# iucario/WorkoutDetector

Measured on AMD Instinct MI355X. Metric: clips/sec (8x3x224x224 TSM-R50), higher is better.
Workload: dtype f32

## Files before the change

workoutdetector_amd/csrc/tsm_engine.hip:

```cpp
#include <hip/hip_runtime.h>

#include <sys/stat.h>

#include <algorithm>
#include <cerrno>
#include <cmath>
#include <cstdio>
#include <cstdlib>
#include <cstring>
#include <map>
#include <string>
#include <vector>

#include "../../include/tsm_hip.h"
#include "tsm_host_util.h"
#include "tsm_kernels.h"

#ifndef TSM_BUILD_ID
#define TSM_BUILD_ID __DATE__ "/" __TIME__
#endif

namespace {

using namespace tsm_host;

const char kBuildTag[] = "tsm-build-id:" TSM_BUILD_ID;

struct Backbone {
  int depth;
  int blocks[4];
  bool basic;
};
constexpr Backbone kBackbones[] = {{18, {2, 2, 2, 2}, true}, {34, {3, 4, 6, 3}, true}, {50, {3, 4, 6, 3}, false}};
constexpr int kPlanes[4] = {64, 128, 256, 512};

const Backbone *find_backbone(int depth) {
  for (const Backbone &b : kBackbones)
    if (b.depth == depth) return &b;
  return nullptr;
}

thread_local std::string g_create_error;

struct HostTensor {
  std::vector<float> data;
  std::vector<int64_t> shape;
};

struct ConvLayer {
  std::string wkey, bnp;
  int cin = 0, cout = 0, k = 1, stride = 1;
  int cp = 0;
  int kp = 0;
  int kseg = 0;
  float *d_w = nullptr, *d_b = nullptr;
};

struct Block {
  int conv1, conv2, conv3, down;
  int stride;
  std::string name;
  float *d_wf = nullptr, *d_bf = nullptr;
  int kpf = 0;
  int ksegf = 0;
  float *d_w3f = nullptr;
  int cmid = 0;
  int cout3 = 0;
};

int ilog2(int v) {
  int l = 0;
  while ((1 << l) < v) ++l;
  return l;
}

struct GuardBuf {
  std::string name;
  char *base = nullptr;
  GuardLayout lay;
  size_t elem_bytes = 4;
  float *ptr() const { return reinterpret_cast<float *>(base + lay.lead); }
};

hipError_t guard_alloc(GuardBuf *g, const char *name, size_t payload_bytes, size_t frame_bytes, size_t elem_bytes = 4) {
  g->name = name;
  g->lay = guard_layout(payload_bytes, frame_bytes);
  g->elem_bytes = elem_bytes;
  void *q = nullptr;
  hipError_t st = hipMalloc(&q, g->lay.total());
  if (st != hipSuccess) return st;
  g->base = static_cast<char *>(q);
  st = hipMemsetD32(reinterpret_cast<hipDeviceptr_t>(q), (int)kPoisonWord, g->lay.total() / 4);
  return st != hipSuccess ? st : hipDeviceSynchronize();
}

hipError_t guard_verify(const GuardBuf &g, std::string *msg) {
  std::vector<uint32_t> host(std::max(g.lay.lead, g.lay.tail) / 4);
  for (int after = 0; after < 2; ++after) {
    const size_t bytes = after ? g.lay.tail : g.lay.lead;
    const hipError_t st = hipMemcpy(host.data(), g.base + (after ? g.lay.lead + g.lay.payload : 0), bytes, hipMemcpyDeviceToHost);
    if (st != hipSuccess) return st;
    const long bad = guard_first_bad(host.data(), bytes / 4);
    if (bad >= 0) {
      *msg = guard_message(g.name, g.lay, after != 0, (size_t)bad, g.elem_bytes, host[bad]);
      return hipSuccess;
    }
  }
  return hipSuccess;
}

}

struct tsm_engine {
  tsm_config cfg{};
  int depth = 50;
  int width = 64;
  int place = 0;
  int consensus = 0;
  int feat = 2048;
  bool weights_started = false;
  size_t tune_sig_base = 0;
  std::string err;
  hipStream_t stream = nullptr;
  bool finalized = false;
  int prec = tsm::kPrecF32;
  float *d_tap = nullptr;
  std::map<std::string, HostTensor> tensors;
  std::vector<ConvLayer> convs;
  std::vector<Block> blocks;
  float *d_fcw = nullptr, *d_fcb = nullptr;
  float *d_in = nullptr;
  float *d_in4 = nullptr;
  float *buf[5] = {nullptr, nullptr, nullptr, nullptr, nullptr};
  float *d_pooled = nullptr, *d_logits = nullptr;
  float *d_partial = nullptr;
  size_t partial_elems = 0;
  size_t buf_elems = 0;
  int h1 = 0, w1 = 0, hp = 0, wp = 0;
  hipEvent_t ev0 = nullptr, ev1 = nullptr;
  bool have_time = false;
  std::vector<void *> allocs;
  bool poison = false;
  std::vector<GuardBuf> guards;
  std::map<int, std::vector<int>> tile_cache;
  bool autotune = true;
  bool stem_pool = true;
  bool stem_direct = true;
  bool stem_planar = true;
  std::string tune_path, tune_sig;
  int force_tile = 0, force_code = -1;
  int fuse23 = -1;
  int fuse_block = -1;
  int fuse31 = -1;
  int fuse_front = -1;
  int walk = -1;
  int n_cu = 256;
  int timing_left = 0;
  bool timing_only3x3 = false;
  std::vector<std::vector<hipEvent_t>> timing;
  std::vector<hipEvent_t> event_pool;
  std::vector<hipEvent_t> *cur_timing = nullptr;
};

namespace {

int fail(tsm_engine *e, int code, const std::string &msg) {
  if (e) e->err = msg; else g_create_error = msg;
  return code;
}

#define TSM_HIP(e, call)                                                                        \
  do {                                                                                          \
    hipError_t _st = (call);                                                                    \
    if (_st != hipSuccess)                                                                      \
      return fail((e), TSM_ERR_HIP, std::string(#call) + ": " + hipGetErrorString(_st));        \
  } while (0)

void build_topology(tsm_engine *e) {
  e->convs.clear();
  e->blocks.clear();
  ConvLayer stem;
  stem.wkey = "base_model.conv1.weight";
  stem.bnp = "base_model.bn1";
  stem.cin = 3; stem.cout = 64; stem.k = 7; stem.stride = 2;
  stem.cp = 4;
  stem.kp = e->prec == tsm::kPrecF32 ? round_up(7 * 7 * 4, 32) : round_up(7 * 4 * 8, e->prec == tsm::kPrecBf16 ? 64 : 32);
  e->convs.push_back(stem);
  const Backbone &bb = *find_backbone(e->depth);
  const int expansion = bb.basic ? 1 : 4;
  int cin = 64;
  for (int li = 0; li < 4; ++li) {
    for (int b = 0; b < bb.blocks[li]; ++b) {
      const int planes = kPlanes[li];
      const int mid = planes * e->width / 64;
      const int stride = (b == 0 && li > 0) ? 2 : 1;
      const bool bp = e->place == 1;
      const std::string p = "base_model.layer" + std::to_string(li + 1) + "." + std::to_string(b) + (bp ? ".net" : "");
      const std::string c1key = p + (bp ? ".conv1.weight" : ".conv1.net.weight");
      Block blk;
      blk.stride = stride;
      blk.name = "layer" + std::to_string(li + 1) + "." + std::to_string(b);
      blk.down = -1;
      if (bb.basic) {
        ConvLayer c1; c1.wkey = c1key; c1.bnp = p + ".bn1";
        c1.cin = cin; c1.cout = planes; c1.k = 3; c1.stride = stride; c1.cp = cin; c1.kp = 9 * cin;
        ConvLayer c2; c2.wkey = p + ".conv2.weight"; c2.bnp = p + ".bn2";
        c2.cin = planes; c2.cout = planes; c2.k = 3; c2.stride = 1; c2.cp = planes; c2.kp = 9 * planes;
        c1.kseg = e->cfg.is_shift ? 0 : segment_len(c1.kp, e->prec);
        blk.conv1 = (int)e->convs.size(); e->convs.push_back(c1);
        blk.conv2 = (int)e->convs.size(); e->convs.push_back(c2);
        blk.conv3 = -1;
        if (stride != 1 || cin != planes) {
          ConvLayer d; d.wkey = p + ".downsample.0.weight"; d.bnp = p + ".downsample.1";
          d.cin = cin; d.cout = planes; d.k = 1; d.stride = stride; d.cp = cin; d.kp = cin;
          blk.down = (int)e->convs.size(); e->convs.push_back(d);
        }
        e->blocks.push_back(blk);
        cin = planes;
        continue;
      }
      ConvLayer c1; c1.wkey = c1key; c1.bnp = p + ".bn1";
      c1.cin = cin; c1.cout = mid; c1.k = 1; c1.stride = 1; c1.cp = cin; c1.kp = cin;
      ConvLayer c2; c2.wkey = p + ".conv2.weight"; c2.bnp = p + ".bn2";
      c2.cin = mid; c2.cout = mid; c2.k = 3; c2.stride = stride; c2.cp = mid; c2.kp = 9 * mid;
      ConvLayer c3; c3.wkey = p + ".conv3.weight"; c3.bnp = p + ".bn3";
      c3.cin = mid; c3.cout = planes * 4; c3.k = 1; c3.stride = 1; c3.cp = mid; c3.kp = mid;
      c1.kseg = segment_len(c1.kp, e->prec);
      c2.kseg = segment_len(c2.kp, e->prec);
      blk.conv1 = (int)e->convs.size(); e->convs.push_back(c1);
      blk.conv2 = (int)e->convs.size(); e->convs.push_back(c2);
      blk.conv3 = (int)e->convs.size(); e->convs.push_back(c3);
      if (b == 0) {
        ConvLayer d; d.wkey = p + ".downsample.0.weight"; d.bnp = p + ".downsample.1";
        d.cin = cin; d.cout = planes * 4; d.k = 1; d.stride = stride; d.cp = cin; d.kp = cin;
        blk.down = (int)e->convs.size(); e->convs.push_back(d);
      }
      e->blocks.push_back(blk);
      cin = planes * 4;
    }
  }
  e->feat = kPlanes[3] * expansion;
}

std::string unwrapped(const tsm_engine *e, const std::string &key) {
  if (e->place == 1) {
    const size_t at = key.find(".net.");
    return at == std::string::npos ? "" : key.substr(0, at) + key.substr(at + 4);
  }
  const std::string net = ".conv1.net.weight";
  if (key.size() > net.size() && key.compare(key.size() - net.size(), net.size(), net) == 0)
    return key.substr(0, key.size() - net.size()) + ".conv1.weight";
  return "";
}

const HostTensor *find_tensor(const tsm_engine *e, const std::string &key) {
  auto it = e->tensors.find(key);
  if (it != e->tensors.end()) return &it->second;
  const std::string alt = unwrapped(e, key);
  if (!alt.empty()) {
    it = e->tensors.find(alt);
    if (it != e->tensors.end()) return &it->second;
  }
  return nullptr;
}

bool known_name(const tsm_engine *e, const std::string &name) {
  if (name == "fc.weight" || name == "fc.bias") return true;
  static const char *bn_suffix[] = {".weight", ".bias", ".running_mean", ".running_var", ".num_batches_tracked"};
  auto is = [&](const std::string &key) { return name == key || name == unwrapped(e, key); };
  for (const ConvLayer &c : e->convs) {
    if (is(c.wkey)) return true;
    for (const char *s : bn_suffix)
      if (is(c.bnp + s)) return true;
  }
  return false;
}

int dev_alloc(tsm_engine *e, float **p, size_t elems, const char *name = "weights", size_t frame_elems = 0) {
  if (e->poison) {
    GuardBuf g;
    TSM_HIP(e, guard_alloc(&g, name, elems * sizeof(float), frame_elems * sizeof(float)));
    e->allocs.push_back(g.base);
    e->guards.push_back(g);
    *p = g.ptr();
    return TSM_OK;
  }
  void *q = nullptr;
  TSM_HIP(e, hipMalloc(&q, elems * sizeof(float)));
  e->allocs.push_back(q);
  *p = static_cast<float *>(q);
  return TSM_OK;
}

int poison_workspace(tsm_engine *e, hipStream_t s) {
  if (!e->poison) return TSM_OK;
  const float *targets[] = {e->buf[0], e->buf[1], e->buf[2], e->buf[3], e->buf[4], e->d_in4, e->d_pooled, e->d_logits, e->d_partial, e->d_tap};
  for (const GuardBuf &g : e->guards)
    for (const float *t : targets)
      if (t && t == g.ptr())
        TSM_HIP(e, hipMemsetD32Async(reinterpret_cast<hipDeviceptr_t>(g.ptr()), (int)kPoisonWord, g.lay.payload / 4, s));
  return TSM_OK;
}

int verify_guards(tsm_engine *e, hipStream_t s) {
  if (!e->poison) return TSM_OK;
  TSM_HIP(e, hipStreamSynchronize(s));
  for (const GuardBuf &g : e->guards) {
    std::string msg;
    TSM_HIP(e, guard_verify(g, &msg));
    if (!msg.empty()) return fail(e, TSM_ERR_GUARD, msg);
  }
  return TSM_OK;
}

tsm::ConvParams make_params(const ConvLayer &c, const float *x, const float *res, float *y, int n, int hi,
                            int wi, bool relu, int T, int shift_div, int prec = tsm::kPrecF32) {
  tsm::ConvParams p{};
  p.prec = prec;
  p.x = x; p.w = c.d_w; p.bias = c.d_b; p.res = res; p.y = y;
  p.N = n; p.Hi = hi; p.Wi = wi; p.C = c.cp; p.logC4 = ilog2(c.cp / 4);
  p.pad = c.k / 2; p.stride = c.stride;
  p.Ho = (hi + 2 * p.pad - c.k) / c.stride + 1;
  p.Wo = (wi + 2 * p.pad - c.k) / c.stride + 1;
  p.Cout = c.cout; p.Kp = c.kp; p.M = n * p.Ho * p.Wo; p.relu = relu ? 1 : 0;
  p.T = T; p.fold = T > 0 ? c.cp / shift_div : 0;
  p.kseg_len = res ? 0 : c.kseg;
  return p;
}

std::string default_tune_cache_path() {
  std::string base;
  if (const char *x = getenv("XDG_CACHE_HOME")) base = x;
  if (base.empty()) {
    const char *h = getenv("HOME");
    if (!h || !*h) return "";
    base = std::string(h) + "/.cache";
    (void)mkdir(base.c_str(), 0700);
  }
  base += "/tsm_hip";
  if (mkdir(base.c_str(), 0700) != 0 && errno != EEXIST) return "";
  return base + "/tune_cache.txt";
}

bool tune_cache_load(tsm_engine *e, int key, std::vector<int> *codes) {
  if (e->tune_path.empty()) return false;
  FILE *f = fopen(e->tune_path.c_str(), "r");
  if (!f) return false;
  const std::string want = e->tune_sig + "|" + std::to_string(key) + "|";
  char line[4096];
  bool ok = false;
  while (!ok && fgets(line, sizeof line, f)) ok = parse_tune_line(line, want, tsm::kNumTiles, codes);
  fclose(f);
  return ok;
}

void tune_cache_store(tsm_engine *e, int key, const std::vector<int> &codes) {
  if (e->tune_path.empty()) return;
  std::string line = e->tune_sig + "|" + std::to_string(key) + "|";
  for (size_t i = 0; i < codes.size(); ++i) line += (i ? "," : "") + std::to_string(codes[i]);
  line += "\n";
  if (line.size() >= 4096) return;
  FILE *f = fopen(e->tune_path.c_str(), "a");
  if (!f) return;
  fwrite(line.data(), 1, line.size(), f);
  fclose(f);
}

bool tail_split_from(const tsm::ConvParams &p, int n_cu, size_t partial_elems, int *tail_from) {
  if (p.kseg_len <= 0) return false;
  const long from = tsm_host::tail_split_point(p.M, p.Cout, tsm::conv_num_segments(p), n_cu, partial_elems);
  *tail_from = (int)from;
  return from > 0;
}

hipError_t launch_conv_code(tsm::ConvParams p, int ks, int code, float *partial, size_t partial_elems, int n_cu, hipStream_t s) {
  p.tile = code & kCodeTileMask;
  if ((code & kCodeSplitK) && p.kseg_len > 0 &&
      (size_t)tsm::conv_num_segments(p) * (size_t)p.M * (size_t)p.Cout <= partial_elems) {
    float *y = p.y;
    p.ksplit = 1;
    p.y = partial;
    hipError_t st = tsm::launch_conv(p, ks, s);
    if (st == hipSuccess)
      st = tsm::launch_splitk_reduce(partial, tsm::conv_num_segments(p), p.M, p.Cout, p.bias, nullptr, y, p.relu, s);
    return st;
  }
  if ((code & kCodeTailK) && (code & kCodeTileMask) == tsm::kTile64x64 && p.kseg_len > 0) {
    int tail_from = 0;
    if (tail_split_from(p, n_cu, partial_elems, &tail_from)) {
      float *y = p.y;
      const int mt0 = tail_from / (p.Cout / 64) * 64;
      p.ksplit = 2;
      p.tail_from = tail_from;
      p.ypart = partial;
      hipError_t st = tsm::launch_conv(p, ks, s);
      if (st == hipSuccess)
        st = tsm::launch_splitk_reduce(partial, tsm::conv_num_segments(p), p.M - mt0, p.Cout, p.bias, nullptr,
                                       y + (size_t)mt0 * p.Cout, p.relu, s);
      return st;
    }
  }
  return tsm::launch_conv(p, ks, s);
}

int checked_code(const tsm::ConvParams &p, int code) {
  return code > 0 && (code & ~kCodeValid) == 0 && tsm::conv_tile_valid(p, code & kCodeTileMask) ? code : 0;
}

struct Tap {
  const float *ptr = nullptr;
  int64_t shape[4] = {0, 0, 0, 0};
  bool hit = false;
};

struct LaunchTimer {
  tsm_engine *e;
  hipStream_t s;
  bool on;
  bool skip;
  LaunchTimer(tsm_engine *e_, hipStream_t s_, bool is3x3)
      : e(e_), s(s_), on(e_->cur_timing != nullptr), skip(e_->timing_only3x3 && !is3x3) { mark(); }
  ~LaunchTimer() { mark(); }
  void mark() {
    if (!on) return;
    if (skip) {
      e->cur_timing->push_back(nullptr);
      return;
    }
    hipEvent_t ev = nullptr;
    if (!e->event_pool.empty()) {
      ev = e->event_pool.back();
      e->event_pool.pop_back();
    } else if (hipEventCreate(&ev) != hipSuccess) {
      return;
    }
    (void)hipEventRecord(ev, s);
    e->cur_timing->push_back(ev);
  }
};
#define TSM_LAUNCH_K(e, s, is3x3, call) \
  do {                                  \
    LaunchTimer _lt((e), (s), (is3x3)); \
    TSM_HIP((e), (call));               \
  } while (0)
#define TSM_LAUNCH(e, s, call) TSM_LAUNCH_K(e, s, false, call)

void skip_slots(tsm_engine *e, int n) {
  if (e->cur_timing) e->cur_timing->insert(e->cur_timing->end(), 2 * (size_t)n, nullptr);
}

template <class F>
int time_best_of(tsm_engine *e, hipStream_t s, F &&launches, float *best_ms) {
  float ms[4];
  for (int rep = 0; rep < 4; ++rep) {
    TSM_HIP(e, hipEventRecord(e->ev0, s));
    TSM_HIP(e, launches());
    TSM_HIP(e, hipEventRecord(e->ev1, s));
    TSM_HIP(e, hipEventSynchronize(e->ev1));
    TSM_HIP(e, hipEventElapsedTime(&ms[rep], e->ev0, e->ev1));
  }
  *best_ms = std::min(ms[1], std::min(ms[2], ms[3]));
  return TSM_OK;
}

bool block_shift(const tsm_engine *e) { return e->place == 1 && e->cfg.is_shift; }

struct BlockLaunches {
  tsm::ConvParams p1, p2, p3;
  tsm::BneckParams pb{};
  tsm::FrontParams pfr{};
  tsm::Fused23Params pf{};
  tsm::Conv31Params q{};
};

BlockLaunches block_launches(const tsm_engine *e, size_t k, int nn, const float *x, float *y, float *t1, float *t2, int hh, int ww) {
  const tsm_config &cfg = e->cfg;
  const Block &blk = e->blocks[k];
  const ConvLayer &c1 = e->convs[blk.conv1], &c2 = e->convs[blk.conv2], &c3 = e->convs[blk.conv3];
  const int T = cfg.num_segments, shiftT = cfg.is_shift ? T : 0, prec = e->prec;
  const int ho = (hh + 2 - 3) / blk.stride + 1, wo = (ww + 2 - 3) / blk.stride + 1;
  const bool fused = blk.down >= 0;
  BlockLaunches L;
  L.p1 = make_params(c1, x, nullptr, t1, nn, hh, ww, true, shiftT, cfg.shift_div, prec);
  L.p2 = make_params(c2, t1, nullptr, t2, nn, hh, ww, true, 0, 1, prec);
  L.p3 = make_params(c3, t2, fused ? nullptr : x, y, nn, ho, wo, true, 0, 1, prec);
  if (fused) {
    const ConvLayer &cd = e->convs[blk.down];
    L.p3.w = blk.d_wf; L.p3.bias = blk.d_bf; L.p3.Kp = blk.kpf; L.p3.K1 = c3.kp; L.p3.kseg_len = blk.ksegf;
    L.p3.x2 = x; L.p3.C2 = cd.cp; L.p3.Hi2 = hh; L.p3.Wi2 = ww; L.p3.stride2 = blk.stride;
  }
  if (block_shift(e)) {
    L.p3.T = T;
    L.p3.fold = (fused ? e->convs[blk.down].cp : c3.cout) / cfg.shift_div;
  }
  tsm::BneckParams &pb = L.pb;
  pb.x = x; pb.w1 = c1.d_w; pb.bias1 = c1.d_b; pb.w2 = c2.d_w; pb.bias2 = c2.d_b; pb.y = y;
  pb.w3 = fused ? blk.d_wf : c3.d_w; pb.bias3 = fused ? blk.d_bf : c3.d_b;
  pb.cin = c1.cin; pb.N = nn; pb.H = hh; pb.W = ww; pb.T = shiftT; pb.fold = L.p1.fold;
  tsm::FrontParams &pfr = L.pfr;
  pfr.x = x; pfr.w1 = c1.d_w; pfr.bias1 = c1.d_b; pfr.w2 = c2.d_w; pfr.bias2 = c2.d_b; pfr.y = t2;
  pfr.N = nn; pfr.H = hh; pfr.W = ww; pfr.T = shiftT; pfr.fold = L.p1.fold;
  tsm::Fused23Params &pf = L.pf;
  pf.x = t1; pf.w2 = c2.d_w; pf.bias2 = c2.d_b; pf.w3f = blk.d_w3f ? blk.d_w3f : c3.d_w; pf.bias3 = c3.d_b; pf.res = x; pf.y = y;
  pf.N = nn; pf.H = hh; pf.W = ww; pf.M = nn * hh * ww; pf.kseg_len = c2.kseg;
  if (k + 1 < e->blocks.size() && e->blocks[k + 1].conv3 >= 0) {
    const ConvLayer &c1n = e->convs[e->blocks[k + 1].conv1];
    tsm::Conv31Params &q = L.q;
    q.t2 = L.p3.x; q.w3 = L.p3.w; q.bias3 = L.p3.bias; q.res = L.p3.res; q.y = L.p3.y;
    q.w1 = c1n.d_w; q.bias1 = c1n.d_b; q.t1 = t1;
    q.n_clips = nn / T; q.T = T; q.HW = ho * wo; q.K3 = L.p3.C; q.C = L.p3.Cout; q.N1 = c1n.cout;
    q.fold = shiftT > 0 ? c1n.cp / cfg.shift_div : 0;
  }
  return L;
}

struct BlockForms {
  bool block = false, front = false, conv23 = false, conv31 = false;
};

BlockForms fused_forms(const tsm_engine *e, size_t k, int nn, int hh, int ww, const char *stage) {
  BlockForms f;
  const Block &blk = e->blocks[k];
  if (blk.conv3 < 0 || block_shift(e)) return f;
  const ConvLayer &c1 = e->convs[blk.conv1], &c2 = e->convs[blk.conv2], &c3 = e->convs[blk.conv3];
  const BlockLaunches L = block_launches(e, k, nn, nullptr, nullptr, nullptr, nullptr, hh, ww);
  const bool bf16 = e->prec == tsm::kPrecBf16;
  auto want = [&](const char *part) { return stage && blk.name + part == stage; };
  f.block = bf16 && blk.stride == 1 && c1.cout == 64 && c2.cin == 64 && c2.cout == 64 && c3.cout == 256 &&
            (blk.down < 0 ? c1.cin == 256 : c1.cin == 64 && e->convs[blk.down].cp == 64) && e->fuse_block != 0 &&
            tsm::bneck_ws_valid(L.pb.cin, L.pb.N, L.pb.H, L.pb.W, L.pb.T, L.pb.fold) && !want(".conv1") && !want(".conv2");
  f.front = bf16 && blk.stride == 2 && c1.cin == 256 && c1.cout == 128 && c2.cin == 128 && c2.cout == 128 && e->fuse_front != 0 &&
            tsm::front_s2_valid(L.pfr.N, L.pfr.H, L.pfr.W, L.pfr.T, L.pfr.fold) && !want(".conv1");
  f.conv23 = (blk.d_w3f != nullptr || (bf16 && blk.cmid == 64 && tsm::conv23_ws_valid(nn, hh, ww))) && e->fuse23 != 0 &&
             !want(".conv2");
  f.conv31 = bf16 && blk.down < 0 && k + 1 < e->blocks.size() && e->blocks[k + 1].conv3 >= 0 && e->fuse31 != 0 &&
             tsm::conv31_valid(L.q);
  return f;
}

struct BlockPlan {
  bool block = false, front = false, conv1_done = false, conv23 = false, conv31_next = false;
};

std::vector<BlockPlan> plan_forward(const tsm_engine *e, const std::vector<int> *codes, int nn, const char *stage) {
  std::vector<BlockPlan> plan(e->blocks.size());
  int hh = e->hp, ww = e->wp;
  for (size_t k = 0; k < e->blocks.size(); ++k) {
    const Block &blk = e->blocks[k];
    const BlockForms can = fused_forms(e, k, nn, hh, ww, stage);
    auto chosen = [&](int force, int conv, int bit) { return force == 1 || (codes && ((*codes)[conv] & bit)); };
    BlockPlan &p = plan[k];
    p.conv1_done = k > 0 && plan[k - 1].conv31_next;
    if (can.block && chosen(e->fuse_block, blk.conv1, kCodeBlock)) p.block = true;
    else if (can.front && !p.conv1_done && chosen(e->fuse_front, blk.conv1, kCodeFront)) p.front = true;
    else if (can.conv23 && chosen(e->fuse23, blk.conv2, kCodeConv23)) p.conv23 = true;
    else if (can.conv31 && chosen(e->fuse31, blk.conv3, kCodeConv31)) p.conv31_next = true;
    hh = (hh + 2 - 3) / blk.stride + 1;
    ww = (ww + 2 - 3) / blk.stride + 1;
  }
  return plan;
}

struct Forward {
  tsm_engine *e;
  hipStream_t s;
  const char *stage;
  Tap *tap;
  int T, shiftT, prec;
  float *t1, *t2, *idb;
  std::vector<int> *tiles = nullptr;
  bool tuning = false;
  bool tapped = false;
  int flip = 0;
  int prev31 = -1;
  BlockLaunches prev;

  Forward(tsm_engine *e_, hipStream_t s_, const char *stage_, Tap *tap_)
      : e(e_), s(s_), stage(stage_), tap(tap_), T(e_->cfg.num_segments), shiftT(e_->cfg.is_shift ? T : 0), prec(e_->prec),
        t1(e_->buf[2]), t2(e_->buf[3]), idb(e_->buf[4]) {}

  int dir(int d) const { return e->walk >= 0 ? e->walk : d; }
  int next_dir() { return dir(flip ^= 1); }
  bool want(const std::string &name) const { return stage && name == stage; }
  int hit(const float *p, int64_t a, int64_t b, int64_t c, int64_t d) {
    tap->ptr = p; tap->shape[0] = a; tap->shape[1] = b; tap->shape[2] = c; tap->shape[3] = d; tap->hit = true;
    tapped = true;
    return TSM_OK;
  }
  hipError_t launch_code(tsm::ConvParams p, int ks, int code);
  hipError_t launch_pair(const tsm::ConvParams &a, int ks_a, int code_a, const tsm::ConvParams &b, int ks_b, int code_b) {
    const hipError_t st = launch_code(a, ks_a, code_a);
    return st != hipSuccess ? st : launch_code(b, ks_b, code_b);
  }
  template <class A, class B>
  int fused_wins(A &&many, B &&one, bool *wins) {
    float many_ms = 0.f, one_ms = 0.f;
    int rc = time_best_of(e, s, many, &many_ms);
    if (!rc) rc = time_best_of(e, s, one, &one_ms);
    *wins = one_ms < many_ms;
    return rc;
  }
  int conv(int idx, tsm::ConvParams p, int ks, bool is3x3);
  int run_basic(size_t k, int nn, float *x, float *y, int hh, int ww);
  int run_block(size_t k, const BlockPlan &plan, int nn, float *x, float *y, int hh, int ww);
  int tune_block(size_t k, int nn, float *x, float *y, int hh, int ww);
};

hipError_t Forward::launch_code(tsm::ConvParams p, int ks, int code) {
  return launch_conv_code(p, ks, code, e->d_partial, e->partial_elems, e->n_cu, s);
}

int Forward::conv(int idx, tsm::ConvParams p, int ks, bool is3x3) {
  p.reverse = next_dir();
  if (!tuning) {
    int code = tiles ? (*tiles)[idx] : 0;
    if (e->force_tile) code = e->force_tile;
    if (e->force_code >= 0) code = e->force_code;
    TSM_LAUNCH_K(e, s, is3x3, launch_code(p, ks, checked_code(p, code)));
    return TSM_OK;
  }
  std::vector<int> cands;
  if (p.kseg_len > 0) {
    const size_t need = (size_t)tsm::conv_num_segments(p) * p.M * p.Cout;
    const long tiles64 = (long)((p.M + 63) / 64) * (p.Cout / 64);
    for (int t : {(int)tsm::kTile64x64, (int)tsm::kTile32x32}) {
      cands.push_back(t);
      if (need <= e->partial_elems && tiles64 < 4L * e->n_cu) cands.push_back(t | kCodeSplitK);
    }
    int tail_from = 0;
    if (tail_split_from(p, e->n_cu, e->partial_elems, &tail_from)) cands.push_back((int)tsm::kTile64x64 | kCodeTailK);
  } else {
    for (int t = 1; t < tsm::kNumTiles; ++t)
      if (tsm::conv_tile_valid(p, t)) cands.push_back(t);
  }
  float best_ms = 0.f;
  int best = 0;
  for (int t : cands) {
    float ms = 0.f;
    const int rc = time_best_of(e, s, [&] { return launch_code(p, ks, t); }, &ms);
    if (rc) return rc;
    if (best == 0 || ms < best_ms) {
      best = t;
      best_ms = ms;
    }
  }
  (*tiles)[idx] = best;
  return TSM_OK;
}

int Forward::run_basic(size_t k, int nn, float *x, float *y, int hh, int ww) {
  const Block &blk = e->blocks[k];
  const std::string &name = blk.name;
  const ConvLayer &c1 = e->convs[blk.conv1], &c2 = e->convs[blk.conv2];
  const int ho = (hh + 2 - 3) / blk.stride + 1, wo = (ww + 2 - 3) / blk.stride + 1;
  const float *identity = x;
  if (blk.down >= 0) {
    tsm::ConvParams pd = make_params(e->convs[blk.down], x, nullptr, idb, nn, hh, ww, false, block_shift(e) ? shiftT : 0,
                                     e->cfg.shift_div, prec);
    int rcd = conv(blk.down, pd, 1, false);
    if (rcd) return rcd;
    identity = idb;
  }
  tsm::ConvParams p1 = make_params(c1, x, nullptr, t1, nn, hh, ww, true, shiftT, e->cfg.shift_div, prec);
  int rc1 = conv(blk.conv1, p1, 3, true);
  if (rc1) return rc1;
  if (want(name + ".conv1")) return hit(t1, nn, ho, wo, c1.cout);
  tsm::ConvParams p2 = make_params(c2, t1, identity, y, nn, ho, wo, true, 0, 1, prec);
  if (block_shift(e) && blk.down < 0) {
    p2.T = T;
    p2.fold = c2.cout / e->cfg.shift_div;
  }
  int rc2 = conv(blk.conv2, p2, 3, true);
  if (rc2) return rc2;
  if (want(name)) return hit(y, nn, ho, wo, c2.cout);
  return TSM_OK;
}

int Forward::run_block(size_t k, const BlockPlan &plan, int nn, float *x, float *y, int hh, int ww) {
  const Block &blk = e->blocks[k];
  const std::string &name = blk.name;
  const int c1out = e->convs[blk.conv1].cout, c2out = e->convs[blk.conv2].cout, c3out = e->convs[blk.conv3].cout;
  const int ho = (hh + 2 - 3) / blk.stride + 1, wo = (ww + 2 - 3) / blk.stride + 1;
  BlockLaunches L = block_launches(e, k, nn, x, y, t1, t2, hh, ww);
  if (blk.down >= 0) skip_slots(e, 1);
  if (plan.block) {
    L.pb.reverse = next_dir();
    TSM_LAUNCH(e, s, tsm::launch_bneck_ws(L.pb, s));
    skip_slots(e, 2);
    return want(name) ? hit(y, nn, ho, wo, c3out) : TSM_OK;
  }
  if (plan.front) {
    L.pfr.reverse = next_dir();
    TSM_LAUNCH(e, s, tsm::launch_front_s2(L.pfr, s));
    next_dir();
    skip_slots(e, 1);
  } else {
    if (plan.conv1_done) {
      skip_slots(e, 1);
    } else {
      int rc1 = conv(blk.conv1, L.p1, 1, false);
      if (rc1) return rc1;
    }
    if (want(name + ".conv1")) return hit(t1, nn, hh, ww, c1out);
    if (plan.conv23) {
      L.pf.reverse = next_dir();
      TSM_LAUNCH_K(e, s, true, tsm::launch_conv23_fused(L.pf, blk.cmid, blk.cout3, prec, s));
      skip_slots(e, 1);
      return want(name) ? hit(y, nn, ho, wo, c3out) : TSM_OK;
    }
    int rc2 = conv(blk.conv2, L.p2, 3, true);
    if (rc2) return rc2;
  }
  if (want(name + ".conv2")) return hit(t2, nn, ho, wo, c2out);
  if (plan.conv31_next) {
    L.q.reverse = next_dir();
    TSM_LAUNCH(e, s, tsm::launch_conv31_fused(L.q, s));
  } else {
    int rc3 = conv(blk.conv3, L.p3, 1, false);
    if (rc3) return rc3;
  }
  return want(name) ? hit(y, nn, ho, wo, c3out) : TSM_OK;
}

int Forward::tune_block(size_t k, int nn, float *x, float *y, int hh, int ww) {
  const Block &blk = e->blocks[k];
  std::vector<int> &codes = *tiles;
  const BlockForms can = fused_forms(e, k, nn, hh, ww, nullptr);
  BlockLaunches L = block_launches(e, k, nn, x, y, t1, t2, hh, ww);
  const int r1 = flip ^ 1;
  bool wins = false;
  int rc = conv(blk.conv1, L.p1, 1, false);
  if (rc) return rc;
  L.p1.reverse = dir(r1);
  if (prev31 >= 0 && e->fuse31 < 0) {
    const int conv3 = e->blocks[prev31].conv3, code3 = codes[conv3], code1 = codes[blk.conv1];
    tsm::ConvParams pc = L.p1;
    pc.reverse = dir(prev.p3.reverse ^ 1);
    prev.q.reverse = prev.p3.reverse;
    rc = fused_wins([&] { return launch_pair(prev.p3, 1, code3, pc, 1, code1); },
                    [&] { return tsm::launch_conv31_fused(prev.q, s); }, &wins);
    if (rc) return rc;
    if (wins) codes[conv3] |= kCodeConv31;
  }
  rc = conv(blk.conv2, L.p2, 3, true);
  if (rc) return rc;
  L.p2.reverse = dir(r1 ^ 1);
  if (can.front && e->fuse_front < 0) {
    const int code1 = codes[blk.conv1], code2 = codes[blk.conv2];
    L.pfr.reverse = dir(r1);
    rc = fused_wins([&] { return launch_pair(L.p1, 1, code1, L.p2, 3, code2); },
                    [&] { return tsm::launch_front_s2(L.pfr, s); }, &wins);
    if (rc) return rc;
    if (wins) codes[blk.conv1] |= kCodeFront;
  }
  rc = conv(blk.conv3, L.p3, 1, false);
  if (rc) return rc;
  L.p3.reverse = dir(r1);
  prev31 = can.conv31 ? (int)k : -1;
  prev = L;
  const int code1 = codes[blk.conv1], code2 = codes[blk.conv2], code3 = codes[blk.conv3];
  L.pf.reverse = dir(r1 ^ 1);
  L.pb.reverse = dir(r1);
  auto pair = [&] { return launch_pair(L.p2, 3, code2, L.p3, 1, code3); };
  auto fused23 = [&] { return tsm::launch_conv23_fused(L.pf, blk.cmid, blk.cout3, prec, s); };
  bool use_fused = can.conv23 && e->fuse23 == 1;
  if (can.conv23 && e->fuse23 < 0) {
    rc = fused_wins(pair, fused23, &use_fused);
    if (rc) return rc;
    if (use_fused) codes[blk.conv2] |= kCodeConv23;
  }
  if (can.block && e->fuse_block < 0) {
    rc = fused_wins([&] {
      const hipError_t st = launch_code(L.p1, 1, code1);
      return st != hipSuccess ? st : use_fused ? fused23() : pair();
    }, [&] { return tsm::launch_bneck_ws(L.pb, s); }, &wins);
    if (rc) return rc;
    if (wins) codes[blk.conv1] |= kCodeBlock;
  }
  return TSM_OK;
}

int run_forward(tsm_engine *e, const float *d_clips, int layout, int n_clips, float *d_logits,
                hipStream_t s, const char *stage, Tap *tap) {
  const tsm_config &cfg = e->cfg;
  const int T = cfg.num_segments, n = n_clips * T;
  Forward f(e, s, stage, tap);
  if (e->autotune && !stage) {
    auto it = e->tile_cache.find(tile_bucket(n_clips) * T);
    if (it == e->tile_cache.end()) {
      it = e->tile_cache.emplace(tile_bucket(n_clips) * T, std::vector<int>(e->convs.size(), 0)).first;
      f.tuning = true;
    }
    f.tiles = &it->second;
  }

  const int prec = e->prec;
  const float *in4 = e->d_in4;
  const bool pool_stem = e->stem_direct && e->stem_pool && !f.want("conv1");
  const bool planar = layout == TSM_LAYOUT_NTCHW && e->stem_planar && pool_stem && !f.want("input") &&
                      (double)cfg.height * cfg.width * 12.0 < 2.0e9 && (reinterpret_cast<uintptr_t>(d_clips) & 15u) == 0;
  if (layout >= TSM_LAYOUT_NTHWC4 || planar) {
    in4 = d_clips;
    skip_slots(e, 1);
  } else {
    TSM_LAUNCH(e, s, tsm::launch_pack_input(d_clips, e->d_in4, n, cfg.height, cfg.width,
                                            layout == TSM_LAYOUT_NTCHW ? 1 : 0, prec, s));
  }
  if (f.want("input"))
    return prec == tsm::kPrecF32 ? f.hit(in4, n, cfg.height, cfg.width, 4) : f.hit(in4, n, cfg.height, (cfg.width + 1) / 2, 8);

  float *cur = e->buf[0], *out = e->buf[1], *t1 = f.t1;
  {
    tsm::ConvParams p = make_params(e->convs[0], in4, nullptr, t1, n, cfg.height, cfg.width, true, 0, 1, prec);
    const bool direct = prec != tsm::kPrecF32 && e->stem_direct;
    if (pool_stem) {
      TSM_LAUNCH(e, s, tsm::launch_stem_pool(in4, e->convs[0].d_w, e->convs[0].d_b, cur, n, cfg.height, cfg.width,
                                              e->convs[0].kp, 1, prec, s, planar ? 1 : 0));
      skip_slots(e, 1);
    } else {
      if (direct) {
        TSM_LAUNCH(e, s, tsm::launch_stem_direct(in4, e->convs[0].d_w, e->convs[0].d_b, t1, n, cfg.height, cfg.width,
                                                  e->convs[0].kp, 1, prec, s));
      } else {
        int rc0 = f.conv(0, p, 7, false);
        if (rc0) return rc0;
      }
      if (f.want("conv1")) return f.hit(t1, n, e->h1, e->w1, 64);
      TSM_LAUNCH(e, s, tsm::launch_maxpool3x3s2(t1, cur, n, e->h1, e->w1, 64, prec, s));
    }
    if (f.want("stem")) return f.hit(cur, n, e->hp, e->wp, 64);
  }
  int h = e->hp, w = e->wp;
  const std::vector<BlockPlan> plan = f.tuning ? std::vector<BlockPlan>() : plan_forward(e, f.tiles, n, stage);
  for (size_t k = 0; k < e->blocks.size(); ++k) {
    const int rc = e->blocks[k].conv3 < 0 ? f.run_basic(k, n, cur, out, h, w)
                   : f.tuning            ? f.tune_block(k, n, cur, out, h, w)
                                         : f.run_block(k, plan[k], n, cur, out, h, w);
    if (rc || f.tapped) return rc;
    std::swap(cur, out);
    h = (h + 2 - 3) / e->blocks[k].stride + 1;
    w = (w + 2 - 3) / e->blocks[k].stride + 1;
  }
  if (stage) return fail(e, TSM_ERR_INVALID_ARG, std::string("unknown stage: ") + stage);
  if (e->consensus == 1) {
    TSM_LAUNCH(e, s, tsm::launch_head_segments(cur, e->d_fcw, e->d_fcb, d_logits, n, h * w, e->feat, cfg.num_class, prec, s));
    return TSM_OK;
  }
  TSM_LAUNCH(e, s, tsm::launch_head(cur, e->d_fcw, e->d_fcb, e->d_pooled, d_logits, n_clips, T, h * w, e->feat,
                                    cfg.num_class, prec, s));
  return TSM_OK;
}

int ensure_tuned(tsm_engine *e, const float *d_clips, int layout, int n_clips, float *d_out, hipStream_t s,
                 bool *from_file = nullptr) {
  const int tune_key = tile_bucket(n_clips) * e->cfg.num_segments;
  if (from_file) *from_file = false;
  if (!e->autotune || e->tile_cache.find(tune_key) != e->tile_cache.end()) return TSM_OK;
  std::vector<int> cached(e->convs.size(), 0);
  if (tune_cache_load(e, tune_key, &cached)) {
    e->tile_cache.emplace(tune_key, cached);
    if (from_file) *from_file = true;
    return TSM_OK;
  }
  std::vector<hipEvent_t> *saved = e->cur_timing;
  e->cur_timing = nullptr;
  const int rc = run_forward(e, d_clips, layout, n_clips, d_out, s, nullptr, nullptr);
  e->cur_timing = saved;
  if (rc) return rc;
  tune_cache_store(e, tune_key, e->tile_cache[tune_key]);
  return TSM_OK;
}

hipStream_t pick_stream(tsm_engine *e, int memkind, void *stream) {
  if (stream) return static_cast<hipStream_t>(stream);
  return memkind == TSM_MEM_HOST ? e->stream : nullptr;
}

void retag_tune_sig(tsm_engine *e) {
  if (e->tune_sig.empty()) return;
  e->tune_sig.resize(e->tune_sig_base);
  if (e->depth != 50) e->tune_sig += " r" + std::to_string(e->depth);
  if (e->width != 64) e->tune_sig += " w" + std::to_string(e->width);
  if (e->place == 1) e->tune_sig += " block";
}

int check_forward_args(tsm_engine *e, const void *clips, int memkind, int layout, int n_clips) {
  if (!e) return TSM_ERR_INVALID_ARG;
  if (!e->finalized) return fail(e, TSM_ERR_NOT_FINALIZED, "tsm_finalize has not been called");
  if (!clips) return fail(e, TSM_ERR_INVALID_ARG, "clips is NULL");
  if (memkind != TSM_MEM_HOST && memkind != TSM_MEM_DEVICE) return fail(e, TSM_ERR_INVALID_ARG, "bad memkind");
  if (layout < TSM_LAYOUT_NTCHW || layout > TSM_LAYOUT_NTHWC8B) return fail(e, TSM_ERR_INVALID_ARG, "bad layout");
  if (layout >= TSM_LAYOUT_NTHWC4 && memkind != TSM_MEM_DEVICE)
    return fail(e, TSM_ERR_INVALID_ARG, "packed layouts (NTHWC4 / NTHWC8S / NTHWC8B) are device-memory layouts");
  if ((layout == TSM_LAYOUT_NTHWC4 && e->prec != tsm::kPrecF32) ||
      (layout == TSM_LAYOUT_NTHWC8S && e->prec != tsm::kPrecBf16x3) ||
      (layout == TSM_LAYOUT_NTHWC8B && e->prec != tsm::kPrecBf16))
    return fail(e, TSM_ERR_INVALID_ARG, "packed layout does not match the engine dtype");
  if (n_clips <= 0) return fail(e, TSM_ERR_INVALID_ARG, "n_clips must be positive");
  if (n_clips > e->cfg.max_clips)
    return fail(e, TSM_ERR_CAPACITY, "n_clips " + std::to_string(n_clips) + " exceeds max_clips " +
                                         std::to_string(e->cfg.max_clips));
  return TSM_OK;
}

}

extern "C" {

int tsm_abi_version(void) { return TSM_ABI_VERSION; }

const char *tsm_build_id(void) { return kBuildTag + sizeof("tsm-build-id:") - 1; }

int tsm_trace_launches(int32_t on) {
  tsm::trace_launches(on != 0);
  return TSM_OK;
}

int64_t tsm_launch_trace(char *buf, int64_t cap) {
  const char *t = tsm::launch_trace();
  const int64_t need = (int64_t)strlen(t) + 1;
  if (buf && cap >= need) memcpy(buf, t, (size_t)need);
  return need;
}

const char *tsm_last_error(const tsm_engine *e) { return e ? e->err.c_str() : g_create_error.c_str(); }

int tsm_create(const tsm_config *cfg, tsm_engine **out) {
  if (!cfg || !out) return fail(nullptr, TSM_ERR_INVALID_ARG, "cfg/out is NULL");
  *out = nullptr;
  if (cfg->struct_size != (int32_t)sizeof(tsm_config))
    return fail(nullptr, TSM_ERR_INVALID_ARG, "tsm_config.struct_size mismatch (ABI)");
  if (cfg->num_class <= 0 || cfg->num_segments <= 0 || cfg->max_clips <= 0)
    return fail(nullptr, TSM_ERR_INVALID_ARG, "num_class, num_segments, max_clips must be positive");
  if (cfg->height < 32 || cfg->width < 32)
    return fail(nullptr, TSM_ERR_INVALID_ARG, "height/width must be >= 32");
  {
    const int64_t rows = (int64_t)cfg->max_clips * cfg->num_segments * ((cfg->height + 1) / 2) * ((cfg->width + 1) / 2);
    if (rows >= (int64_t)1 << 31)
      return fail(nullptr, TSM_ERR_CAPACITY, "max_clips * num_segments * (H/2) * (W/2) must stay below 2^31");
  }
  if (cfg->shift_div <= 0 || (64 % cfg->shift_div) != 0 || (64 / cfg->shift_div) % 4 != 0)
    return fail(nullptr, TSM_ERR_UNSUPPORTED, "shift_div must divide 64 with fold % 4 == 0 (8 or 16... )");
  if (cfg->dtype != TSM_DTYPE_F32 && cfg->dtype != TSM_DTYPE_BF16X3 && cfg->dtype != TSM_DTYPE_BF16)
    return fail(nullptr, TSM_ERR_UNSUPPORTED, "dtype must be TSM_DTYPE_F32, TSM_DTYPE_BF16X3 or TSM_DTYPE_BF16");
  if (cfg->dtype != TSM_DTYPE_F32 && (64 / cfg->shift_div) % 8 != 0)
    return fail(nullptr, TSM_ERR_UNSUPPORTED, "the bf16 formats need fold % 8 == 0 (shift_div <= 8)");
  int ndev = 0;
  hipError_t st = hipGetDeviceCount(&ndev);
  if (st != hipSuccess || ndev <= 0)
    return fail(nullptr, TSM_ERR_HIP, std::string("no HIP device: ") + hipGetErrorString(st));
  if (cfg->device_id < 0 || cfg->device_id >= ndev) return fail(nullptr, TSM_ERR_INVALID_ARG, "bad device_id");
  tsm_engine *e = new tsm_engine();
  e->cfg = *cfg;
  e->prec = cfg->dtype == TSM_DTYPE_BF16X3 ? tsm::kPrecBf16x3
            : cfg->dtype == TSM_DTYPE_BF16 ? tsm::kPrecBf16 : tsm::kPrecF32;
  if (const char *at = getenv("TSM_AUTOTUNE")) e->autotune = atoi(at) != 0;
  if (const char *sd = getenv("TSM_STEM_DIRECT")) e->stem_direct = atoi(sd) != 0;
  if (const char *sp = getenv("TSM_STEM_POOL")) e->stem_pool = atoi(sp) != 0;
  if (const char *pl = getenv("TSM_STEM_PLANAR")) e->stem_planar = atoi(pl) != 0;
  if (const char *ft = getenv("TSM_CONV_TILE")) e->force_tile = tsm::conv_tile_from_name(ft);
  if (const char *fc = getenv("TSM_CONV_CODE")) e->force_code = atoi(fc);
  if (const char *f23 = getenv("TSM_FUSE_CONV23")) e->fuse23 = atoi(f23) != 0;
  if (const char *fb = getenv("TSM_FUSE_BLOCK")) e->fuse_block = atoi(fb) != 0;
  if (const char *f31 = getenv("TSM_FUSE_C3C1")) e->fuse31 = atoi(f31) != 0;
  if (const char *ff = getenv("TSM_FUSE_FRONT")) e->fuse_front = atoi(ff) != 0;
  if (const char *wk = getenv("TSM_WALK")) e->walk = atoi(wk) != 0;
  if (const char *po = getenv("TSM_POISON")) e->poison = atoi(po) != 0;
  {
    const char *tc = getenv("TSM_TUNE_CACHE");
    if (tc) {
      if (*tc && strcmp(tc, "0") != 0 && strcmp(tc, "off") != 0) e->tune_path = tc;
    } else {
      e->tune_path = default_tune_cache_path();
    }
  }
  build_topology(e);
  st = hipSetDevice(cfg->device_id);
  if (st == hipSuccess) st = hipStreamCreateWithFlags(&e->stream, hipStreamNonBlocking);
  if (st == hipSuccess) st = hipDeviceGetAttribute(&e->n_cu, hipDeviceAttributeMultiprocessorCount, cfg->device_id);
  if (st == hipSuccess) st = hipEventCreate(&e->ev0);
  if (st == hipSuccess) st = hipEventCreate(&e->ev1);
  if (st != hipSuccess) {
    g_create_error = std::string("engine init: ") + hipGetErrorString(st);
    delete e;
    return TSM_ERR_HIP;
  }
  if (!e->tune_path.empty()) {
    hipDeviceProp_t prop;
    e->tune_sig = "abi" + std::to_string(TSM_ABI_VERSION) + " build " TSM_BUILD_ID " " +
                  (hipGetDeviceProperties(&prop, cfg->device_id) == hipSuccess ? std::string(prop.gcnArchName) : "?") +
                  " cu" + std::to_string(e->n_cu) +
                  " T" + std::to_string(cfg->num_segments) + " " + std::to_string(cfg->height) + "x" +
                  std::to_string(cfg->width) + " dtype" + std::to_string(cfg->dtype) + " shift" +
                  std::to_string(cfg->is_shift ? cfg->shift_div : 0) + " fuse" + std::to_string(e->fuse23) + "/" + std::to_string(e->fuse_block) + "/" + std::to_string(e->fuse31) + "/" + std::to_string(e->fuse_front) +
                  " stem" + std::to_string(e->stem_direct ? 1 : 0) +
                  std::to_string(e->stem_pool ? 1 : 0) + std::to_string(e->stem_planar ? 1 : 0);
    e->tune_sig_base = e->tune_sig.size();
  }
  *out = e;
  return TSM_OK;
}

int tsm_set_backbone(tsm_engine *e, int32_t depth) {
  if (!e) return TSM_ERR_INVALID_ARG;
  if (e->weights_started || e->finalized)
    return fail(e, TSM_ERR_INVALID_ARG, "tsm_set_backbone must come before the first tsm_set_tensor");
  if (!find_backbone(depth)) return fail(e, TSM_ERR_UNSUPPORTED, "depth must be 18, 34 or 50");
  if (find_backbone(depth)->basic && e->width != 64)
    return fail(e, TSM_ERR_UNSUPPORTED, "a BasicBlock backbone (depth 18 / 34) has no bottleneck width: the engine's is " +
                                            std::to_string(e->width));
  e->depth = depth;
  build_topology(e);
  retag_tune_sig(e);
  return TSM_OK;
}

int tsm_set_bottleneck_width(tsm_engine *e, int32_t width_per_group) {
  if (!e) return TSM_ERR_INVALID_ARG;
  if (e->weights_started || e->finalized)
    return fail(e, TSM_ERR_INVALID_ARG, "tsm_set_bottleneck_width must come before the first tsm_set_tensor");
  if (width_per_group != 64 && width_per_group != 128)
    return fail(e, TSM_ERR_UNSUPPORTED, "width_per_group must be 64 or 128 (wide_resnet50_2)");
  if (width_per_group != 64 && find_backbone(e->depth)->basic)
    return fail(e, TSM_ERR_UNSUPPORTED, "width_per_group 128 needs a Bottleneck backbone (depth 50): torchvision's BasicBlock "
                                        "supports 64 only");
  e->width = width_per_group;
  build_topology(e);
  retag_tune_sig(e);
  return TSM_OK;
}

int tsm_set_shift_place(tsm_engine *e, int32_t place) {
  if (!e) return TSM_ERR_INVALID_ARG;
  if (e->weights_started || e->finalized)
    return fail(e, TSM_ERR_INVALID_ARG, "tsm_set_shift_place must come before the first tsm_set_tensor");
  if (place != 0 && place != 1) return fail(e, TSM_ERR_UNSUPPORTED, "place must be 0 (blockres) or 1 (block)");
  e->place = place;
  build_topology(e);
  retag_tune_sig(e);
  return TSM_OK;
}

int tsm_set_consensus(tsm_engine *e, int32_t consensus) {
  if (!e) return TSM_ERR_INVALID_ARG;
  if (e->weights_started || e->finalized)
    return fail(e, TSM_ERR_INVALID_ARG, "tsm_set_consensus must come before the first tsm_set_tensor");
  if (consensus != 0 && consensus != 1) return fail(e, TSM_ERR_UNSUPPORTED, "consensus must be 0 (avg) or 1 (identity)");
  e->consensus = consensus;
  return TSM_OK;
}

void tsm_destroy(tsm_engine *e) {
  if (!e) return;
  (void)hipSetDevice(e->cfg.device_id);
  if (e->stream) (void)hipStreamSynchronize(e->stream);
  for (void *p : e->allocs) (void)hipFree(p);
  for (auto &v : e->timing)
    for (hipEvent_t ev : v)
      if (ev) (void)hipEventDestroy(ev);
  for (hipEvent_t ev : e->event_pool) (void)hipEventDestroy(ev);
  if (e->ev0) (void)hipEventDestroy(e->ev0);
  if (e->ev1) (void)hipEventDestroy(e->ev1);
  if (e->stream) (void)hipStreamDestroy(e->stream);
  delete e;
}

int tsm_set_tensor(tsm_engine *e, const char *name, const float *host_data, const int64_t *shape,
                   int32_t ndim) {
  if (!e) return TSM_ERR_INVALID_ARG;
  if (!name || !host_data || !shape || ndim < 1 || ndim > 4) return fail(e, TSM_ERR_INVALID_ARG, "bad tensor args");
  if (e->finalized) return fail(e, TSM_ERR_INVALID_ARG, "engine already finalized");
  const std::string key(name);
  e->weights_started = true;
  if (!known_name(e, key)) return fail(e, TSM_ERR_INVALID_ARG, "unknown tensor name: " + key);
  HostTensor t;
  size_t elems = 1;
  for (int i = 0; i < ndim; ++i) {
    if (shape[i] <= 0) return fail(e, TSM_ERR_SHAPE, "non-positive dim in " + key);
    t.shape.push_back(shape[i]);
    elems *= (size_t)shape[i];
  }
  t.data.assign(host_data, host_data + elems);
  e->tensors[key] = std::move(t);
  return TSM_OK;
}

int tsm_finalize(tsm_engine *e) {
  if (!e) return TSM_ERR_INVALID_ARG;
  if (e->finalized) return TSM_OK;
  TSM_HIP(e, hipSetDevice(e->cfg.device_id));
  const tsm_config &cfg = e->cfg;
  std::vector<std::vector<float>> host_wp(e->convs.size()), host_bias(e->convs.size());
  for (size_t ci = 0; ci < e->convs.size(); ++ci) {
    ConvLayer &c = e->convs[ci];
    const HostTensor *w = find_tensor(e, c.wkey);
    const HostTensor *g = find_tensor(e, c.bnp + ".weight"), *b = find_tensor(e, c.bnp + ".bias");
    const HostTensor *m = find_tensor(e, c.bnp + ".running_mean"), *v = find_tensor(e, c.bnp + ".running_var");
    if (!w) return fail(e, TSM_ERR_MISSING_TENSOR, "missing " + c.wkey);
    if (!g || !b || !m || !v) return fail(e, TSM_ERR_MISSING_TENSOR, "missing BatchNorm tensors of " + c.bnp);
    const std::vector<int64_t> want = {c.cout, c.cin, c.k, c.k};
    if (w->shape != want) return fail(e, TSM_ERR_SHAPE, "shape mismatch for " + c.wkey);
    for (const HostTensor *t : {g, b, m, v})
      if (t->shape.size() != 1 || t->shape[0] != c.cout) return fail(e, TSM_ERR_SHAPE, "BN shape mismatch for " + c.bnp);
    std::vector<float> wp, bias;
    if (c.k == 7 && e->prec != tsm::kPrecF32)
      fold_and_pack_stem_pairs(w->data.data(), g->data.data(), b->data.data(), m->data.data(), v->data.data(), c.cout,
                               c.kp, &wp, &bias);
    else
      fold_and_pack(w->data.data(), g->data.data(), b->data.data(), m->data.data(), v->data.data(), c.cout,
                    c.cin, c.k, c.cp, c.kp, &wp, &bias);
    if (c.k == 1) {
      host_wp[ci] = wp;
      host_bias[ci] = bias;
    }
    if (e->prec == tsm::kPrecBf16x3) to_split(&wp);
    if (e->prec == tsm::kPrecBf16) to_bf16(&wp);
    int rc = dev_alloc(e, &c.d_w, wp.size());
    if (rc) return rc;
    rc = dev_alloc(e, &c.d_b, bias.size());
    if (rc) return rc;
    TSM_HIP(e, hipMemcpy(c.d_w, wp.data(), wp.size() * sizeof(float), hipMemcpyHostToDevice));
    TSM_HIP(e, hipMemcpy(c.d_b, bias.data(), bias.size() * sizeof(float), hipMemcpyHostToDevice));
  }
  for (Block &blk : e->blocks) {
    if (blk.down < 0 || blk.conv3 < 0) continue;
    const ConvLayer &c3 = e->convs[blk.conv3], &cd = e->convs[blk.down];
    blk.kpf = c3.kp + cd.kp;
    blk.ksegf = segment_len(blk.kpf, e->prec);
    std::vector<float> wf, bf;
    concat_k_pair(host_wp[blk.conv3], host_bias[blk.conv3], c3.kp, host_wp[blk.down], host_bias[blk.down], cd.kp, c3.cout,
                  &wf, &bf);
    if (e->prec == tsm::kPrecBf16x3) to_split(&wf);
    if (e->prec == tsm::kPrecBf16) to_bf16(&wf);
    int rcf = dev_alloc(e, &blk.d_wf, wf.size());
    if (rcf) return rcf;
    rcf = dev_alloc(e, &blk.d_bf, bf.size());
    if (rcf) return rcf;
    TSM_HIP(e, hipMemcpy(blk.d_wf, wf.data(), wf.size() * sizeof(float), hipMemcpyHostToDevice));
    TSM_HIP(e, hipMemcpy(blk.d_bf, bf.data(), bf.size() * sizeof(float), hipMemcpyHostToDevice));
  }
  for (Block &blk : e->blocks) {
    if (blk.conv3 < 0) continue;
    const ConvLayer &c2 = e->convs[blk.conv2], &c3 = e->convs[blk.conv3];
    if (blk.down >= 0 || blk.stride != 1 || (c2.cout != 64 && c2.cout != 128)) continue;
    if (e->prec == tsm::kPrecBf16) {
      if (c2.cout == 64 && c2.cin == 64 && c3.cout == 256) { blk.cmid = 64; blk.cout3 = 256; }
      continue;
    }
    const int nchunk = c3.cout == 4 * c2.cout ? 4 : (c3.cout == 2 * c2.cout && c2.cout == 128) ? 2 : 0;
    if (nchunk == 0) continue;
    std::vector<float> w3f;
    if (e->prec == tsm::kPrecBf16x3) pack_w3_fragments_split(host_wp[blk.conv3].data(), c2.cout, &w3f, nchunk);
    else pack_w3_fragments(host_wp[blk.conv3].data(), c2.cout, &w3f, nchunk);
    int rcw = dev_alloc(e, &blk.d_w3f, w3f.size());
    if (rcw) return rcw;
    TSM_HIP(e, hipMemcpy(blk.d_w3f, w3f.data(), w3f.size() * sizeof(float), hipMemcpyHostToDevice));
    blk.cmid = c2.cout;
    blk.cout3 = c3.cout;
  }
  host_wp.clear();
  host_bias.clear();
  const HostTensor *fw = find_tensor(e, "fc.weight"), *fb = find_tensor(e, "fc.bias");
  if (!fw || !fb) return fail(e, TSM_ERR_MISSING_TENSOR, "missing fc.weight / fc.bias");
  if (fw->shape != std::vector<int64_t>{cfg.num_class, e->feat} || fb->shape != std::vector<int64_t>{cfg.num_class})
    return fail(e, TSM_ERR_SHAPE, "fc shape mismatch (want [num_class, " + std::to_string(e->feat) + "])");
  int rc = dev_alloc(e, &e->d_fcw, fw->data.size());
  if (rc) return rc;
  rc = dev_alloc(e, &e->d_fcb, fb->data.size());
  if (rc) return rc;
  TSM_HIP(e, hipMemcpy(e->d_fcw, fw->data.data(), fw->data.size() * sizeof(float), hipMemcpyHostToDevice));
  TSM_HIP(e, hipMemcpy(e->d_fcb, fb->data.data(), fb->data.size() * sizeof(float), hipMemcpyHostToDevice));

  e->h1 = (cfg.height + 6 - 7) / 2 + 1;
  e->w1 = (cfg.width + 6 - 7) / 2 + 1;
  e->hp = (e->h1 + 2 - 3) / 2 + 1;
  e->wp = (e->w1 + 2 - 3) / 2 + 1;
  const size_t frames = (size_t)cfg.max_clips * cfg.num_segments;
  size_t per_frame = (size_t)e->h1 * e->w1 * 64;
  {
    int hh = e->hp, ww = e->wp;
    for (const Block &blk : e->blocks) {
      const size_t in_px = (size_t)hh * ww;
      hh = (hh + 2 - 3) / blk.stride + 1;
      ww = (ww + 2 - 3) / blk.stride + 1;
      const size_t out_px = (size_t)hh * ww;
      for (int ci : {blk.conv1, blk.conv2, blk.conv3, blk.down}) {
        if (ci < 0) continue;
        const bool at_input = blk.conv3 >= 0 && ci == blk.conv1;
        per_frame = std::max(per_frame, (at_input ? in_px : out_px) * (size_t)e->convs[ci].cout);
      }
    }
  }
  e->buf_elems = frames * per_frame;
  for (int i = 0; i < 5; ++i) {
    static const char *const kBufNames[5] = {"buf[0]", "buf[1]", "buf[2]", "buf[3]", "buf[4]"};
    rc = dev_alloc(e, &e->buf[i], e->buf_elems, kBufNames[i], per_frame);
    if (rc) return rc;
  }
  rc = dev_alloc(e, &e->d_in, frames * 3 * cfg.height * cfg.width, "d_in", (size_t)3 * cfg.height * cfg.width);
  if (rc) return rc;
  rc = dev_alloc(e, &e->d_in4, frames * 4 * cfg.height * (cfg.width + 1), "d_in4", (size_t)4 * cfg.height * (cfg.width + 1));
  if (rc) return rc;
  rc = dev_alloc(e, &e->d_pooled, frames * (size_t)e->feat, "d_pooled", (size_t)e->feat);
  if (rc) return rc;
  rc = dev_alloc(e, &e->d_logits, (size_t)cfg.max_clips * (e->consensus == 1 ? cfg.num_segments : 1) * cfg.num_class, "d_logits",
                 (size_t)cfg.num_class);
  if (rc) return rc;
  if (e->prec == tsm::kPrecF32) {
    e->partial_elems = (size_t)16 << 20;
    rc = dev_alloc(e, &e->d_partial, e->partial_elems, "d_partial", per_frame);
    if (rc) return rc;
  }
  e->tensors.clear();
  e->finalized = true;
  return TSM_OK;
}

int tsm_forward(tsm_engine *e, const void *clips, int32_t memkind, int32_t layout, int32_t n_clips,
                float *logits, void *stream) {
  int rc = check_forward_args(e, clips, memkind, layout, n_clips);
  if (rc) return rc;
  if (!logits) return fail(e, TSM_ERR_INVALID_ARG, "logits is NULL");
  TSM_HIP(e, hipSetDevice(e->cfg.device_id));
  hipStream_t s = pick_stream(e, memkind, stream);
  const size_t in_elems = (size_t)n_clips * e->cfg.num_segments * 3 * e->cfg.height * e->cfg.width;
  const float *d_clips = static_cast<const float *>(clips);
  float *d_out = logits;
  if (memkind == TSM_MEM_HOST) {
    TSM_HIP(e, hipMemcpyAsync(e->d_in, clips, in_elems * sizeof(float), hipMemcpyHostToDevice, s));
    d_clips = e->d_in;
    d_out = e->d_logits;
  }
  e->cur_timing = nullptr;
  if (e->timing_left > 0) {
    --e->timing_left;
    e->timing.emplace_back();
    e->cur_timing = &e->timing.back();
  }
  rc = ensure_tuned(e, d_clips, layout, n_clips, d_out, s);
  if (rc) return rc;
  rc = poison_workspace(e, s);
  if (rc) return rc;
  TSM_HIP(e, hipEventRecord(e->ev0, s));
  rc = run_forward(e, d_clips, layout, n_clips, d_out, s, nullptr, nullptr);
  e->cur_timing = nullptr;
  if (rc) return rc;
  TSM_HIP(e, hipEventRecord(e->ev1, s));
  e->have_time = true;
  if (memkind == TSM_MEM_HOST) {
    const size_t rows = (size_t)n_clips * (e->consensus == 1 ? e->cfg.num_segments : 1);
    TSM_HIP(e, hipMemcpyAsync(logits, e->d_logits, rows * e->cfg.num_class * sizeof(float), hipMemcpyDeviceToHost, s));
    TSM_HIP(e, hipStreamSynchronize(s));
  }
  return e->poison ? verify_guards(e, s) : TSM_OK;
}

int tsm_tune(tsm_engine *e, int32_t n_clips, void *stream) {
  if (!e) return TSM_ERR_INVALID_ARG;
  if (!e->finalized) return fail(e, TSM_ERR_NOT_FINALIZED, "tsm_finalize has not been called");
  if (n_clips <= 0) return fail(e, TSM_ERR_INVALID_ARG, "n_clips must be positive");
  if (n_clips > e->cfg.max_clips)
    return fail(e, TSM_ERR_CAPACITY, "n_clips " + std::to_string(n_clips) + " exceeds max_clips " + std::to_string(e->cfg.max_clips));
  const int tune_key = tile_bucket(n_clips) * e->cfg.num_segments;
  if (!e->autotune || e->tile_cache.find(tune_key) != e->tile_cache.end()) return TSM_OK;
  TSM_HIP(e, hipSetDevice(e->cfg.device_id));
  hipStream_t s = static_cast<hipStream_t>(stream);
  const size_t frames = (size_t)n_clips * e->cfg.num_segments;
  TSM_HIP(e, hipMemsetAsync(e->d_in4, 0, frames * 4 * e->cfg.height * (e->cfg.width + 1) * sizeof(float), s));
  const int layout = e->prec == tsm::kPrecF32 ? TSM_LAYOUT_NTHWC4 : e->prec == tsm::kPrecBf16x3 ? TSM_LAYOUT_NTHWC8S : TSM_LAYOUT_NTHWC8B;
  bool from_file = false;
  int rc = ensure_tuned(e, e->d_in4, layout, n_clips, e->d_logits, s, &from_file);
  if (rc || !from_file) return rc;
  std::vector<hipEvent_t> *saved = e->cur_timing;
  e->cur_timing = nullptr;
  rc = run_forward(e, e->d_in4, layout, n_clips, e->d_logits, s, nullptr, nullptr);
  e->cur_timing = saved;
  return rc;
}

int tsm_forward_tap(tsm_engine *e, const void *clips, int32_t memkind, int32_t layout, int32_t n_clips,
                    const char *stage, float *out, int64_t out_capacity, int64_t out_shape[4],
                    void *stream) {
  int rc = check_forward_args(e, clips, memkind, layout, n_clips);
  if (rc) return rc;
  if (!stage || !out || !out_shape) return fail(e, TSM_ERR_INVALID_ARG, "stage/out/out_shape is NULL");
  TSM_HIP(e, hipSetDevice(e->cfg.device_id));
  hipStream_t s = pick_stream(e, memkind, stream);
  const size_t in_elems = (size_t)n_clips * e->cfg.num_segments * 3 * e->cfg.height * e->cfg.width;
  const float *d_clips = static_cast<const float *>(clips);
  if (memkind == TSM_MEM_HOST) {
    TSM_HIP(e, hipMemcpyAsync(e->d_in, clips, in_elems * sizeof(float), hipMemcpyHostToDevice, s));
    d_clips = e->d_in;
  }
  rc = poison_workspace(e, s);
  if (rc) return rc;
  Tap tap;
  rc = run_forward(e, d_clips, layout, n_clips, e->d_logits, s, stage, &tap);
  if (rc) return rc;
  const int64_t elems = tap.shape[0] * tap.shape[1] * tap.shape[2] * tap.shape[3];
  for (int i = 0; i < 4; ++i) out_shape[i] = tap.shape[i];
  if (elems > out_capacity) return fail(e, TSM_ERR_CAPACITY, "tap output buffer too small");
  if (e->prec != tsm::kPrecF32) {
    if (!e->d_tap) {
      const size_t cap = e->buf_elems > (size_t)e->cfg.max_clips * e->cfg.num_segments * 8 * e->cfg.height * e->cfg.width
                             ? e->buf_elems
                             : (size_t)e->cfg.max_clips * e->cfg.num_segments * 8 * e->cfg.height * e->cfg.width;
      rc = dev_alloc(e, &e->d_tap, cap, "d_tap", cap / ((size_t)e->cfg.max_clips * e->cfg.num_segments));
      if (rc) return rc;
    }
    TSM_HIP(e, tsm::launch_to_f32(tap.ptr, e->d_tap, elems / 8, e->prec, s));
    tap.ptr = e->d_tap;
  }
  TSM_HIP(e, hipMemcpyAsync(out, tap.ptr, (size_t)elems * sizeof(float),
                            memkind == TSM_MEM_HOST ? hipMemcpyDeviceToHost : hipMemcpyDeviceToDevice, s));
  TSM_HIP(e, hipStreamSynchronize(s));
  return e->poison ? verify_guards(e, s) : TSM_OK;
}

int tsm_set_layer_timing(tsm_engine *e, int32_t n_forwards, int32_t only_conv3x3) {
  if (!e) return TSM_ERR_INVALID_ARG;
  if (n_forwards < 0 || n_forwards > 64) return fail(e, TSM_ERR_INVALID_ARG, "n_forwards must be in [0, 64]");
  e->timing_only3x3 = only_conv3x3 != 0;
  for (auto &v : e->timing)
    for (hipEvent_t ev : v)
      if (ev) e->event_pool.push_back(ev);
  e->timing.clear();
  e->timing.reserve(64);
  e->timing_left = n_forwards;
  return TSM_OK;
}

int tsm_layer_times(tsm_engine *e, int32_t forward_index, float *ms_out, int32_t cap, int32_t *n_out) {
  if (!e || !ms_out || !n_out) return TSM_ERR_INVALID_ARG;
  if (forward_index < 0 || forward_index >= (int32_t)e->timing.size())
    return fail(e, TSM_ERR_INVALID_ARG, "no timing recorded for that forward");
  const std::vector<hipEvent_t> &ev = e->timing[forward_index];
  const int n = (int)ev.size() / 2;
  *n_out = n;
  if (n > cap) return fail(e, TSM_ERR_CAPACITY, "ms_out too small");
  for (int i = 0; i < n; ++i) {
    ms_out[i] = -1.f;
    if (!ev[2 * i] || !ev[2 * i + 1]) continue;
    TSM_HIP(e, hipEventSynchronize(ev[2 * i + 1]));
    TSM_HIP(e, hipEventElapsedTime(&ms_out[i], ev[2 * i], ev[2 * i + 1]));
  }
  return TSM_OK;
}

int tsm_conv_tiles(tsm_engine *e, int32_t n_clips, int32_t *tiles_out, int32_t cap, int32_t *n_out) {
  if (!e || !tiles_out || !n_out) return TSM_ERR_INVALID_ARG;
  std::vector<int> codes(e->convs.size(), 0);
  auto it = e->tile_cache.find(tile_bucket(n_clips) * e->cfg.num_segments);
  if (it != e->tile_cache.end()) {
    const std::vector<BlockPlan> plan = plan_forward(e, &it->second, n_clips * e->cfg.num_segments, nullptr);
    for (size_t i = 0; i < codes.size(); ++i) codes[i] = it->second[i] & ~kCodeFused;
    for (size_t k = 0; k < e->blocks.size(); ++k) {
      const Block &b = e->blocks[k];
      const BlockPlan &p = plan[k];
      codes[b.conv1] |= it->second[b.conv1] & ((p.block ? kCodeBlock : 0) | (p.front ? kCodeFront : 0));
      if (p.conv23) codes[b.conv2] |= it->second[b.conv2] & kCodeConv23;
      if (p.conv31_next) codes[b.conv3] |= it->second[b.conv3] & kCodeConv31;
    }
  }
  std::vector<int> order{0};
  for (const Block &b : e->blocks)
    for (int ci : {b.down, b.conv1, b.conv2, b.conv3})
      if (ci >= 0) order.push_back(ci);
  *n_out = (int32_t)order.size();
  if ((int)order.size() > cap) return fail(e, TSM_ERR_CAPACITY, "tiles_out too small");
  for (size_t i = 0; i < order.size(); ++i) tiles_out[i] = codes[order[i]];
  return TSM_OK;
}

float tsm_last_forward_ms(tsm_engine *e) {
  if (!e || !e->have_time) return -1.f;
  if (hipEventSynchronize(e->ev1) != hipSuccess) return -1.f;
  float ms = -1.f;
  if (hipEventElapsedTime(&ms, e->ev0, e->ev1) != hipSuccess) return -1.f;
  return ms;
}


int tsm_temporal_shift(const float *x, float *y, int64_t n_frames, int32_t n_segment, int64_t hw, int32_t c,
                       int32_t fold_div, void *stream) {
  if (!x || !y || n_frames <= 0 || hw <= 0 || c <= 0 || fold_div <= 0) return TSM_ERR_INVALID_ARG;
  const int fold = c / fold_div;
  hipError_t st = tsm::launch_temporal_shift(x, y, n_frames, n_segment, hw, c, fold, static_cast<hipStream_t>(stream));
  if (st != hipSuccess) return fail(nullptr, st == hipErrorInvalidValue ? TSM_ERR_INVALID_ARG : TSM_ERR_HIP,
                                    std::string("temporal_shift: ") + hipGetErrorString(st));
  return TSM_OK;
}

int tsm_conv_op(const tsm_conv_args *a, void *stream) {
  if (!a || a->struct_size != (int32_t)sizeof(tsm_conv_args))
    return fail(nullptr, TSM_ERR_INVALID_ARG, "tsm_conv_args.struct_size must be sizeof(tsm_conv_args)");
  const int dtype = a->dtype;
  if (dtype != TSM_DTYPE_F32 && dtype != TSM_DTYPE_BF16X3 && dtype != TSM_DTYPE_BF16)
    return fail(nullptr, TSM_ERR_UNSUPPORTED, "bad dtype");
  const int prec = dtype == TSM_DTYPE_BF16X3 ? tsm::kPrecBf16x3 : dtype == TSM_DTYPE_BF16 ? tsm::kPrecBf16 : tsm::kPrecF32;
  const bool x3 = prec != tsm::kPrecF32;
  const int n = a->n, hi = a->hi, wi = a->wi, cin = a->cin, cout = a->cout, k = a->k, stride = a->stride;
  const int T = a->shift_segments, fold_div = a->fold_div > 0 ? a->fold_div : 1;
  const float *residual = a->residual;
  const bool dual = a->x2 != nullptr;
  if (!a->x || !a->w || !a->gamma || !a->beta || !a->mean || !a->var || !a->y) return fail(nullptr, TSM_ERR_INVALID_ARG, "NULL pointer");
  if (n <= 0 || hi <= 0 || wi <= 0) return fail(nullptr, TSM_ERR_INVALID_ARG, "n, hi and wi must be positive");
  if (k != 1 && k != 3 && k != 7) return fail(nullptr, TSM_ERR_UNSUPPORTED, "k must be 1, 3 or 7");
  if (stride != 1 && stride != 2) return fail(nullptr, TSM_ERR_UNSUPPORTED, "stride must be 1 or 2");
  const bool stem = (k == 7);
  if (stem ? (cin != 3) : (cin % 32 != 0 || (cin & (cin - 1)) != 0))
    return fail(nullptr, TSM_ERR_UNSUPPORTED, "cin must be 3 (k=7) or a power of two >= 32");
  if (prec == tsm::kPrecBf16 && !stem && cin % 64 != 0)
    return fail(nullptr, TSM_ERR_UNSUPPORTED, "TSM_DTYPE_BF16 needs cin % 64 == 0");
  if (cout % 64 != 0) return fail(nullptr, TSM_ERR_UNSUPPORTED, "cout must be a multiple of 64");
  if (stem && (residual || dual || T > 0)) return fail(nullptr, TSM_ERR_INVALID_ARG, "the 7x7 stem has no residual, second source or shift");
  if (a->shift_target != 0 && a->shift_target != 1) return fail(nullptr, TSM_ERR_INVALID_ARG, "shift_target must be 0 or 1");
  const bool strided_1x1 = k == 1 && stride != 1;
  if (a->shift_target == 1 && !residual && !dual && !strided_1x1)
    return fail(nullptr, TSM_ERR_INVALID_ARG, "shift_target 1 needs a residual, a second source or a 1x1 at stride 2");
  if (T > 0 && a->shift_target == 0) {
    if (residual) return fail(nullptr, TSM_ERR_INVALID_ARG, "a shifted input with a residual: no such launch (shift_target 1 shifts the residual)");
    if (dual) return fail(nullptr, TSM_ERR_INVALID_ARG, "a shifted first source with a second source: no such launch");
    if (strided_1x1) return fail(nullptr, TSM_ERR_INVALID_ARG, "a shifted 1x1 at stride 2 is the identity's (shift_target 1)");
  }
  const int pad_ = k / 2;
  const int ho = (hi + 2 * pad_ - k) / stride + 1, wo = (wi + 2 * pad_ - k) / stride + 1;
  const int cin2 = a->cin2;
  if (dual) {
    if (k != 1) return fail(nullptr, TSM_ERR_UNSUPPORTED, "a second source needs a 1x1 main conv");
    if (residual) return fail(nullptr, TSM_ERR_INVALID_ARG, "a second source with a residual: no such launch");
    if (!a->w2 || !a->gamma2 || !a->beta2 || !a->mean2 || !a->var2) return fail(nullptr, TSM_ERR_INVALID_ARG, "NULL pointer (second source)");
    if (cin2 % 32 != 0 || (cin2 & (cin2 - 1)) != 0 || (prec == tsm::kPrecBf16 && cin2 % 64 != 0))
      return fail(nullptr, TSM_ERR_UNSUPPORTED, "cin2 must be a power of two >= 32 (TSM_DTYPE_BF16: >= 64)");
    if (a->stride2 != 1 && a->stride2 != 2) return fail(nullptr, TSM_ERR_UNSUPPORTED, "stride2 must be 1 or 2");
    if (a->hi2 <= 0 || a->wi2 <= 0 || (a->hi2 - 1) / a->stride2 + 1 != ho || (a->wi2 - 1) / a->stride2 + 1 != wo)
      return fail(nullptr, TSM_ERR_INVALID_ARG, "the second source's output size must equal the main conv's");
  }
  int fold = 0;
  if (T > 0) {
    const int shifted_c = a->shift_target == 0 ? cin : residual ? cout : dual ? cin2 : cin;
    fold = shifted_c / fold_div;
    if (n % T != 0) return fail(nullptr, TSM_ERR_INVALID_ARG, "n must be a whole number of T-frame clips");
    if (fold % (x3 ? 8 : 4) != 0)
      return fail(nullptr, TSM_ERR_UNSUPPORTED, x3 ? "the bf16 formats shift whole 8-channel groups: fold % 8 == 0"
                                                   : "fp32 shifts whole 4-channel groups: fold % 4 == 0");
    if (2 * fold > shifted_c) return fail(nullptr, TSM_ERR_INVALID_ARG, "2 * fold exceeds the shifted tensor's channels");
  }
  hipStream_t s = static_cast<hipStream_t>(stream);
  ConvLayer c;
  c.cin = cin; c.cout = cout; c.k = k; c.stride = stride;
  c.cp = stem ? 4 : cin;
  c.kp = (stem && x3) ? round_up(7 * 4 * 8, prec == tsm::kPrecBf16 ? 64 : 32)
                      : round_up(k * k * c.cp, prec == tsm::kPrecBf16 ? 64 : 32);
  const int kp2 = dual ? round_up(cin2, prec == tsm::kPrecBf16 ? 64 : 32) : 0;
#define TSM_HIP0(call)                                                                              \
  do {                                                                                              \
    hipError_t _st = (call);                                                                        \
    if (_st != hipSuccess) return fail(nullptr, TSM_ERR_HIP, std::string(#call) + ": " + hipGetErrorString(_st)); \
  } while (0)
  auto fetch_packed = [&](const float *w, const float *g, const float *b, const float *m, const float *v, int ci, int kk,
                          int cp, int kp, std::vector<float> *wp, std::vector<float> *bias) -> int {
    std::vector<float> hw_((size_t)cout * ci * kk * kk), hg(cout), hb(cout), hm(cout), hv(cout);
    TSM_HIP0(hipMemcpy(hw_.data(), w, hw_.size() * sizeof(float), hipMemcpyDeviceToHost));
    TSM_HIP0(hipMemcpy(hg.data(), g, cout * sizeof(float), hipMemcpyDeviceToHost));
    TSM_HIP0(hipMemcpy(hb.data(), b, cout * sizeof(float), hipMemcpyDeviceToHost));
    TSM_HIP0(hipMemcpy(hm.data(), m, cout * sizeof(float), hipMemcpyDeviceToHost));
    TSM_HIP0(hipMemcpy(hv.data(), v, cout * sizeof(float), hipMemcpyDeviceToHost));
    if (kk == 7 && x3) fold_and_pack_stem_pairs(hw_.data(), hg.data(), hb.data(), hm.data(), hv.data(), cout, kp, wp, bias);
    else fold_and_pack(hw_.data(), hg.data(), hb.data(), hm.data(), hv.data(), cout, ci, kk, cp, kp, wp, bias);
    return TSM_OK;
  };
  if (stem && x3 && stride != 2) return fail(nullptr, TSM_ERR_UNSUPPORTED, "the bf16 formats implement the 7x7 stem for stride 2 only");
  TSM_HIP0(hipStreamSynchronize(s));
  std::vector<float> wp, bias;
  int rc = fetch_packed(a->w, a->gamma, a->beta, a->mean, a->var, cin, k, c.cp, c.kp, &wp, &bias);
  if (rc) return rc;
  if (dual) {
    std::vector<float> wp2, bias2, wf, bf;
    rc = fetch_packed(a->w2, a->gamma2, a->beta2, a->mean2, a->var2, cin2, 1, cin2, kp2, &wp2, &bias2);
    if (rc) return rc;
    concat_k_pair(wp, bias, c.kp, wp2, bias2, kp2, cout, &wf, &bf);
    wp.swap(wf);
    bias.swap(bf);
  }
  if (prec == tsm::kPrecBf16x3) to_split(&wp);
  if (prec == tsm::kPrecBf16) to_bf16(&wp);
  float *d_w = nullptr, *d_b = nullptr, *d_x4 = nullptr, *d_xs = nullptr, *d_rs = nullptr, *d_ys = nullptr, *d_x2s = nullptr,
        *d_part = nullptr;
  struct Scratch {
    GuardBuf g[8];
    int n = 0;
    ~Scratch() {
      for (int i = 0; i < n; ++i)
        if (g[i].base) (void)hipFree(g[i].base);
    }
  } scratch;
  auto galloc = [&scratch](float **p, const char *name, size_t bytes, size_t frame_bytes, size_t elem_bytes) -> hipError_t {
    GuardBuf &g = scratch.g[scratch.n++];
    const hipError_t st_ = guard_alloc(&g, name, bytes, frame_bytes, elem_bytes);
    if (st_ == hipSuccess) *p = g.ptr();
    return st_;
  };
  const size_t act_bytes = prec == tsm::kPrecBf16 ? 2 : 4;
  TSM_HIP0(galloc(&d_w, "d_w", wp.size() * sizeof(float), (size_t)(wp.size() / cout) * sizeof(float), 4));
  TSM_HIP0(galloc(&d_b, "d_b", bias.size() * sizeof(float), 0, 4));
  TSM_HIP0(hipMemcpy(d_w, wp.data(), wp.size() * sizeof(float), hipMemcpyHostToDevice));
  TSM_HIP0(hipMemcpy(d_b, bias.data(), bias.size() * sizeof(float), hipMemcpyHostToDevice));
  c.d_w = d_w; c.d_b = d_b;
  const float *xin = a->x, *x2in = a->x2;
  const float *rin = residual;
  float *yout = a->y;
  const size_t out_elems = (size_t)n * ho * wo * cout;
  if (stem) {
    TSM_HIP0(galloc(&d_x4, "d_x4", (size_t)n * hi * wi * 8 * sizeof(float), (size_t)hi * wi * 8 * sizeof(float), 4));
    TSM_HIP0(tsm::launch_pack_input(a->x, d_x4, n, hi, wi, 0, prec, s));
    xin = d_x4;
  } else if (x3) {
    TSM_HIP0(galloc(&d_xs, "d_xs", (size_t)n * hi * wi * cin * act_bytes, (size_t)hi * wi * cin * act_bytes, act_bytes));
    TSM_HIP0(tsm::launch_from_f32(a->x, d_xs, (int64_t)n * hi * wi * cin / 8, prec, s));
    xin = d_xs;
  }
  if (x3) {
    TSM_HIP0(galloc(&d_ys, "d_ys", out_elems * act_bytes, (size_t)ho * wo * cout * act_bytes, act_bytes));
    yout = d_ys;
    if (residual) {
      TSM_HIP0(galloc(&d_rs, "d_rs", out_elems * act_bytes, (size_t)ho * wo * cout * act_bytes, act_bytes));
      TSM_HIP0(tsm::launch_from_f32(residual, d_rs, (int64_t)out_elems / 8, prec, s));
      rin = d_rs;
    }
    if (dual) {
      const size_t x2_elems = (size_t)n * a->hi2 * a->wi2 * cin2;
      TSM_HIP0(galloc(&d_x2s, "d_x2s", x2_elems * act_bytes, (size_t)a->hi2 * a->wi2 * cin2 * act_bytes, act_bytes));
      TSM_HIP0(tsm::launch_from_f32(a->x2, d_x2s, (int64_t)x2_elems / 8, prec, s));
      x2in = d_x2s;
    }
  }
  tsm::ConvParams p = make_params(c, xin, rin, yout, n, hi, wi, a->relu != 0, T > 0 ? T : 0, fold_div, prec);
  p.fold = fold;
  p.reverse = a->reverse != 0;
  if (dual) {
    p.Kp = c.kp + kp2; p.K1 = c.kp; p.kseg_len = segment_len(p.Kp, prec);
    p.x2 = x2in; p.C2 = cin2; p.Hi2 = a->hi2; p.Wi2 = a->wi2; p.stride2 = a->stride2;
  }
  const int code = checked_code(p, a->code);
  size_t part_elems = 0;
  if ((code & (kCodeSplitK | kCodeTailK)) && p.kseg_len > 0) {
    part_elems = (size_t)tsm::conv_num_segments(p) * p.M * p.Cout;
    TSM_HIP0(galloc(&d_part, "d_part", part_elems * sizeof(float), (size_t)ho * wo * cout * sizeof(float), 4));
  }
  int dev = 0, n_cu = 256;
  TSM_HIP0(hipGetDevice(&dev));
  TSM_HIP0(hipDeviceGetAttribute(&n_cu, hipDeviceAttributeMultiprocessorCount, dev));
  const char *sd_env = getenv("TSM_STEM_DIRECT");
  hipError_t st;
  if (stem && x3 && cout == 64 && !(sd_env && atoi(sd_env) == 0))
    st = tsm::launch_stem_direct(xin, c.d_w, c.d_b, yout, n, hi, wi, c.kp, a->relu != 0, prec, s);
  else
    st = launch_conv_code(p, k, code, d_part, part_elems, n_cu, s);
  if (st == hipSuccess && x3) st = tsm::launch_to_f32(d_ys, a->y, (int64_t)out_elems / 8, prec, s);
  hipError_t st2 = hipStreamSynchronize(s);
  if (st != hipSuccess) return fail(nullptr, st == hipErrorInvalidValue ? TSM_ERR_INVALID_ARG : TSM_ERR_HIP,
                                    std::string("launch_conv: ") + hipGetErrorString(st));
  if (st2 != hipSuccess) return fail(nullptr, TSM_ERR_HIP, std::string("conv sync: ") + hipGetErrorString(st2));
  for (int i = 0; i < scratch.n; ++i) {
    std::string msg;
    TSM_HIP0(guard_verify(scratch.g[i], &msg));
    if (!msg.empty()) return fail(nullptr, TSM_ERR_GUARD, "tsm_conv_op: " + msg);
  }
  return TSM_OK;
#undef TSM_HIP0
}

int tsm_conv_bn_act(const float *x, const float *w, const float *gamma, const float *beta, const float *mean,
                    const float *var, const float *residual, float *y, int32_t n, int32_t hi, int32_t wi,
                    int32_t cin, int32_t cout, int32_t k, int32_t stride, int32_t relu, int32_t shift_segments,
                    int32_t fold_div, int32_t dtype, void *stream) {
  tsm_conv_args a{};
  a.struct_size = sizeof(tsm_conv_args);
  a.x = x; a.w = w; a.gamma = gamma; a.beta = beta; a.mean = mean; a.var = var; a.residual = residual; a.y = y;
  a.n = n; a.hi = hi; a.wi = wi; a.cin = cin; a.cout = cout; a.k = k; a.stride = stride; a.relu = relu;
  a.shift_segments = shift_segments; a.fold_div = fold_div; a.dtype = dtype;
  a.code = tsm::conv_tile_from_name(getenv("TSM_CONV_TILE"));
  return tsm_conv_op(&a, stream);
}

int tsm_maxpool3x3s2(const float *x, float *y, int32_t n, int32_t hi, int32_t wi, int32_t c, void *stream) {
  if (!x || !y || n <= 0 || hi <= 0 || wi <= 0) return TSM_ERR_INVALID_ARG;
  hipError_t st = tsm::launch_maxpool3x3s2(x, y, n, hi, wi, c, tsm::kPrecF32, static_cast<hipStream_t>(stream));
  if (st != hipSuccess) return fail(nullptr, st == hipErrorInvalidValue ? TSM_ERR_INVALID_ARG : TSM_ERR_HIP,
                                    std::string("maxpool: ") + hipGetErrorString(st));
  return TSM_OK;
}

int tsm_preprocess(const void *frames, int32_t pixel, int32_t n, int32_t h, int32_t w, float *out,
                   int32_t out_layout, int32_t resize, int32_t crop, int32_t scale_255, void *stream) {
  if (!frames || !out || n <= 0 || h <= 0 || w <= 0 || resize <= 0 || crop <= 0)
    return fail(nullptr, TSM_ERR_INVALID_ARG, "bad preprocess arguments");
  if (pixel != TSM_PIXEL_U8 && pixel != TSM_PIXEL_F32) return fail(nullptr, TSM_ERR_INVALID_ARG, "bad pixel type");
  if (out_layout != TSM_LAYOUT_NTHWC4 && out_layout != TSM_LAYOUT_NTCHW && out_layout != TSM_LAYOUT_NTHWC8S &&
      out_layout != TSM_LAYOUT_NTHWC8B)
    return fail(nullptr, TSM_ERR_INVALID_ARG, "out_layout must be NTHWC4, NTHWC8S, NTHWC8B or NTCHW");
  tsm::PreprocParams p{};
  p.src = frames; p.dst = out; p.n = n; p.h = h; p.w = w;
  if (h <= w) { p.nh = resize; p.nw = (int)((double)resize * w / h); }
  else { p.nh = (int)((double)resize * h / w); p.nw = resize; }
  if (crop > p.nh || crop > p.nw) return fail(nullptr, TSM_ERR_INVALID_ARG, "crop larger than the resized frame");
  p.top = (int)std::nearbyint((p.nh - crop) / 2.0);
  p.left = (int)std::nearbyint((p.nw - crop) / 2.0);
  p.crop = crop;
  p.src_is_u8 = pixel == TSM_PIXEL_U8;
  p.out_mode = out_layout == TSM_LAYOUT_NTCHW ? 1 : out_layout == TSM_LAYOUT_NTHWC8S ? 2
               : out_layout == TSM_LAYOUT_NTHWC8B ? 3 : 0;
  p.pre_scale = scale_255 ? 1.0f / 255.0f : 1.0f;
  hipError_t st = tsm::launch_preprocess(p, static_cast<hipStream_t>(stream));
  if (st != hipSuccess) return fail(nullptr, st == hipErrorInvalidValue ? TSM_ERR_INVALID_ARG : TSM_ERR_HIP,
                                    std::string("preprocess: ") + hipGetErrorString(st));
  return TSM_OK;
}

int tsm_gather_clips(const void *frames, int64_t n_frames, int64_t frame_bytes, int64_t first_frame, int64_t total_frames,
                     int64_t pad_frame, int64_t first_clip, int32_t n_clips, int32_t n_segment, int32_t clip_step,
                     int32_t clip_stride, void *out, void *stream) {
  if (!frames || !out) return fail(nullptr, TSM_ERR_INVALID_ARG, "gather_clips: null pointer");
  tsm::GatherParams p{};
  p.frames = frames; p.out = out; p.n_frames = n_frames; p.frame_bytes = frame_bytes; p.first_frame = first_frame;
  p.total_frames = total_frames; p.first_clip = first_clip; p.pad_frame = pad_frame; p.n_clips = n_clips;
  p.n_segment = n_segment; p.clip_step = clip_step; p.clip_stride = clip_stride;
  hipError_t st = tsm::launch_gather_clips(p, static_cast<hipStream_t>(stream));
  if (st != hipSuccess)
    return fail(nullptr, st == hipErrorInvalidValue ? TSM_ERR_INVALID_ARG : TSM_ERR_HIP,
                st == hipErrorInvalidValue ? std::string("gather_clips: a clip of the range reads outside the frame buffer, "
                                                         "the pad frame is one of the range's video frames, or frame_bytes "
                                                         "is not a multiple of 16")
                                           : std::string("gather_clips: ") + hipGetErrorString(st));
  return TSM_OK;
}

int tsm_preprocess_clips(const void *frames, int32_t pixel, int64_t n_frames, int32_t h, int32_t w, int64_t first_frame,
                         int64_t total_frames, int64_t first_clip, int32_t n_clips, int32_t n_segment, int32_t clip_step,
                         int32_t clip_stride, const int32_t *boxes, float *out, int32_t out_layout, int32_t size,
                         int32_t scale_255, void *stream) {
  if (!frames || !boxes || !out) return fail(nullptr, TSM_ERR_INVALID_ARG, "preprocess_clips: null pointer");
  if (n_frames <= 0 || h <= 0 || w <= 0 || size <= 0 || n_clips <= 0 || n_segment <= 0)
    return fail(nullptr, TSM_ERR_INVALID_ARG, "preprocess_clips: non-positive size");
  if (pixel != TSM_PIXEL_U8 && pixel != TSM_PIXEL_F32) return fail(nullptr, TSM_ERR_INVALID_ARG, "bad pixel type");
  if (out_layout != TSM_LAYOUT_NTHWC4 && out_layout != TSM_LAYOUT_NTCHW && out_layout != TSM_LAYOUT_NTHWC8S &&
      out_layout != TSM_LAYOUT_NTHWC8B)
    return fail(nullptr, TSM_ERR_INVALID_ARG, "out_layout must be NTHWC4, NTHWC8S, NTHWC8B or NTCHW");
  tsm::ClipPreprocParams p{};
  p.src = frames; p.dst = out; p.boxes = boxes; p.n_frames = n_frames; p.first_frame = first_frame;
  p.total_frames = total_frames; p.first_clip = first_clip; p.n_clips = n_clips; p.n_segment = n_segment;
  p.clip_step = clip_step; p.clip_stride = clip_stride; p.h = h; p.w = w; p.size = size;
  p.src_is_u8 = pixel == TSM_PIXEL_U8;
  p.out_mode = out_layout == TSM_LAYOUT_NTCHW ? 1 : out_layout == TSM_LAYOUT_NTHWC8S ? 2
               : out_layout == TSM_LAYOUT_NTHWC8B ? 3 : 0;
  p.pre_scale = scale_255 ? 1.0f / 255.0f : 1.0f;
  hipError_t st = tsm::launch_preprocess_clips(p, static_cast<hipStream_t>(stream));
  if (st != hipSuccess)
    return fail(nullptr, st == hipErrorInvalidValue ? TSM_ERR_INVALID_ARG : TSM_ERR_HIP,
                st == hipErrorInvalidValue ? std::string("preprocess_clips: clip_step is not a multiple of clip_stride, a clip "
                                                         "starts past the end of the video, or a clip of the range reads "
                                                         "outside the frame buffer")
                                           : std::string("preprocess_clips: ") + hipGetErrorString(st));
  return TSM_OK;
}

int tsm_head(const float *feat, const float *fc_w, const float *fc_b, float *logits, int32_t n_clips,
             int32_t n_segment, int32_t hw, int32_t c, int32_t num_class, void *stream) {
  if (!feat || !fc_w || !fc_b || !logits || n_clips <= 0 || n_segment <= 0 || hw <= 0 || c <= 0 || num_class <= 0)
    return TSM_ERR_INVALID_ARG;
  hipStream_t s = static_cast<hipStream_t>(stream);
  float *pooled = nullptr;
  hipError_t st = hipMalloc(reinterpret_cast<void **>(&pooled), (size_t)n_clips * n_segment * c * sizeof(float));
  if (st != hipSuccess) return fail(nullptr, TSM_ERR_HIP, std::string("head scratch: ") + hipGetErrorString(st));
  st = tsm::launch_head(feat, fc_w, fc_b, pooled, logits, n_clips, n_segment, hw, c, num_class, tsm::kPrecF32, s);
  hipError_t st2 = hipStreamSynchronize(s);
  (void)hipFree(pooled);
  if (st != hipSuccess || st2 != hipSuccess)
    return fail(nullptr, TSM_ERR_HIP, std::string("head: ") + hipGetErrorString(st != hipSuccess ? st : st2));
  return TSM_OK;
}

int tsm_head_segments(const float *feat, const float *fc_w, const float *fc_b, float *logits, int32_t n_frames, int32_t hw,
                      int32_t c, int32_t num_class, void *stream) {
  if (!feat || !fc_w || !fc_b || !logits || n_frames <= 0 || hw <= 0 || c <= 0 || num_class <= 0)
    return fail(nullptr, TSM_ERR_INVALID_ARG, "head_segments: NULL pointer or non-positive size");
  if (c % 8 != 0 || c > 2048) return fail(nullptr, TSM_ERR_UNSUPPORTED, "head_segments: c must be a multiple of 8, at most 2048");
  hipError_t st = tsm::launch_head_segments(feat, fc_w, fc_b, logits, n_frames, hw, c, num_class, tsm::kPrecF32,
                                            static_cast<hipStream_t>(stream));
  if (st != hipSuccess) return fail(nullptr, TSM_ERR_HIP, std::string("head_segments: ") + hipGetErrorString(st));
  return TSM_OK;
}

int tsm_scores_to_states(const float *logits, int32_t n_clips, int32_t num_class, int32_t softmax, float threshold,
                         int32_t *states, float *top_score, void *stream) {
  if (!logits || !states || n_clips <= 0 || num_class <= 0)
    return fail(nullptr, TSM_ERR_INVALID_ARG, "scores_to_states: NULL pointer or non-positive size");
  hipError_t st = tsm::launch_scores_to_states(logits, n_clips, num_class, softmax != 0, threshold, states, top_score,
                                               static_cast<hipStream_t>(stream));
  if (st != hipSuccess) return fail(nullptr, TSM_ERR_HIP, std::string("scores_to_states: ") + hipGetErrorString(st));
  return TSM_OK;
}

}
```

workoutdetector_amd/csrc/tsm_host_util.h:

```cpp
#pragma once
#include <cmath>
#include <cstddef>
#include <cstdint>
#include <cstdio>
#include <cstdlib>
#include <cstring>
#include <string>
#include <vector>

namespace tsm_host {

constexpr float kBnEps = 1e-5f;

inline int segment_len(int kp, int prec) {
  if (prec != 0 ) return 0;
  const int nk = kp / 32;
  if (nk < 32) return 0;
  const int nseg = nk / 16;
  return (nk + nseg - 1) / nseg;
}

inline int round_up(int v, int m) { return (v + m - 1) / m * m; }

inline long tail_split_point(long m_rows, int cout, int n_seg, int n_cu, size_t scratch_elems, int wg_per_cu = 5) {
  if (m_rows <= 0 || cout <= 0 || cout % 64 != 0 || n_seg < 2 || n_cu <= 0) return 0;
  const long ntn = cout / 64, ntm = (m_rows + 63) / 64, tiles = ntm * ntn, slots = (long)wg_per_cu * n_cu;
  const long rounds = tiles / slots, rem = tiles - rounds * slots;
  if (rounds < 1 || rem == 0 || rem * 100 > slots * 85) return 0;
  const long from = rounds * slots / ntn * ntn;
  if (from <= 0 || from >= tiles) return 0;
  const size_t tail_rows = (size_t)(m_rows - (from / ntn) * 64);
  if ((size_t)n_seg * tail_rows * (size_t)cout > scratch_elems) return 0;
  return from;
}

inline uint16_t f2bf(float f) {
  uint32_t u;
  std::memcpy(&u, &f, 4);
  if ((u & 0x7fffffffu) > 0x7f800000u) return (uint16_t)((u >> 16) | 0x40);
  u += 0x7fffu + ((u >> 16) & 1u);
  return (uint16_t)(u >> 16);
}
inline float bf2f(uint16_t h) {
  const uint32_t u = (uint32_t)h << 16;
  float f;
  std::memcpy(&f, &u, 4);
  return f;
}
inline void to_bf16(std::vector<float> *v) {
  std::vector<float> out((v->size() + 1) / 2, 0.f);
  uint16_t *o = reinterpret_cast<uint16_t *>(out.data());
  for (size_t i = 0; i < v->size(); ++i) o[i] = f2bf((*v)[i]);
  v->swap(out);
}
inline void to_split(std::vector<float> *v) {
  uint16_t g[16];
  for (size_t i = 0; i + 8 <= v->size(); i += 8) {
    for (int e = 0; e < 8; ++e) {
      const float x = (*v)[i + e];
      g[e] = f2bf(x);
      g[8 + e] = f2bf(x - bf2f(g[e]));
    }
    std::memcpy(v->data() + i, g, 32);
  }
}

inline void fold_and_pack_stem_pairs(const float *w, const float *gamma, const float *beta, const float *mean,
                              const float *var, int cout, int kp, std::vector<float> *wp, std::vector<float> *bias) {
  wp->assign((size_t)cout * kp, 0.f);
  bias->resize(cout);
  for (int o = 0; o < cout; ++o) {
    const float scale = gamma[o] / std::sqrt(var[o] + kBnEps);
    (*bias)[o] = beta[o] - mean[o] * scale;
    float *dst = wp->data() + (size_t)o * kp;
    for (int c = 0; c < 3; ++c)
      for (int ky = 0; ky < 7; ++ky)
        for (int kx = 0; kx < 7; ++kx) {
          const int j = (kx + 1) >> 1, q = (kx + 1) & 1;
          dst[((ky * 4 + j) * 2 + q) * 4 + c] = w[(((size_t)o * 3 + c) * 7 + ky) * 7 + kx] * scale;
        }
  }
}

inline void fold_and_pack(const float *w, const float *gamma, const float *beta, const float *mean,
                   const float *var, int cout, int cin, int k, int cp, int kp, std::vector<float> *wp,
                   std::vector<float> *bias) {
  wp->assign((size_t)cout * kp, 0.f);
  bias->resize(cout);
  for (int o = 0; o < cout; ++o) {
    const float scale = gamma[o] / std::sqrt(var[o] + kBnEps);
    (*bias)[o] = beta[o] - mean[o] * scale;
    float *dst = wp->data() + (size_t)o * kp;
    for (int c = 0; c < cin; ++c)
      for (int ky = 0; ky < k; ++ky)
        for (int kx = 0; kx < k; ++kx)
          dst[(ky * k + kx) * cp + c] = w[(((size_t)o * cin + c) * k + ky) * k + kx] * scale;
  }
}

inline void concat_k_pair(const std::vector<float> &w1, const std::vector<float> &b1, int kp1, const std::vector<float> &w2,
                          const std::vector<float> &b2, int kp2, int cout, std::vector<float> *wf, std::vector<float> *bf) {
  const int kpf = kp1 + kp2;
  wf->assign((size_t)cout * kpf, 0.f);
  bf->resize(cout);
  for (int o = 0; o < cout; ++o) {
    std::memcpy(&(*wf)[(size_t)o * kpf], &w1[(size_t)o * kp1], kp1 * sizeof(float));
    std::memcpy(&(*wf)[(size_t)o * kpf + kp1], &w2[(size_t)o * kp2], kp2 * sizeof(float));
    (*bf)[o] = b1[o] + b2[o];
  }
}

constexpr uint32_t kPoisonWord = 0x7FC07FC0u;
constexpr size_t kGuardAlign = 512, kGuardMinBand = 4096;

inline size_t guard_band_bytes(size_t frame_bytes) {
  const size_t r = (frame_bytes + kGuardAlign - 1) / kGuardAlign * kGuardAlign;
  return r < kGuardMinBand ? kGuardMinBand : r;
}

struct GuardLayout {
  size_t lead = 0;
  size_t payload = 0;
  size_t tail = 0;
  size_t total() const { return lead + payload + tail; }
};

inline GuardLayout guard_layout(size_t payload_bytes, size_t frame_bytes) {
  GuardLayout g;
  g.payload = (payload_bytes + 3) / 4 * 4;
  g.lead = guard_band_bytes(frame_bytes);
  g.tail = (g.payload + kGuardAlign - 1) / kGuardAlign * kGuardAlign - g.payload + g.lead;
  return g;
}

inline long guard_first_bad(const uint32_t *words, size_t n, uint32_t fill = kPoisonWord) {
  for (size_t i = 0; i < n; ++i)
    if (words[i] != fill) return (long)i;
  return -1;
}

inline std::string guard_message(const std::string &name, const GuardLayout &g, bool after, size_t idx, size_t elem_bytes, uint32_t got) {
  const long long rel = after ? (long long)(g.payload + 4 * idx) : (long long)(4 * idx) - (long long)g.lead;
  const long long eb = elem_bytes ? (long long)elem_bytes : 4;
  const long long elem = rel >= 0 ? rel / eb : -((-rel + eb - 1) / eb);
  char hex[16];
  std::snprintf(hex, sizeof hex, "0x%08x", got);
  return name + ": stray store into the band " + (after ? "after" : "before") + " the buffer, element offset " + std::to_string(elem) +
         (after ? " (" + std::to_string(rel - (long long)g.payload) + " bytes past its end)" : " (" + std::to_string(-rel) + " bytes before its start)") +
         ", the word there is " + hex;
}

inline int tile_bucket(int n_clips) {
  int b = 1;
  while (b < n_clips) b <<= 1;
  return b;
}


inline void pack_w3_fragments(const float *w3p, int cmid, std::vector<float> *out, int nchunk = 4) {
  const int wgn = cmid / 32, nkk = cmid / 8;
  out->assign((size_t)nchunk * cmid * cmid, 0.f);
  for (int j = 0; j < nchunk; ++j)
    for (int wn = 0; wn < wgn; ++wn)
      for (int kk = 0; kk < nkk; ++kk)
        for (int lane = 0; lane < 64; ++lane)
          for (int s = 0; s < 4; ++s) {
            const int n = j * cmid + wn * 32 + (lane & 31), k = 8 * kk + 4 * (lane >> 5) + s;
            (*out)[((((size_t)j * wgn + wn) * nkk + kk) * 64 + lane) * 4 + s] = w3p[(size_t)n * cmid + k];
          }
}

inline void pack_w3_fragments_split(const float *w3p, int cmid, std::vector<float> *out, int nchunk = 4) {
  const int wgn = cmid / 32, nkq = cmid / 16;
  out->assign((size_t)nchunk * cmid * cmid, 0.f);
  uint16_t *o = reinterpret_cast<uint16_t *>(out->data());
  for (int j = 0; j < nchunk; ++j)
    for (int wn = 0; wn < wgn; ++wn)
      for (int kq = 0; kq < nkq; ++kq)
        for (int lane = 0; lane < 64; ++lane) {
          const int n = j * cmid + wn * 32 + (lane & 31), k0 = 16 * kq + 8 * (lane >> 5);
          const size_t base = ((((size_t)j * wgn + wn) * (2 * nkq) + 2 * kq) * 64 + lane) * 8;
          for (int e = 0; e < 8; ++e) {
            const float x = w3p[(size_t)n * cmid + k0 + e];
            const uint16_t hi = f2bf(x);
            o[base + e] = hi;
            o[base + 64 * 8 + e] = f2bf(x - bf2f(hi));
          }
        }
}

constexpr int kCodeTileMask = 0xF;
constexpr int kCodeSplitK = 0x100;
constexpr int kCodeTailK = 0x200;
constexpr int kCodeConv23 = 0x400;
constexpr int kCodeBlock = 0x800;
constexpr int kCodeConv31 = 0x1000;
constexpr int kCodeFront = 0x2000;
constexpr int kCodeFused = kCodeConv23 | kCodeBlock | kCodeConv31 | kCodeFront;
constexpr int kCodeValid = kCodeTileMask | kCodeSplitK | kCodeTailK | kCodeFused;

inline bool parse_tune_line(const char *line, const std::string &want, int num_tiles, std::vector<int> *codes) {
  if (strncmp(line, want.c_str(), want.size()) != 0) return false;
  std::vector<int> got;
  const char *q = line + want.size();
  while (*q && *q != '\n') {
    char *end = nullptr;
    const long v = strtol(q, &end, 10);
    if (end == q) return false;
    if (v < 0 || (v & ~(long)kCodeValid) != 0 || (int)(v & kCodeTileMask) >= num_tiles) return false;
    got.push_back((int)v);
    if (*end == ',') q = end + 1;
    else if (*end == '\n' || *end == 0) q = end;
    else return false;
  }
  if (got.size() != codes->size()) return false;
  *codes = got;
  return true;
}

}
```

workoutdetector_amd/csrc/tsm_igemm.hip:

```cpp
#include "tsm_device.h"

namespace tsm {

template <int BM, int BN, int WGM, int WGN, int KS, bool SHIFT, bool RES, int PREC, bool DUAL = false, bool SEG = false>
__global__ void __launch_bounds__(64 * WGM * WGN, (SEG && BM == 64) ? ((PREC & kPrecBlockShift) ? 4 : 5) : 1)
conv_igemm(const ConvParams p) {
  constexpr bool BSHIFT = (PREC & kPrecBlockShift) != 0;
  constexpr int PMODE = PREC & ~kPrecBlockShift;
  static_assert(!BSHIFT || (!SHIFT && !RES), "block placement: a shifted identity (DUAL = false) or a shifted second source");
  constexpr bool RESID = RES || (BSHIFT && !DUAL);
  static_assert(!SEG || (PMODE == kPrecF32 && !RES && WGM * WGN <= 4 && BM == BN && BM <= 64),
                "segmented K accumulation: fp32, 64x64 / 32x32 tiles, no residual (ConvParams::kseg_len)");
  static_assert(WGM * WGN == 4 || WGM * WGN == 1 || WGM * WGN == 8,
                "4 waves per workgroup, 1 (32x32 small-M tiles) or 8 (128x128 with 4 waves per SIMD at 2 workgroups/CU)");
  constexpr int NT = 64 * WGM * WGN;
  constexpr int LRP = NT / 8;
  static_assert(!DUAL || (KS == 1 && !SHIFT && !RES), "K-concatenated second source: plain 1x1 convs only");
  constexpr bool X3 = PMODE == kPrecBf16x3;
  constexpr bool BF = PMODE == kPrecBf16;
  constexpr int EB = BF ? 2 : 4;
  constexpr int KC = 128 / EB;
  static_assert(!SHIFT || KS == 1 || (KS == 3 && !SEG), "the temporal shift is fused into 1x1 and unsegmented 3x3 convs only");
  constexpr int WTM = BM / WGM, WTN = BN / WGN;
  constexpr int TM = WTM / 32, TN = WTN / 32;
  constexpr int APASS = BM / LRP, BPASS = BN / LRP;
  constexpr bool RK = PMODE == kPrecF32 && ((BM == 64 && BN == 64) || (BM == 32 && BN == 32));
  constexpr int NBUF = RK ? 1 : 2;
  constexpr int CLD = BN + 4;
  static_assert(TM >= 1 && TN >= 1, "wave tile must hold at least one 32x32 MFMA tile");
  constexpr int SMEM_FLOATS = NBUF * (BM + BN) * kLds > BM * CLD ? NBUF * (BM + BN) * kLds : BM * CLD;

  __shared__ __attribute__((aligned(16))) float smem[SMEM_FLOATS];

  const int tid = threadIdx.x;
  const int lane = tid & 63;
  const int wave = tid >> 6;
  const int wm = wave / WGN, wn = wave % WGN;
  const int half = lane >> 5, l31 = lane & 31;

  const int bid = blockIdx.x;
  const bool tail_mode = SEG && p.ksplit == 2;
  const bool in_tail = tail_mode && bid >= p.tail_from;
  const int nwg = tail_mode ? p.tail_from : (int)gridDim.x;
  const int q = nwg >> 3, r = nwg & 7, xcd = bid & 7;
  int tile = (xcd < r ? xcd * (q + 1) : r * (q + 1) + (xcd - r) * q) + (bid >> 3);
  if (p.reverse) tile = nwg - 1 - tile;
  int seg = 0;
  if (SEG && p.ksplit == 1) {
    seg = tile / (p.ntm * p.ntn);
    tile -= seg * (p.ntm * p.ntn);
  }
  if (in_tail) {
    const int u = bid - p.tail_from, n_tail = p.ntm * p.ntn - p.tail_from;
    seg = u / n_tail;
    tile = p.tail_from + (u - seg * n_tail);
  }
  const bool split_wg = SEG && (p.ksplit == 1 || in_tail);
  const int tm = tile / p.ntn, tn = tile - tm * p.ntn;
  const int m0 = tm * BM, n0 = tn * BN;

  const int HoWo = p.Ho * p.Wo;
  const int n_first = m0 / HoWo;
  const int frame0 = SHIFT ? (n_first > 0 ? n_first - 1 : 0) : n_first;
  constexpr bool PAIRS = KS == 7 && PMODE != kPrecF32;
  const int wpairs = (p.Wi + 1) >> 1;
  const size_t frame_elems = PAIRS ? (size_t)p.Hi * wpairs * 8 : (size_t)p.Hi * p.Wi * p.C;
  const size_t a_bytes = ((size_t)p.N - frame0) * frame_elems * EB;
  const __amdgpu_buffer_rsrc_t rsrcA = __builtin_amdgcn_make_buffer_rsrc(
      const_cast<char *>(reinterpret_cast<const char *>(p.x) + (size_t)frame0 * frame_elems * EB), 0,
      (int)(a_bytes > 0x7FFFFFF0u ? 0x7FFFFFF0u : a_bytes), 0x00020000);
  const __amdgpu_buffer_rsrc_t rsrcB = __builtin_amdgcn_make_buffer_rsrc(
      const_cast<char *>(reinterpret_cast<const char *>(p.w) + (size_t)n0 * p.Kp * EB), 0, BN * p.Kp * EB,
      0x00020000);

  const size_t frame_elems2 = DUAL ? (size_t)p.Hi2 * p.Wi2 * p.C2 : 0;
  const int frame02 = (BSHIFT && DUAL && n_first > 0) ? n_first - 1 : n_first;
  const size_t a2_bytes = DUAL ? ((size_t)p.N - frame02) * frame_elems2 * EB : 0;
  const __amdgpu_buffer_rsrc_t rsrcA2 = __builtin_amdgcn_make_buffer_rsrc(
      const_cast<char *>(reinterpret_cast<const char *>(DUAL ? p.x2 : p.x) + (size_t)frame02 * frame_elems2 * EB), 0,
      (int)(a2_bytes > 0x7FFFFFF0u ? 0x7FFFFFF0u : a2_bytes), 0x00020000);

  const int lrow = tid >> 3;
  const int chunk = tid & 7;
  const int frame_bytes = (int)(frame_elems * EB);
  unsigned a_off[APASS];
  unsigned a_offp[SHIFT ? APASS : 1], a_offm[SHIFT ? APASS : 1];
  unsigned a_mask[KS == 3 ? APASS : 1];
  unsigned a_off2[DUAL ? APASS : 1];
  unsigned a_off2p[(BSHIFT && DUAL) ? APASS : 1], a_off2m[(BSHIFT && DUAL) ? APASS : 1];
  int a_iy[KS == 7 ? APASS : 1], a_ix[KS == 7 ? APASS : 1];
#pragma unroll
  for (int pp = 0; pp < APASS; ++pp) {
    const int m = m0 + lrow + LRP * pp;
    const bool ok = m < p.M;
    const int mm = ok ? m : m0;
    const int n = mm / HoWo;
    const int rem = mm - n * HoWo;
    const int oy = rem / p.Wo, ox = rem - oy * p.Wo;
    const int iy0 = oy * p.stride - p.pad, ix0 = ox * p.stride - p.pad;
    if (KS == 7) {
      a_off[pp] = ok ? (unsigned)((n - frame0) * frame_bytes) : kInvalid;
      a_iy[pp] = iy0;
      a_ix[pp] = PAIRS ? (ix0 - 1) >> 1 : ix0;
    } else {
      const int base = (n - frame0) * frame_bytes + (iy0 * p.Wi + ix0) * p.C * EB + chunk * 16;
      a_off[pp] = (KS == 1 && !ok) ? kInvalid : (unsigned)base;
      if (DUAL)
        a_off2[pp] = ok ? (unsigned)((n - frame02) * (int)(frame_elems2 * EB) +
                                     (oy * p.stride2 * p.Wi2 + ox * p.stride2) * p.C2 * EB + chunk * 16)
                        : kInvalid;
      if (BSHIFT && DUAL) {
        const int t = n % p.T;
        a_off2p[pp] = (ok && t < p.T - 1) ? a_off2[pp] + (unsigned)(frame_elems2 * EB) : kInvalid;
        a_off2m[pp] = (ok && t > 0) ? a_off2[pp] - (unsigned)(frame_elems2 * EB) : kInvalid;
      }
      if (KS == 3) {
        unsigned mask = 0;
#pragma unroll
        for (int ky = 0; ky < 3; ++ky)
#pragma unroll
          for (int kx = 0; kx < 3; ++kx)
            if ((unsigned)(iy0 + ky) < (unsigned)p.Hi && (unsigned)(ix0 + kx) < (unsigned)p.Wi)
              mask |= 1u << (ky * 3 + kx);
        a_mask[pp] = ok ? mask : 0u;
      }
      if (SHIFT) {
        const int t = n % p.T;
        a_offp[pp] = (ok && t < p.T - 1) ? (unsigned)(base + frame_bytes) : kInvalid;
        a_offm[pp] = (ok && t > 0) ? (unsigned)(base - frame_bytes) : kInvalid;
      }
    }
  }
  unsigned b_off[BPASS];
#pragma unroll
  for (int pp = 0; pp < BPASS; ++pp) b_off[pp] = (unsigned)((lrow + LRP * pp) * p.Kp * EB + chunk * 16);

  f32x4 ra[APASS], rb[BPASS];
  const int nk1 = DUAL ? p.K1 / KC : 0;

  constexpr int NITEMS = APASS + BPASS;
  struct KStep {
    unsigned kbytes;
    int tap, tap_off;
    unsigned dead;
    unsigned mp, mm, m0;
  };
  auto kstep = [&](int kt, int nk_) {
    KStep k;
    k.kbytes = (unsigned)kt * (kBK * 4);
    k.dead = (~(unsigned)((kt - nk_) >> 31)) & kInvalid;
    k.tap = 0;
    k.tap_off = 0;
    int c0 = kt * KC;
    if (KS == 3) {
      k.tap = (kt * KC) >> (p.logC4 + 2);
      c0 = kt * KC - k.tap * p.C;
      const int ky = k.tap / 3, kx = k.tap - ky * 3;
      k.tap_off = ((ky * p.Wi + kx) * p.C + c0) * EB;
    }
    k.mp = k.mm = 0u;
    k.m0 = ~0u;
    if (SHIFT) {
      const int c = c0 + (X3 ? (chunk >> 1) * 8 : (BF ? chunk * 8 : chunk * 4));
      k.mp = 0u - (unsigned)(c < p.fold);
      k.mm = (0u - (unsigned)(c < 2 * p.fold)) & ~k.mp;
      k.m0 = ~(k.mp | k.mm);
    }
    if (BSHIFT && DUAL) {
      const int c = c0 - nk1 * KC + (X3 ? (chunk >> 1) * 8 : (BF ? chunk * 8 : chunk * 4));
      k.mp = 0u - (unsigned)(c < p.fold);
      k.mm = (0u - (unsigned)(c < 2 * p.fold)) & ~k.mp;
      k.m0 = ~(k.mp | k.mm);
    }
    return k;
  };
  auto gload_item = [&](const KStep &k, int kt, int item) {
    if (item < APASS) {
      const int pp = item;
      if (KS == 1) {
        unsigned off = a_off[pp];
        if (SHIFT) off = (a_offp[pp] & k.mp) | (a_offm[pp] & k.mm) | (a_off[pp] & k.m0);
        if (DUAL) {
          const bool second = kt >= nk1;
          const unsigned off2 = BSHIFT ? (a_off2p[pp] & k.mp) | (a_off2m[pp] & k.mm) | (a_off2[pp] & k.m0) : a_off2[pp];
          ra[pp] = buf_load4(second ? rsrcA2 : rsrcA, (second ? off2 : off) | k.dead,
                             second ? k.kbytes - (unsigned)nk1 * 128u : k.kbytes);
        } else {
          ra[pp] = buf_load4(rsrcA, off | k.dead, k.kbytes);
        }
      } else if (KS == 3) {
        if (SHIFT) {
          const unsigned off = (a_offp[pp] & k.mp) | (a_offm[pp] & k.mm) | (a_off[pp] & k.m0);
          const bool ok = ((a_mask[pp] >> k.tap) & 1u) && off != kInvalid;
          ra[pp] = buf_load4(rsrcA, (ok ? off + (unsigned)k.tap_off : kInvalid) | k.dead, 0);
        } else {
          ra[pp] = buf_load4(rsrcA, (((a_mask[pp] >> k.tap) & 1u) ? a_off[pp] + (unsigned)k.tap_off : kInvalid) | k.dead, 0);
        }
      } else {
        if constexpr (PAIRS) {
          const int g = X3 ? (kt * 8 + chunk) >> 1 : kt * 8 + chunk;
          const int ky = g >> 2, j = g & 3;
          const int iy = a_iy[pp] + ky, pc = a_ix[pp] + j;
          const bool ok = g < 28 && (unsigned)iy < (unsigned)p.Hi && (unsigned)pc < (unsigned)wpairs;
          const unsigned pix = X3 ? (unsigned)((iy * wpairs + pc) * 32 + (chunk & 1) * 16)
                                  : (unsigned)((iy * wpairs + pc) * 16);
          ra[pp] = buf_load4(rsrcA, (ok ? a_off[pp] + pix : kInvalid) | k.dead, 0);
        } else {
          const int tap = kt * 8 + chunk;
          const int ky = tap / 7, kx = tap - ky * 7;
          const int iy = a_iy[pp] + ky, ix = a_ix[pp] + kx;
          const bool ok = tap < 49 && (unsigned)iy < (unsigned)p.Hi && (unsigned)ix < (unsigned)p.Wi;
          ra[pp] = buf_load4(rsrcA, (ok ? a_off[pp] + (unsigned)((iy * p.Wi + ix) * 16) : kInvalid) | k.dead, 0);
        }
      }
    } else {
      const int pp = item - APASS;
      rb[pp] = buf_load4(rsrcB, b_off[pp] | k.dead, k.kbytes);
    }
  };
  auto lstore_item = [&](int buf, int item) {
    float *As = smem + buf * (BM + BN) * kLds;
    if (item < APASS)
      *reinterpret_cast<f32x4 *>(As + (lrow + LRP * item) * kLds + chunk * 4) = ra[item];
    else
      *reinterpret_cast<f32x4 *>(As + BM * kLds + (lrow + LRP * (item - APASS)) * kLds + chunk * 4) = rb[item - APASS];
  };

  f32x16 acc[TM][TN];
#pragma unroll
  for (int i = 0; i < TM; ++i)
#pragma unroll
    for (int j = 0; j < TN; ++j)
#pragma unroll
      for (int e = 0; e < 16; ++e) acc[i][j][e] = 0.f;

  f32x4 af[2][TM], bf[2][TN];
  auto frag_load = [&](int buf, int kk, int set) {
    const float *As = smem + buf * (BM + BN) * kLds + (wm * WTM + l31) * kLds + half * 4;
    const float *Bs = smem + buf * (BM + BN) * kLds + BM * kLds + (wn * WTN + l31) * kLds + half * 4;
#pragma unroll
    for (int i = 0; i < TM; ++i) af[set][i] = *reinterpret_cast<const f32x4 *>(As + i * 32 * kLds + kk * 8);
#pragma unroll
    for (int j = 0; j < TN; ++j) bf[set][j] = *reinterpret_cast<const f32x4 *>(Bs + j * 32 * kLds + kk * 8);
  };
  constexpr int NMFMA = 4 * TM * TN;
  auto mfma_group = [&](int set, auto &&inject) {
    int cnt = 0;
#pragma unroll
    for (int s = 0; s < 4; ++s)
#pragma unroll
      for (int i = 0; i < TM; ++i)
#pragma unroll
        for (int j = 0; j < TN; ++j) {
          acc[i][j] = __builtin_amdgcn_mfma_f32_32x32x2f32(af[set][i][s], bf[set][j][s], acc[i][j], 0, 0, 0);
          ++cnt;
          const int done = (cnt * NITEMS) / NMFMA, before = ((cnt - 1) * NITEMS) / NMFMA;
#pragma unroll
          for (int it = before; it < done; ++it) {
            inject(it);
            __builtin_amdgcn_sched_barrier(0);
          }
        }
  };
  auto no_inject = [](int) {};
  auto mfma_plain = [&](int set) {
#pragma unroll
    for (int s = 0; s < 4; ++s)
#pragma unroll
      for (int i = 0; i < TM; ++i)
#pragma unroll
        for (int j = 0; j < TN; ++j)
          acc[i][j] = __builtin_amdgcn_mfma_f32_32x32x2f32(af[set][i][s], bf[set][j][s], acc[i][j], 0, 0, 0);
  };
  (void)no_inject;

  u32x4 ah[2][TM], al[2][TM], bh[2][TN], bl[2][TN];
  auto frag_load_x3 = [&](int buf, int qg, int set) {
    const float *As = smem + buf * (BM + BN) * kLds + (wm * WTM + l31) * kLds + (2 * qg + half) * 8;
    const float *Bs = smem + buf * (BM + BN) * kLds + BM * kLds + (wn * WTN + l31) * kLds + (2 * qg + half) * 8;
#pragma unroll
    for (int i = 0; i < TM; ++i) {
      ah[set][i] = *reinterpret_cast<const u32x4 *>(As + i * 32 * kLds);
      al[set][i] = *reinterpret_cast<const u32x4 *>(As + i * 32 * kLds + 4);
    }
#pragma unroll
    for (int j = 0; j < TN; ++j) {
      bh[set][j] = *reinterpret_cast<const u32x4 *>(Bs + j * 32 * kLds);
      bl[set][j] = *reinterpret_cast<const u32x4 *>(Bs + j * 32 * kLds + 4);
    }
  };
  constexpr int NMFMA3 = 3 * TM * TN;
  auto mfma_x3 = [&](int set, int nitems, auto &&inject) {
    int cnt = 0;
#pragma unroll
    for (int i = 0; i < TM; ++i)
#pragma unroll
      for (int j = 0; j < TN; ++j)
#pragma unroll
        for (int t = 0; t < 3; ++t) {
          const bf16x8 a = __builtin_bit_cast(bf16x8, t == 2 ? al[set][i] : ah[set][i]);
          const bf16x8 b = __builtin_bit_cast(bf16x8, t == 1 ? bl[set][j] : bh[set][j]);
          acc[i][j] = __builtin_amdgcn_mfma_f32_32x32x16_bf16(a, b, acc[i][j], 0, 0, 0);
          ++cnt;
          const int done = (cnt * nitems) / NMFMA3, before = ((cnt - 1) * nitems) / NMFMA3;
#pragma unroll
          for (int it = before; it < done; ++it) {
            inject(it);
            __builtin_amdgcn_sched_barrier(0);
          }
        }
  };

  u32x4 af16[4][TM], bf16f[4][TN];
  auto frag_load_bf = [&](int buf, int qg) {
    const float *As = smem + buf * (BM + BN) * kLds + (wm * WTM + l31) * kLds + qg * 8 + half * 4;
    const float *Bs = smem + buf * (BM + BN) * kLds + BM * kLds + (wn * WTN + l31) * kLds + qg * 8 + half * 4;
#pragma unroll
    for (int i = 0; i < TM; ++i) af16[qg][i] = *reinterpret_cast<const u32x4 *>(As + i * 32 * kLds);
#pragma unroll
    for (int j = 0; j < TN; ++j) bf16f[qg][j] = *reinterpret_cast<const u32x4 *>(Bs + j * 32 * kLds);
  };
  constexpr int NMFMA_BF = TM * TN;
  auto mfma_bf = [&](int qg, int item0, int nitems, auto &&inject) {
    int cnt = 0;
#pragma unroll
    for (int i = 0; i < TM; ++i)
#pragma unroll
      for (int j = 0; j < TN; ++j) {
        acc[i][j] = __builtin_amdgcn_mfma_f32_32x32x16_bf16(__builtin_bit_cast(bf16x8, af16[qg][i]),
                                                            __builtin_bit_cast(bf16x8, bf16f[qg][j]), acc[i][j], 0, 0, 0);
        ++cnt;
        const int done = (cnt * nitems) / NMFMA_BF, before = ((cnt - 1) * nitems) / NMFMA_BF;
#pragma unroll
        for (int it = before; it < done; ++it) {
          inject(item0 + it);
          __builtin_amdgcn_sched_barrier(0);
        }
      }
  };

  constexpr int EW = (X3 || BF) ? 8 : 4;
  constexpr int TPR = BN / EW;
  constexpr int RPP = NT / TPR;
  constexpr int EPASS = BM / RPP;
  const int ecol = (tid % TPR) * EW, erow = tid / TPR;
  f32x4 rres[(RESID && !X3 && !BF) ? EPASS : 1];
  u32x4 rres_h[(RESID && (X3 || BF)) ? EPASS : 1], rres_l[(RESID && X3) ? EPASS : 1];
  if (RESID && (X3 || BF) && !BSHIFT) {
    const size_t r_bytes = ((size_t)p.M - m0) * p.Cout * EB;
    const __amdgpu_buffer_rsrc_t rsrcR = __builtin_amdgcn_make_buffer_rsrc(
        const_cast<char *>(reinterpret_cast<const char *>(p.res) + (size_t)m0 * p.Cout * EB), 0,
        (int)(r_bytes > 0x7FFFFFF0u ? 0x7FFFFFF0u : r_bytes), 0x00020000);
#pragma unroll
    for (int k = 0; k < EPASS; ++k) {
      const unsigned o = (unsigned)(((erow + k * RPP) * p.Cout + n0 + ecol) * EB);
      rres_h[k] = __builtin_amdgcn_raw_buffer_load_b128(rsrcR, (int)o, 0, 0);
      if (X3) rres_l[k] = __builtin_amdgcn_raw_buffer_load_b128(rsrcR, (int)(o + 16), 0, 0);
    }
  }
  if (RESID && !X3 && !BF && !BSHIFT) {
    const size_t r_bytes = ((size_t)p.M - m0) * p.Cout * 4;
    const __amdgpu_buffer_rsrc_t rsrcR = __builtin_amdgcn_make_buffer_rsrc(
        const_cast<float *>(p.res + (size_t)m0 * p.Cout), 0,
        (int)(r_bytes > 0x7FFFFFF0u ? 0x7FFFFFF0u : r_bytes), 0x00020000);
#pragma unroll
    for (int k = 0; k < EPASS; ++k)
      rres[k] = buf_load4(rsrcR, (unsigned)(((erow + k * RPP) * p.Cout + n0 + ecol) * 4), 0);
  }
  if constexpr (RESID && BSHIFT) {
    const int rbase = m0 >= HoWo ? m0 - HoWo : 0;
    const int c = n0 + ecol;
    const int sel = c < p.fold ? 1 : c < 2 * p.fold ? -1 : 0;
    const unsigned step = (unsigned)(HoWo * p.Cout * EB);
    const size_t r_bytes = ((size_t)p.M - rbase) * p.Cout * EB;
    const __amdgpu_buffer_rsrc_t rsrcR = __builtin_amdgcn_make_buffer_rsrc(
        const_cast<char *>(reinterpret_cast<const char *>(p.res) + (size_t)rbase * p.Cout * EB), 0,
        (int)(r_bytes > 0x7FFFFFF0u ? 0x7FFFFFF0u : r_bytes), 0x00020000);
#pragma unroll
    for (int k = 0; k < EPASS; ++k) {
      const int rr = erow + k * RPP;
      const int t = ((m0 + rr) / HoWo) % p.T;
      unsigned o = (unsigned)(((m0 - rbase + rr) * p.Cout + c) * EB);
      if (sel > 0) o = t < p.T - 1 ? o + step : kInvalid;
      if (sel < 0) o = t > 0 ? o - step : kInvalid;
      if constexpr (X3 || BF) {
        rres_h[k] = __builtin_amdgcn_raw_buffer_load_b128(rsrcR, (int)o, 0, 0);
        if (X3) rres_l[k] = __builtin_amdgcn_raw_buffer_load_b128(rsrcR, (int)(o + 16), 0, 0);
      } else {
        rres[k] = buf_load4(rsrcR, o, 0);
      }
    }
  }

  int kt0 = 0, nk = p.Kp / KC;
  if (split_wg) {
    kt0 = seg * p.kseg_len;
    nk = kt0 + p.kseg_len < nk ? kt0 + p.kseg_len : nk;
  }
  f32x16 tot[SEG ? TM : 1][SEG ? TN : 1];
  if constexpr (SEG) {
#pragma unroll
    for (int i = 0; i < TM; ++i)
#pragma unroll
      for (int j = 0; j < TN; ++j)
#pragma unroll
        for (int e = 0; e < 16; ++e) tot[i][j][e] = 0.f;
  }
  auto seg_flush = [&]() {
    if constexpr (SEG) {
#pragma unroll
      for (int i = 0; i < TM; ++i)
#pragma unroll
        for (int j = 0; j < TN; ++j) {
          tot[i][j] += acc[i][j];
#pragma unroll
          for (int e = 0; e < 16; ++e) acc[i][j][e] = 0.f;
        }
    }
  };
  const int seg_len = (SEG && p.kseg_len > 0) ? p.kseg_len : 0x3fffffff;
  {
    const KStep k0 = kstep(kt0, nk);
#pragma unroll
    for (int it = 0; it < NITEMS; ++it) gload_item(k0, kt0, it);
#pragma unroll
    for (int it = 0; it < NITEMS; ++it) lstore_item(0, it);
    const KStep k1 = kstep(kt0 + 1, nk);
#pragma unroll
    for (int it = 0; it < NITEMS; ++it) gload_item(k1, kt0 + 1, it);
  }
  __syncthreads();
  if constexpr (BF) {
    frag_load_bf(0, 0);
    frag_load_bf(0, 1);
    for (int kt = kt0; kt < nk; ++kt) {
      const int cur = (kt - kt0) & 1;
      const KStep k2 = kstep(kt + 2, nk);
      frag_load_bf(cur, 2);
      frag_load_bf(cur, 3);
      auto inject = [&](int it) {
        if (it < NITEMS) lstore_item(cur ^ 1, it);
        else gload_item(k2, kt + 2, it - NITEMS);
      };
      mfma_bf(0, 0, NITEMS, inject);
      mfma_bf(1, NITEMS, NITEMS, inject);
      __syncthreads();
      __builtin_amdgcn_sched_barrier(0);
      mfma_bf(2, 0, 0, [](int) {});
      frag_load_bf(cur ^ 1, 0);
      __builtin_amdgcn_sched_barrier(0);
      mfma_bf(3, 0, 0, [](int) {});
      __builtin_amdgcn_sched_barrier(0);
      frag_load_bf(cur ^ 1, 1);
      __builtin_amdgcn_sched_barrier(0);
    }
  } else if constexpr (RK) {
    f32x4 ra_[4], rb_[4];
    const bool trim = KS == 7 && p.Kp == 224 && nk == 7;
    const int nk_full = trim ? nk - 1 : nk;
    for (int kt = kt0; kt < nk_full;) {
    const int kend = (SEG && kt + seg_len < nk_full) ? kt + seg_len : nk_full;
    for (; kt < kend; ++kt) {
      const KStep k2 = kstep(kt + 2, nk);
      {
        const float *As = smem + (wm * WTM + l31) * kLds + half * 4;
        const float *Bs = smem + BM * kLds + (wn * WTN + l31) * kLds + half * 4;
#pragma unroll
        for (int kk = 0; kk < 4; ++kk) {
          ra_[kk] = *reinterpret_cast<const f32x4 *>(As + kk * 8);
          rb_[kk] = *reinterpret_cast<const f32x4 *>(Bs + kk * 8);
        }
      }
      __syncthreads();
      int cnt = 0;
#pragma unroll
      for (int kk = 0; kk < 4; ++kk)
#pragma unroll
        for (int s4 = 0; s4 < 4; ++s4) {
          acc[0][0] = __builtin_amdgcn_mfma_f32_32x32x2f32(ra_[kk][s4], rb_[kk][s4], acc[0][0], 0, 0, 0);
          ++cnt;
          const int done = cnt < 12 ? (cnt * 2 * NITEMS) / 12 : 2 * NITEMS;
          const int before = cnt - 1 < 12 ? ((cnt - 1) * 2 * NITEMS) / 12 : 2 * NITEMS;
#pragma unroll
          for (int it = before; it < done; ++it) {
            if (it < NITEMS) lstore_item(0, it);
            else gload_item(k2, kt + 2, it - NITEMS);
            __builtin_amdgcn_sched_barrier(0);
          }
        }
      __syncthreads();
    }
    seg_flush();
    }
    if (KS == 7 && trim) {
      const f32x4 a0 = *reinterpret_cast<const f32x4 *>(smem + (wm * WTM + l31) * kLds + half * 4);
      const f32x4 b0 = *reinterpret_cast<const f32x4 *>(smem + BM * kLds + (wn * WTN + l31) * kLds + half * 4);
      __syncthreads();
#pragma unroll
      for (int s4 = 0; s4 < 4; ++s4)
        acc[0][0] = __builtin_amdgcn_mfma_f32_32x32x2f32(a0[s4], b0[s4], acc[0][0], 0, 0, 0);
    }
  } else if constexpr (!X3) {
    frag_load(0, 0, 0);
    frag_load(0, 1, 1);
    for (int kt = kt0; kt < nk;) {
    const int kend = (SEG && kt + seg_len < nk) ? kt + seg_len : nk;
    for (; kt < kend; ++kt) {
      const int cur = (kt - kt0) & 1;
      const KStep k2 = kstep(kt + 2, nk);
      mfma_plain(0);
      frag_load(cur, 2, 0);
      mfma_group(1, [&](int it) { lstore_item(cur ^ 1, it); });
      frag_load(cur, 3, 1);
      mfma_group(0, [&](int it) { gload_item(k2, kt + 2, it); });
      __syncthreads();
      frag_load(cur ^ 1, 0, 0);
      __builtin_amdgcn_sched_barrier(0);
      mfma_plain(1);
      __builtin_amdgcn_sched_barrier(0);
      frag_load(cur ^ 1, 1, 1);
      __builtin_amdgcn_sched_barrier(0);
    }
    seg_flush();
    }
  } else {
    frag_load_x3(0, 0, 0);
    frag_load_x3(0, 1, 1);
    for (int kt = kt0; kt < nk; ++kt) {
      const int cur = (kt - kt0) & 1;
      const KStep k2 = kstep(kt + 2, nk);
      mfma_x3(0, 2 * NITEMS, [&](int it) {
        if (it < NITEMS) lstore_item(cur ^ 1, it);
        else gload_item(k2, kt + 2, it - NITEMS);
      });
      __syncthreads();
      frag_load_x3(cur ^ 1, 0, 0);
      __builtin_amdgcn_sched_barrier(0);
      mfma_x3(1, 0, [](int) {});
      __builtin_amdgcn_sched_barrier(0);
      frag_load_x3(cur ^ 1, 1, 1);
      __builtin_amdgcn_sched_barrier(0);
    }
  }

  float *Cs = smem;
#pragma unroll
  for (int i = 0; i < TM; ++i)
#pragma unroll
    for (int j = 0; j < TN; ++j)
#pragma unroll
      for (int e = 0; e < 16; ++e)
        Cs[(wm * WTM + i * 32 + (e & 3) + 8 * (e >> 2) + 4 * half) * CLD + wn * WTN + j * 32 + l31] =
            SEG ? tot[SEG ? i : 0][SEG ? j : 0][e] : acc[i][j][e];
  __syncthreads();

  const bool partial = split_wg;
  const size_t y_bytes = ((size_t)p.M - m0) * p.Cout * EB;
  const int mt0 = in_tail ? (p.tail_from / p.ntn) * BM : 0;
  char *ybase = in_tail ? reinterpret_cast<char *>(p.ypart) + ((size_t)seg * (p.M - mt0) + (m0 - mt0)) * p.Cout * EB
                        : reinterpret_cast<char *>(p.y) + ((size_t)(partial ? seg : 0) * p.M + m0) * p.Cout * EB;
  const __amdgpu_buffer_rsrc_t rsrcY = __builtin_amdgcn_make_buffer_rsrc(
      ybase, 0, (int)(y_bytes > 0x7FFFFFF0u ? 0x7FFFFFF0u : y_bytes), 0x00020000);
  const float floor_ = (p.relu && !partial) ? 0.f : -INFINITY;
  if constexpr (BF) {
    const f32x4 bias0 = *reinterpret_cast<const f32x4 *>(p.bias + n0 + ecol);
    const f32x4 bias1 = *reinterpret_cast<const f32x4 *>(p.bias + n0 + ecol + 4);
#pragma unroll
    for (int k = 0; k < EPASS; ++k) {
      const int rr = erow + k * RPP;
      const f32x4 c0 = *reinterpret_cast<const f32x4 *>(Cs + rr * CLD + ecol);
      const f32x4 c1 = *reinterpret_cast<const f32x4 *>(Cs + rr * CLD + ecol + 4);
      float v[8] = {c0[0] + bias0[0], c0[1] + bias0[1], c0[2] + bias0[2], c0[3] + bias0[3],
                    c1[0] + bias1[0], c1[1] + bias1[1], c1[2] + bias1[2], c1[3] + bias1[3]};
      if (RESID) {
#pragma unroll
        for (int e = 0; e < 8; ++e) v[e] += split_elem(rres_h[k], e);
      }
      u32x4 o;
#pragma unroll
      for (int w = 0; w < 4; ++w) o[w] = pack_bf16(fmaxf(v[2 * w], floor_), fmaxf(v[2 * w + 1], floor_));
      __builtin_amdgcn_raw_buffer_store_b128(o, rsrcY, (rr * p.Cout + n0 + ecol) * 2, 0, 0);
    }
  } else if constexpr (!X3) {
    f32x4 bias = *reinterpret_cast<const f32x4 *>(p.bias + n0 + ecol);
    if (partial) bias = f32x4{0.f, 0.f, 0.f, 0.f};
#pragma unroll
    for (int k = 0; k < EPASS; ++k) {
      const int rr = erow + k * RPP;
      f32x4 v = *reinterpret_cast<const f32x4 *>(Cs + rr * CLD + ecol);
      v += bias;
      if (RESID) v += rres[k];
      v[0] = fmaxf(v[0], floor_);
      v[1] = fmaxf(v[1], floor_);
      v[2] = fmaxf(v[2], floor_);
      v[3] = fmaxf(v[3], floor_);
      __builtin_amdgcn_raw_buffer_store_b128(__builtin_bit_cast(u32x4, v), rsrcY,
                                             (int)((rr * p.Cout + n0 + ecol) * 4), 0, 0);
    }
  } else {
    const f32x4 bias0 = *reinterpret_cast<const f32x4 *>(p.bias + n0 + ecol);
    const f32x4 bias1 = *reinterpret_cast<const f32x4 *>(p.bias + n0 + ecol + 4);
#pragma unroll
    for (int k = 0; k < EPASS; ++k) {
      const int rr = erow + k * RPP;
      const f32x4 c0 = *reinterpret_cast<const f32x4 *>(Cs + rr * CLD + ecol);
      const f32x4 c1 = *reinterpret_cast<const f32x4 *>(Cs + rr * CLD + ecol + 4);
      float v[8] = {c0[0] + bias0[0], c0[1] + bias0[1], c0[2] + bias0[2], c0[3] + bias0[3],
                    c1[0] + bias1[0], c1[1] + bias1[1], c1[2] + bias1[2], c1[3] + bias1[3]};
      if (RESID) {
#pragma unroll
        for (int e = 0; e < 8; ++e) v[e] += split_elem(rres_h[k], e) + split_elem(rres_l[k], e);
      }
      u32x4 oh, ol;
#pragma unroll
      for (int w = 0; w < 4; ++w) {
        const float x0 = fmaxf(v[2 * w], floor_), x1 = fmaxf(v[2 * w + 1], floor_);
        unsigned hw, lw;
        split_pair(x0, x1, &hw, &lw);
        oh[w] = hw;
        ol[w] = lw;
      }
      const int o = (rr * p.Cout + n0 + ecol) * 4;
      __builtin_amdgcn_raw_buffer_store_b128(oh, rsrcY, o, 0, 0);
      __builtin_amdgcn_raw_buffer_store_b128(ol, rsrcY, o + 16, 0, 0);
    }
  }
}

int conv_num_segments(const ConvParams &p) {
  if (p.kseg_len <= 0) return 1;
  const int nk = p.Kp / kBK;
  return (nk + p.kseg_len - 1) / p.kseg_len;
}

template <int BM, int BN, int WGM, int WGN, int KS, bool SHIFT>
static hipError_t launch_conv_seg(ConvParams p, hipStream_t s) {
  if constexpr (!((BM == 64 && BN == 64) || (BM == 32 && BN == 32))) {
    return hipErrorInvalidValue;
  } else {
    p.ntm = (p.M + BM - 1) / BM;
    p.ntn = p.Cout / BN;
    const int ntiles = p.ntm * p.ntn;
    if (p.ksplit == 2 && (!p.ypart || p.tail_from <= 0 || p.tail_from >= ntiles || p.tail_from % p.ntn != 0)) return hipErrorInvalidValue;
    const dim3 grid((unsigned)(p.ksplit == 2 ? p.tail_from + (ntiles - p.tail_from) * conv_num_segments(p)
                                             : ntiles * (p.ksplit ? conv_num_segments(p) : 1)));
    const dim3 block(64 * WGM * WGN);
    if constexpr (KS == 1 && !SHIFT) {
      if (p.x2 && p.T > 0) {
        TSM_KLAUNCH_WALK(p.reverse, (conv_igemm<BM, BN, WGM, WGN, 1, false, false, kPrecF32 | kPrecBlockShift, true, true>), grid, block, 0, s, p);
        return hipGetLastError();
      }
      if (p.x2) {
        TSM_KLAUNCH_WALK(p.reverse, (conv_igemm<BM, BN, WGM, WGN, 1, false, false, kPrecF32, true, true>), grid, block, 0, s, p);
        return hipGetLastError();
      }
    }
    TSM_KLAUNCH_WALK(p.reverse, (conv_igemm<BM, BN, WGM, WGN, KS, SHIFT, false, kPrecF32, false, true>), grid, block, 0, s, p);
    return hipGetLastError();
  }
}

template <int BM, int BN, int WGM, int WGN, int KS, bool SHIFT, bool RES>
static hipError_t launch_conv_t(ConvParams p, hipStream_t s) {
  if (p.kseg_len > 0) {
    if constexpr (!RES && KS != 7 && !(SHIFT && KS == 3)) return launch_conv_seg<BM, BN, WGM, WGN, KS, SHIFT>(p, s);
    else return hipErrorInvalidValue;
  }
  p.ntm = (p.M + BM - 1) / BM;
  p.ntn = p.Cout / BN;
  const dim3 grid((unsigned)(p.ntm * p.ntn));
  if constexpr (KS == 1 && !SHIFT && !RES) {
    if (p.x2 && p.T > 0) {
      if (p.prec == kPrecBf16x3)
        TSM_KLAUNCH_WALK(p.reverse, (conv_igemm<BM, BN, WGM, WGN, 1, false, false, kPrecBf16x3 | kPrecBlockShift, true>), grid, dim3(64 * WGM * WGN), 0, s, p);
      else if (p.prec == kPrecBf16)
        TSM_KLAUNCH_WALK(p.reverse, (conv_igemm<BM, BN, WGM, WGN, 1, false, false, kPrecBf16 | kPrecBlockShift, true>), grid, dim3(64 * WGM * WGN), 0, s, p);
      else
        TSM_KLAUNCH_WALK(p.reverse, (conv_igemm<BM, BN, WGM, WGN, 1, false, false, kPrecF32 | kPrecBlockShift, true>), grid, dim3(64 * WGM * WGN), 0, s, p);
      return hipGetLastError();
    }
    if (p.x2) {
      if (p.prec == kPrecBf16x3)
        TSM_KLAUNCH_WALK(p.reverse, (conv_igemm<BM, BN, WGM, WGN, 1, false, false, kPrecBf16x3, true>), grid, dim3(64 * WGM * WGN), 0, s, p);
      else if (p.prec == kPrecBf16)
        TSM_KLAUNCH_WALK(p.reverse, (conv_igemm<BM, BN, WGM, WGN, 1, false, false, kPrecBf16, true>), grid, dim3(64 * WGM * WGN), 0, s, p);
      else
        TSM_KLAUNCH_WALK(p.reverse, (conv_igemm<BM, BN, WGM, WGN, 1, false, false, kPrecF32, true>), grid, dim3(64 * WGM * WGN), 0, s, p);
      return hipGetLastError();
    }
  }
  if constexpr (RES && !SHIFT && KS != 7) {
    if (p.T > 0) {
      if (p.prec == kPrecBf16x3)
        TSM_KLAUNCH_WALK(p.reverse, (conv_igemm<BM, BN, WGM, WGN, KS, false, false, kPrecBf16x3 | kPrecBlockShift>), grid, dim3(64 * WGM * WGN), 0, s, p);
      else if (p.prec == kPrecBf16)
        TSM_KLAUNCH_WALK(p.reverse, (conv_igemm<BM, BN, WGM, WGN, KS, false, false, kPrecBf16 | kPrecBlockShift>), grid, dim3(64 * WGM * WGN), 0, s, p);
      else
        TSM_KLAUNCH_WALK(p.reverse, (conv_igemm<BM, BN, WGM, WGN, KS, false, false, kPrecF32 | kPrecBlockShift>), grid, dim3(64 * WGM * WGN), 0, s, p);
      return hipGetLastError();
    }
  }
  if (p.prec == kPrecBf16x3)
    TSM_KLAUNCH_WALK(p.reverse, (conv_igemm<BM, BN, WGM, WGN, KS, SHIFT, RES, kPrecBf16x3>), grid, dim3(64 * WGM * WGN), 0, s, p);
  else if (p.prec == kPrecBf16)
    TSM_KLAUNCH_WALK(p.reverse, (conv_igemm<BM, BN, WGM, WGN, KS, SHIFT, RES, kPrecBf16>), grid, dim3(64 * WGM * WGN), 0, s, p);
  else
    TSM_KLAUNCH_WALK(p.reverse, (conv_igemm<BM, BN, WGM, WGN, KS, SHIFT, RES, kPrecF32>), grid, dim3(64 * WGM * WGN), 0, s, p);
  return hipGetLastError();
}

void conv_tile_shape(const ConvParams &p, int *bm, int *bn) {
  int BN = (p.Cout % 128 == 0) ? 128 : 64;
  int BM = 128;
  const long tiles128 = (long)((p.M + 127) / 128) * (p.Cout / BN);
  if (tiles128 < 256) {
    BM = 64;
    BN = 64;
  }
  *bm = BM;
  *bn = BN;
}

int conv_tile_from_name(const char *name) {
  if (!name) return kTileAuto;
  static const struct { const char *n; int t; } names[] = {{"128x128", kTile128x128}, {"128x64", kTile128x64},
      {"64x64", kTile64x64}, {"32x32", kTile32x32}, {"128x128w8", kTile128x128w8}, {"256x256", kTile256x256}, {"ws", kTileWs}, {"256x256p", kTile256x256p}};
  for (const auto &e : names)
    if (strcmp(name, e.n) == 0) return e.t;
  return kTileAuto;
}

bool conv_tile_valid(const ConvParams &p, int tile) {
  if (p.T > 0 && (p.res || p.x2 || (p.pad == 0 && p.stride != 1)) &&
      (tile == kTile256x256 || tile == kTileWs || (tile == kTile256x256p && (p.pad != 0 || !(p.res || p.x2)))))
    return false;
  switch (tile) {
    case kTile128x128: return p.Cout % 128 == 0;
    case kTile128x64:
    case kTile64x64: return p.Cout % 64 == 0;
    case kTile32x32: return p.Cout % 32 == 0 && p.prec == kPrecF32;
    case kTile128x128w8: return p.Cout % 128 == 0;
    case kTile256x256:
      return p.prec == kPrecBf16 && p.Cout % 256 == 0 && p.C % 64 == 0 && !(p.res && p.x2) && (p.pad != 1 || (!p.res && p.T == 0)) &&
             (!p.x2 || (p.K1 % 64 == 0 && p.C2 % 64 == 0));
    case kTile256x256p:
      return p.prec == kPrecBf16 && p.Cout % 256 == 0 && p.Cout <= 2048 && p.C % 64 == 0 && p.Kp >= 128 && !(p.res && p.x2) &&
             (p.pad != 1 || (!p.res && p.T == 0)) &&
             (!p.x2 || (p.K1 % 64 == 0 && p.C2 % 64 == 0));
    case kTileWs: return conv3x3_ws_valid(p) || conv3x3_ws128_valid(p) || conv1x1_ws_valid(p) || conv1x1_wsn_valid(p);
    default: return false;
  }
}

void conv_tile_dims(int tile, int *bm, int *bn) {
  *bm = (tile == kTile256x256 || tile == kTile256x256p || tile == kTileWs) ? 256 : tile == kTile32x32 ? 32 : (tile == kTile64x64 ? 64 : 128);
  *bn = (tile == kTile256x256 || tile == kTile256x256p) ? 256 : tile == kTile32x32 ? 32 : ((tile == kTile128x128 || tile == kTile128x128w8) ? 128 : 64);
}


template <int KS, bool SHIFT, bool RES>
static hipError_t launch_conv_ks(const ConvParams &p_in, hipStream_t s) {
  ConvParams p = p_in;
  int bm, bn;
  conv_tile_shape(p, &bm, &bn);
  if (p.tile != kTileAuto) {
    if (!conv_tile_valid(p, p.tile)) return hipErrorInvalidValue;
    conv_tile_dims(p.tile, &bm, &bn);
  }
  if (p.tile == kTile256x256) {
    if constexpr (KS != 7) return launch_conv_bf16_256(p, KS, s);
    else return hipErrorInvalidValue;
  }
  if (p.tile == kTile256x256p) {
    if constexpr (KS != 7) return launch_conv_bf16_256p(p, KS, s);
    else return hipErrorInvalidValue;
  }
  if (p.tile == kTileWs) {
    if constexpr (KS == 3) return launch_conv3x3_ws(p, s);
    else if constexpr (KS == 1 && !RES) return conv1x1_ws_valid(p) ? launch_conv1x1_ws(p, s) : launch_conv1x1_wsn(p, s);
    else return hipErrorInvalidValue;
  }
  if (p.kseg_len > 0 && !(bm == 32 && bn == 32)) {
    bm = 64;
    bn = 64;
    if (p.tile == kTile128x128w8) p.tile = kTile64x64;
  }
  if (bm == 32 && bn == 32) {
    if (p.prec != kPrecF32) return hipErrorInvalidValue;
    return launch_conv_t<32, 32, 1, 1, KS, SHIFT, RES>(p, s);
  }
  if (bm == 128 && bn == 128 && p.tile == kTile128x128w8) return launch_conv_t<128, 128, 4, 2, KS, SHIFT, RES>(p, s);
  if (bm == 128 && bn == 128) return launch_conv_t<128, 128, 2, 2, KS, SHIFT, RES>(p, s);
  if (bm == 128 && bn == 64) return launch_conv_t<128, 64, 2, 2, KS, SHIFT, RES>(p, s);
  return launch_conv_t<64, 64, 2, 2, KS, SHIFT, RES>(p, s);
}

hipError_t launch_conv(const ConvParams &p_in, int ks, hipStream_t s) {
  ConvParams p = p_in;
  const int kc = p.prec == kPrecBf16 ? 64 : kBK;
  if (p.Cout % 64 != 0 || p.Kp % kc != 0 || p.M <= 0) return hipErrorInvalidValue;
  if ((1 << p.logC4) * 4 != p.C) return hipErrorInvalidValue;
  if (ks != 7 && p.C % kc != 0) return hipErrorInvalidValue;
  if (p.T > 0 && ((ks != 1 && ks != 3) || (ks == 3 && p.kseg_len > 0) || p.N % p.T != 0 || p.fold % 4 != 0 ||
                  (p.res && 2 * p.fold > p.Cout) || (p.x2 && 2 * p.fold > p.C2)))
    return hipErrorInvalidValue;
  if (p.x2 && (ks != 1 || p.res || p.K1 % kc != 0 || p.C2 % kc != 0 || p.K1 + p.C2 != p.Kp || p.K1 != p.C))
    return hipErrorInvalidValue;
  if (p.x2 && (128.0 / ((double)p.Ho * p.Wo) + 4.0) * (double)p.Hi2 * p.Wi2 * p.C2 * 4.0 > 2.0e9) return hipErrorInvalidValue;
  if (p.T > 0 && p.res && (128.0 + 2.0 * p.Ho * p.Wo) * p.Cout * 4.0 > 2.0e9) return hipErrorInvalidValue;
  if (p.prec != kPrecF32 && p.prec != kPrecBf16x3 && p.prec != kPrecBf16) return hipErrorInvalidValue;
  if (p.kseg_len < 0 || (p.kseg_len > 0 && (p.prec != kPrecF32 || p.res || ks == 7))) return hipErrorInvalidValue;
  if ((p.ksplit && p.kseg_len <= 0) || p.ksplit < 0 || p.ksplit > 2) return hipErrorInvalidValue;
  if (p.prec != kPrecF32 && p.T > 0 && p.fold % 8 != 0) return hipErrorInvalidValue;
  if (ks == 7 && (p.C != 4 || (p.prec != kPrecF32 && (p.stride != 2 || p.pad != 3)))) return hipErrorInvalidValue;
  const double frames = 128.0 / ((double)p.Ho * p.Wo) + 4.0;
  if (frames * (double)p.Hi * p.Wi * p.C * 4.0 > 2.0e9) return hipErrorInvalidValue;
  switch (ks) {
    case 1:
      if (p.res) return launch_conv_ks<1, false, true>(p, s);
      return p.T > 0 && !p.x2 ? launch_conv_ks<1, true, false>(p, s) : launch_conv_ks<1, false, false>(p, s);
    case 3:
      if (p.res) return launch_conv_ks<3, false, true>(p, s);
      return p.T > 0 ? launch_conv_ks<3, true, false>(p, s) : launch_conv_ks<3, false, false>(p, s);
    case 7: return p.res ? hipErrorInvalidValue : launch_conv_ks<7, false, false>(p, s);
    default: return hipErrorInvalidValue;
  }
}


__global__ void __launch_bounds__(256) splitk_reduce_kernel(const float *__restrict__ partial, int n_seg, int64_t n4,
                                                            int64_t seg_stride4, int cout4,
                                                            const float *__restrict__ bias, const float *__restrict__ res,
                                                            float *__restrict__ y, int relu) {
  const int64_t stride = (int64_t)gridDim.x * blockDim.x;
  const float floor_ = relu ? 0.f : -INFINITY;
  const f32x4 *p4 = reinterpret_cast<const f32x4 *>(partial);
  for (int64_t i = (int64_t)blockIdx.x * blockDim.x + threadIdx.x; i < n4; i += stride) {
    f32x4 t = p4[i];
    for (int sgm = 1; sgm < n_seg; ++sgm) t += p4[i + sgm * seg_stride4];
    f32x4 v = t + reinterpret_cast<const f32x4 *>(bias)[i % cout4];
    if (res) v += reinterpret_cast<const f32x4 *>(res)[i];
    v[0] = fmaxf(v[0], floor_);
    v[1] = fmaxf(v[1], floor_);
    v[2] = fmaxf(v[2], floor_);
    v[3] = fmaxf(v[3], floor_);
    reinterpret_cast<f32x4 *>(y)[i] = v;
  }
}


hipError_t launch_splitk_reduce(const float *partial, int n_seg, int64_t m, int cout, const float *bias,
                                const float *res, float *y, int relu, hipStream_t s) {
  if (!partial || !bias || !y || n_seg < 1 || m <= 0 || cout <= 0 || cout % 4 != 0) return hipErrorInvalidValue;
  const int64_t n4 = m * cout / 4;
  TSM_KLAUNCH(splitk_reduce_kernel, dim3(grid_for(n4, 2048)), dim3(256), 0, s, partial, n_seg, n4, n4, cout / 4,
                     bias, res, y, relu);
  return hipGetLastError();
}

}
```

workoutdetector_amd/csrc/tsm_kernels.h:

```cpp
#pragma once
#include <hip/hip_runtime.h>
#include <stdint.h>

namespace tsm {

struct ConvParams {
  const float *x;
  const float *w;
  const float *bias;
  const float *res;
  float *y;
  int N, Hi, Wi, C, logC4;
  int Ho, Wo, Cout;
  int stride, pad;
  int Kp;
  int M;
  int relu;
  int T;
  int fold;
  int ntm, ntn;
  int tile;
  int prec;
  const float *x2;
  int C2, Hi2, Wi2, stride2;
  int K1;
  int kseg_len;
  int ksplit;
  int tail_from;
  float *ypart;
  int reverse;
};

enum ConvPrec { kPrecF32 = 0, kPrecBf16x3 = 1, kPrecBf16 = 2 };
constexpr int kPrecBlockShift = 4;

enum ConvTile {
  kTileAuto = 0, kTile128x128 = 1, kTile128x64 = 2, kTile64x64 = 3, kTile32x32 = 4,
  kTile128x128w8 = 5,
  kTile256x256 = 6,
  kTileWs = 7,
  kTile256x256p = 8,
  kNumTiles = 9
};
void conv_tile_dims(int tile, int *bm, int *bn);
int conv_tile_from_name(const char *name);
bool conv_tile_valid(const ConvParams &p, int tile);
bool conv3x3_ws_valid(const ConvParams &p);
bool conv3x3_ws128_valid(const ConvParams &p);
bool conv1x1_wsn_valid(const ConvParams &p);
bool conv1x1_ws_valid(const ConvParams &p);

hipError_t launch_conv(const ConvParams &p, int ks, hipStream_t s);
struct Fused23Params {
  const float *x;
  const float *w2;
  const float *bias2;
  const float *w3f;
  const float *bias3;
  const float *res;
  float *y;
  int N, H, W;
  int M;
  int kseg_len;
  int reverse;
};
hipError_t launch_conv23_fused(const Fused23Params &p, int cmid, int cout3, int prec, hipStream_t s);
bool conv23_ws_valid(int n, int h, int w);

struct BneckParams {
  const void *x;
  const void *w1;
  const float *bias1;
  const void *w2;
  const float *bias2;
  const void *w3;
  const float *bias3;
  void *y;
  int cin;
  int N, H, W;
  int T, fold;
  int reverse;
};
bool bneck_ws_valid(int cin, int n, int h, int w, int T, int fold);
hipError_t launch_bneck_ws(const BneckParams &p, hipStream_t s);

struct FrontParams {
  const void *x;
  const void *w1;
  const float *bias1;
  const void *w2;
  const float *bias2;
  void *y;
  int N, H, W;
  int T, fold;
  int reverse;
};
bool front_s2_valid(int n, int h, int w, int T, int fold);
hipError_t launch_front_s2(const FrontParams &p, hipStream_t s);

struct Conv31Params {
  const void *t2;
  const void *w3;
  const float *bias3;
  const void *res;
  void *y;
  const void *w1;
  const float *bias1;
  void *t1;
  int n_clips, T, HW;
  int K3, C, N1;
  int fold;
  int reverse;
  int log_px;
};
bool conv31_valid(const Conv31Params &p);
hipError_t launch_conv31_fused(const Conv31Params &p, hipStream_t s);

hipError_t launch_stem_direct(const float *x, const float *w, const float *bias, float *y, int n, int hi, int wi, int kp,
                              int relu, int prec, hipStream_t s);
hipError_t launch_stem_pool(const float *x, const float *w, const float *bias, float *y, int n, int hi, int wi, int kp,
                            int relu, int prec, hipStream_t s, int planar = 0);
int conv_num_segments(const ConvParams &p);
hipError_t launch_splitk_reduce(const float *partial, int n_seg, int64_t m, int cout, const float *bias,
                                const float *res, float *y, int relu, hipStream_t s);
void conv_tile_shape(const ConvParams &p, int *bm, int *bn);

hipError_t launch_pack_input(const float *src, float *dst, int64_t n_frames, int h, int w,
                             int nchw, int prec, hipStream_t s);
hipError_t launch_from_f32(const float *x, float *y, int64_t n8, int prec, hipStream_t s);
hipError_t launch_to_f32(const float *x, float *y, int64_t n8, int prec, hipStream_t s);
struct PreprocParams {
  const void *src;
  float *dst;
  int n, h, w;
  int nh, nw;
  int top, left, crop;
  int src_is_u8;
  int out_mode;
  float pre_scale;
};
hipError_t launch_preprocess(const PreprocParams &p, hipStream_t s);

struct GatherParams {
  const void *frames;
  void *out;
  int64_t n_frames, frame_bytes, first_frame, total_frames, first_clip, pad_frame;
  int n_clips, n_segment, clip_step, clip_stride;
  int64_t row0;
};
hipError_t launch_gather_clips(const GatherParams &p, hipStream_t s);

struct ClipPreprocParams {
  const void *src;
  float *dst;
  const int *boxes;
  int64_t n_frames, first_frame, total_frames, first_clip;
  int n_clips, n_segment, clip_step, clip_stride;
  int h, w, size;
  int src_is_u8;
  int out_mode;
  float pre_scale;
};
hipError_t launch_preprocess_clips(const ClipPreprocParams &p, hipStream_t s);

hipError_t launch_maxpool3x3s2(const float *x, float *y, int n, int hi, int wi, int c, int prec,
                               hipStream_t s);
hipError_t launch_temporal_shift(const float *x, float *y, int64_t n_frames, int n_segment,
                                 int64_t hw, int c, int fold, hipStream_t s);
hipError_t launch_head(const float *feat, const float *fc_w, const float *fc_b, float *pooled,
                       float *logits, int n_clips, int n_segment, int hw, int c, int num_class, int prec,
                       hipStream_t s);
hipError_t launch_head_segments(const float *feat, const float *fc_w, const float *fc_b, float *logits, int n_frames,
                                int hw, int c, int num_class, int prec, hipStream_t s);

hipError_t launch_scores_to_states(const float *logits, int n, int c, int softmax, float threshold, int *states, float *top,
                                   hipStream_t s);

void note_launch(const char *kernel, const char *where, int reverse = -1);
void trace_launches(bool on);
const char *launch_trace();

}
```

workoutdetector_amd/engine.py:

```python
from __future__ import annotations

import ctypes as C
from dataclasses import dataclass
from typing import Dict, List, Mapping, Optional, Sequence

import numpy as np

from . import _lib
from .weights import (BACKBONES, DEPTHS, SHIFT_PLACES, WIDTHS, is_mmaction_state_dict, make_state_dict, remap_checkpoint_keys,
                      remap_mmaction_keys)

CONSENSUS_TYPES = {'avg': 0, 'identity': 1}


@dataclass
class NodeArg:
    name: str
    shape: list
    type: str = 'tensor(float)'


def _as_f32(a) -> np.ndarray:
    return np.ascontiguousarray(np.asarray(a), dtype=np.float32)


class TsmEngine:
    INPUT_NAME = 'input'
    OUTPUT_NAME = 'output'

    def __init__(self, num_class: int = 12, num_segments: int = 8, height: int = 224, width: int = 224,
                 shift_div: int = 8, is_shift: bool = True, max_clips: int = 32, device: int = 0,
                 state_dict: Optional[Mapping[str, object]] = None, dtype: str = 'f32',
                 base_model: str = 'resnet50', shift_place: str = 'blockres', consensus_type: str = 'avg'):
        if base_model not in DEPTHS:
            raise NotImplementedError(f'{base_model}: the engine implements {", ".join(sorted(DEPTHS))}')
        if shift_place not in SHIFT_PLACES:
            raise ValueError(f"shift_place must be one of {list(SHIFT_PLACES)}, got {shift_place!r}")
        if consensus_type not in CONSENSUS_TYPES:
            raise ValueError(f"consensus_type must be one of {list(CONSENSUS_TYPES)}, got {consensus_type!r}")
        self._lib = _lib.load()
        self._h = C.c_void_p()
        self.num_class, self.num_segments = int(num_class), int(num_segments)
        self.height, self.width = int(height), int(width)
        self.max_clips, self.device = int(max_clips), int(device)
        if dtype not in _lib.DTYPES:
            raise ValueError(f'dtype must be one of {sorted(_lib.DTYPES)}, got {dtype!r}')
        self.dtype = dtype
        self.base_model = base_model
        self.shift_place = shift_place
        self.consensus_type = consensus_type
        self.packed_layout = {'f32': _lib.LAYOUT_NTHWC4, 'bf16x3': _lib.LAYOUT_NTHWC8S,
                              'bf16': _lib.LAYOUT_NTHWC8B}[dtype]
        cfg = _lib.TsmConfig(C.sizeof(_lib.TsmConfig), num_class, num_segments, height, width, shift_div,
                             1 if is_shift else 0, max_clips, device, _lib.DTYPES[dtype])
        _lib.check(self._lib.tsm_create(C.byref(cfg), C.byref(self._h)))
        if DEPTHS[base_model] != 50:
            _lib.check(self._lib.tsm_set_backbone(self._h, DEPTHS[base_model]), self._h)
        if base_model in WIDTHS:
            _lib.check(self._lib.tsm_set_bottleneck_width(self._h, WIDTHS[base_model]), self._h)
        if shift_place != 'blockres':
            _lib.check(self._lib.tsm_set_shift_place(self._h, SHIFT_PLACES[shift_place]), self._h)
        if consensus_type != 'avg':
            _lib.check(self._lib.tsm_set_consensus(self._h, CONSENSUS_TYPES[consensus_type]), self._h)
        self._finalized = False
        if state_dict is not None:
            self.load_state_dict(state_dict)

    def load_state_dict(self, state_dict: Mapping[str, object], strict: bool = False) -> 'TsmEngine':
        for name, value in state_dict.items():
            if name.endswith('num_batches_tracked'):
                continue
            arr = _as_f32(value.detach().cpu().numpy() if hasattr(value, 'detach') else value)
            shape = (C.c_int64 * arr.ndim)(*arr.shape)
            rc = self._lib.tsm_set_tensor(self._h, name.encode(), arr.ctypes.data, shape, arr.ndim)
            if rc == -1 and not strict and b'unknown tensor name' in (self._lib.tsm_last_error(self._h) or b''):
                continue
            _lib.check(rc, self._h)
        _lib.check(self._lib.tsm_finalize(self._h), self._h)
        self._finalized = True
        return self

    def get_inputs(self) -> List[NodeArg]:
        return [NodeArg(self.INPUT_NAME, [None, self.num_segments, 3, self.height, self.width])]

    def get_outputs(self) -> List[NodeArg]:
        return [NodeArg(self.OUTPUT_NAME, [None] + list(self._out_shape(0)[1:]))]

    def _out_shape(self, b: int) -> tuple:
        return (b, self.num_segments, self.num_class) if self.consensus_type == 'identity' else (b, self.num_class)

    def run(self, output_names: Optional[Sequence[str]], input_feed: Dict[str, np.ndarray]) -> List[np.ndarray]:
        if output_names is not None and list(output_names) != [self.OUTPUT_NAME]:
            raise ValueError(f'unknown outputs {output_names}; engine has [{self.OUTPUT_NAME!r}]')
        if set(input_feed) != {self.INPUT_NAME}:
            raise ValueError(f'feed must have exactly the key {self.INPUT_NAME!r}, got {sorted(input_feed)}')
        x = input_feed[self.INPUT_NAME]
        want = (self.num_segments, 3, self.height, self.width)
        if x.ndim != 5 or tuple(x.shape[1:]) != want:
            raise ValueError(f'input must be [B,{want[0]},3,{want[2]},{want[3]}], got {tuple(x.shape)}')
        return [self.forward_host(_as_f32(x))]

    def __call__(self, x):
        is_torch = hasattr(x, 'is_cuda')
        shape = tuple(x.shape)
        if len(shape) == 4:
            if shape[0] % self.num_segments or shape[1:] != (3, self.height, self.width):
                raise ValueError(f'input must be [B*{self.num_segments},3,{self.height},{self.width}], got {shape}')
            b = shape[0] // self.num_segments
        elif len(shape) == 5 and shape[1:] == (self.num_segments, 3, self.height, self.width):
            b = shape[0]
        else:
            raise ValueError(f'bad input shape {shape}')
        if is_torch and x.is_cuda:
            return self.forward_device(x.reshape(b, self.num_segments, 3, self.height, self.width))
        arr = _as_f32(x.detach().numpy() if is_torch else x)
        out = self.forward_host(arr.reshape(b, self.num_segments, 3, self.height, self.width))
        if is_torch:
            import torch
            return torch.from_numpy(out)
        return out

    def eval(self) -> 'TsmEngine':
        return self

    def to(self, *_args, **_kw) -> 'TsmEngine':
        return self

    def _floats_per_clip(self, layout: int) -> int:
        t, h, w = self.num_segments, self.height, self.width
        per = {_lib.LAYOUT_NTCHW: 3 * h * w, _lib.LAYOUT_NTHWC: 3 * h * w, _lib.LAYOUT_NTHWC4: 4 * h * w,
               _lib.LAYOUT_NTHWC8S: 8 * h * ((w + 1) // 2), _lib.LAYOUT_NTHWC8B: 4 * h * ((w + 1) // 2)}
        if layout not in per:
            raise ValueError(f'unknown layout {layout}')
        return t * per[layout]

    def _check_clips(self, n_elems: int, b: int, layout: int) -> None:
        if b <= 0 or n_elems != b * self._floats_per_clip(layout):
            raise ValueError(f'clips hold {n_elems} float32 values; layout {layout} needs {self._floats_per_clip(layout)} '
                             f'per clip x {b} clips (T={self.num_segments}, H={self.height}, W={self.width})')

    def forward_host(self, clips: np.ndarray, layout: int = _lib.LAYOUT_NTCHW) -> np.ndarray:
        self._need_finalized()
        clips = _as_f32(clips)
        b = clips.shape[0]
        self._check_clips(clips.size, b, layout)
        out = np.empty(self._out_shape(b), dtype=np.float32)
        for s in range(0, b, self.max_clips):
            chunk = np.ascontiguousarray(clips[s:s + self.max_clips])
            o = out[s:s + chunk.shape[0]]
            _lib.check(self._lib.tsm_forward(self._h, chunk.ctypes.data, _lib.MEM_HOST, layout, chunk.shape[0],
                                             o.ctypes.data, None), self._h)
        return out

    def forward_device(self, clips, out=None, layout: int = _lib.LAYOUT_NTCHW):
        import torch
        self._need_finalized()
        if not (clips.is_cuda and clips.dtype == torch.float32):
            raise ValueError('forward_device needs a float32 CUDA tensor')
        if clips.device.index != self.device:
            raise ValueError(f'tensor on cuda:{clips.device.index}, engine on cuda:{self.device}')
        clips = clips.contiguous()
        b = clips.shape[0]
        self._check_clips(clips.numel(), b, layout)
        if out is None:
            out = torch.empty(self._out_shape(b), dtype=torch.float32, device=clips.device)
        elif not (out.is_cuda and out.device == clips.device and out.dtype == torch.float32 and out.is_contiguous()
                  and tuple(out.shape) == self._out_shape(b)):
            raise ValueError(f'out must be a contiguous float32 {list(self._out_shape(b))} tensor on {clips.device}')
        stream = torch.cuda.current_stream(clips.device).cuda_stream
        for s in range(0, b, self.max_clips):
            n = min(self.max_clips, b - s)
            _lib.check(self._lib.tsm_forward(self._h, clips[s:s + n].data_ptr(), _lib.MEM_DEVICE, layout, n,
                                             out[s:s + n].data_ptr(), stream), self._h)
        return out

    def warmup(self, batch_sizes: Optional[Sequence[int]] = None) -> 'TsmEngine':
        import torch
        self._need_finalized()
        if batch_sizes is None:
            batch_sizes, b = [], 1
            while b < self.max_clips:
                batch_sizes.append(b)
                b *= 2
            batch_sizes.append(self.max_clips)
        stream = torch.cuda.current_stream(torch.device('cuda', self.device)).cuda_stream
        for b in batch_sizes:
            b = max(1, min(int(b), self.max_clips))
            _lib.check(self._lib.tsm_tune(self._h, b, stream), self._h)
        return self

    def forward_tap(self, clips: np.ndarray, stage: str) -> np.ndarray:
        self._need_finalized()
        clips = _as_f32(clips)
        self._check_clips(clips.size, clips.shape[0], _lib.LAYOUT_NTCHW)
        n = clips.shape[0] * self.num_segments
        h1, w1 = (self.height - 1) // 2 + 1, (self.width - 1) // 2 + 1
        hp, wp = (h1 - 1) // 2 + 1, (w1 - 1) // 2 + 1
        cap = n * max(h1 * w1 * 64, hp * wp * 256, self.height * self.width * 8)
        buf = np.empty(cap, dtype=np.float32)
        shape = (C.c_int64 * 4)()
        _lib.check(self._lib.tsm_forward_tap(self._h, clips.ctypes.data, _lib.MEM_HOST, _lib.LAYOUT_NTCHW,
                                             clips.shape[0], stage.encode(), buf.ctypes.data, cap, shape, None),
                   self._h)
        dims = tuple(int(v) for v in shape)
        return buf[:int(np.prod(dims))].reshape(dims).copy()

    def launch_names(self) -> List[str]:
        names = ['pack_input', 'conv1', 'maxpool']
        blocks, kind = BACKBONES[self.base_model]
        for li, nb in enumerate(blocks, start=1):
            for b in range(nb):
                p = f'layer{li}.{b}'
                if kind == 'basic':
                    names += ([p + '.downsample'] if b == 0 and li > 1 else []) + [p + '.conv1', p + '.conv2']
                else:
                    names += ([p + '.downsample'] if b == 0 else []) + [p + '.conv1', p + '.conv2', p + '.conv3']
        return names + ['head']

    TILE_NAMES = {0: 'heuristic', 1: '128x128', 2: '128x64', 3: '64x64', 4: '32x32', 5: '128x128w8', 6: '256x256', 7: 'ws',
                  8: '256x256p'}

    @classmethod
    def tile_name(cls, code: int) -> str:
        return (cls.TILE_NAMES[code & 15] + ('/splitK' if code & 0x100 else '') + ('/tailK' if code & 0x200 else '') + ('+conv3' if code & 0x400 else '') +
                ('+block' if code & 0x800 else '') + ('+conv1' if code & 0x1000 else '') + ('+conv2' if code & 0x2000 else ''))

    def conv_tiles(self, n_clips: int) -> Dict[str, str]:
        buf = (C.c_int32 * 64)()
        n = C.c_int32()
        _lib.check(self._lib.tsm_conv_tiles(self._h, n_clips, buf, 64, C.byref(n)), self._h)
        names = [k for k in self.launch_names() if k not in ('pack_input', 'maxpool', 'head')]
        assert n.value == len(names)
        return {k: self.tile_name(buf[i]) for i, k in enumerate(names)}

    def set_layer_timing(self, n_forwards: int, only_conv3x3: bool = False) -> None:
        _lib.check(self._lib.tsm_set_layer_timing(self._h, n_forwards, int(only_conv3x3)), self._h)

    def layer_times_ms(self, forward_index: int) -> Dict[str, float]:
        buf = (C.c_float * 80)()
        n = C.c_int32()
        _lib.check(self._lib.tsm_layer_times(self._h, forward_index, C.addressof(buf), 80, C.byref(n)), self._h)
        names = self.launch_names()
        assert n.value == len(names), (n.value, len(names))
        return {k: float(buf[i]) for i, k in enumerate(names)}

    @property
    def last_forward_ms(self) -> float:
        return float(self._lib.tsm_last_forward_ms(self._h))

    def _need_finalized(self) -> None:
        if not self._finalized:
            raise _lib.TsmError(-3, 'load_state_dict() has not been called')

    def close(self) -> None:
        if getattr(self, '_h', None) is not None and self._h.value:
            self._lib.tsm_destroy(self._h)
            self._h = C.c_void_p()

    def __del__(self):
        try:
            self.close()
        except Exception:
            pass


def create_model(num_class: int = 2, num_segments: int = 8, base_model: str = 'resnet50',
                 checkpoint: Optional[str] = None, device: Optional[object] = None, fc_lr5: bool = True,
                 is_shift: bool = True, shift_div: int = 8, shift_place: str = 'blockres',
                 consensus_type: str = 'avg', img_feature_dim: int = 256, non_local: bool = False,
                 height: int = 224, width: int = 224, max_clips: int = 32, seed: int = 0, dtype: str = 'f32',
                 **kwargs) -> TsmEngine:
    if base_model not in DEPTHS:
        raise NotImplementedError(f'{base_model}: the engine implements {", ".join(sorted(DEPTHS))}')
    assert consensus_type in ['avg', 'identity']
    if shift_place not in SHIFT_PLACES:
        raise ValueError(f"shift_place must be one of {list(SHIFT_PLACES)}, got {shift_place!r}")
    if non_local:
        raise NotImplementedError('non_local')
    dev = 0
    if device is not None:
        s = str(device)
        if s == 'cpu':
            raise RuntimeError('TsmEngine has no CPU path; pass a CUDA/HIP device')
        dev = int(s.split(':')[1]) if ':' in s else 0
    if checkpoint is not None and str(checkpoint).endswith('.onnx'):
        from .onnx_import import load_onnx_state_dict
        sd = load_onnx_state_dict(checkpoint, num_class, base_model, shift_place=shift_place)
    elif checkpoint is not None:
        import torch
        ckpt = torch.load(checkpoint, map_location='cpu')
        raw = ckpt['state_dict'] if 'state_dict' in ckpt else ckpt
        sd = (remap_mmaction_keys(raw) if is_mmaction_state_dict(raw)
              else remap_checkpoint_keys(raw, num_class, base_model))
    else:
        sd = make_state_dict(seed=seed, num_class=num_class, base_model=base_model, shift_place=shift_place)
    return TsmEngine(num_class=num_class, num_segments=num_segments, height=height, width=width,
                     shift_div=shift_div, is_shift=is_shift, max_clips=max_clips, device=dev, state_dict=sd,
                     dtype=dtype, base_model=base_model, shift_place=shift_place, consensus_type=consensus_type)


class launch_trace:

    def __init__(self):
        self.kernels: List[str] = []

    def __enter__(self) -> 'launch_trace':
        _lib.load().tsm_trace_launches(1)
        return self

    def __exit__(self, *exc) -> None:
        lib = _lib.load()
        need = int(lib.tsm_launch_trace(None, 0))
        buf = C.create_string_buffer(need)
        lib.tsm_launch_trace(buf, need)
        lib.tsm_trace_launches(0)
        self.kernels = [ln for ln in buf.value.decode().split('\n') if ln]

    def ran(self, prefix: str) -> bool:
        return any(k.startswith(prefix) for k in self.kernels)

    def count(self, prefix: str) -> int:
        return sum(k.startswith(prefix) for k in self.kernels)


def _ptr(t) -> Optional[int]:
    return None if t is None else t.data_ptr()


def _stream(t) -> int:
    import torch
    return torch.cuda.current_stream(t.device).cuda_stream


def _need_cuda_f32(**tensors) -> None:
    import torch
    for name, t in tensors.items():
        if t is None:
            continue
        if not (hasattr(t, 'is_cuda') and t.is_cuda and t.dtype == torch.float32):
            raise ValueError(f'{name} must be a float32 CUDA tensor')


def _out(out, shape, dtype, like, name: str = 'out'):
    import torch
    shape = tuple(int(d) for d in shape)
    if out is None:
        return torch.empty(shape, dtype=dtype, device=like.device)
    if not (hasattr(out, 'is_cuda') and out.is_cuda and out.device == like.device and out.dtype == dtype
            and tuple(out.shape) == shape and out.is_contiguous()):
        raise ValueError(f'{name} must be a contiguous {dtype} tensor of shape {shape} on {like.device}, got '
                         f'{getattr(out, "dtype", type(out))} {tuple(getattr(out, "shape", ()))} on {getattr(out, "device", None)}')
    return out


def temporal_shift_nhwc(x, n_segment: int, fold_div: int = 8, out=None):
    import torch
    _need_cuda_f32(x=x)
    x = x.contiguous()
    n, h, w, c = x.shape
    if n_segment <= 0 or n % n_segment:
        raise ValueError(f'{n} frames are not a whole number of {n_segment}-frame clips')
    y = _out(out, x.shape, torch.float32, x)
    _lib.check(_lib.load().tsm_temporal_shift(x.data_ptr(), y.data_ptr(), n, n_segment, h * w, c, fold_div,
                                              _stream(x)))
    return y


def conv_bn_act_nhwc(x, w, gamma, beta, mean, var, stride: int = 1, relu: bool = True, residual=None,
                     shift_segments: int = 0, fold_div: int = 8, dtype: str = 'f32', *, shift_identity: bool = False,
                     x2=None, w2=None, bn2=None, stride2: int = 1, code: Optional[int] = None, reverse: bool = False, out=None):
    import torch
    _need_cuda_f32(x=x, w=w, gamma=gamma, beta=beta, mean=mean, var=var, residual=residual, x2=x2, w2=w2)
    x = x.contiguous()
    n, hi, wi, cin = x.shape
    cout, wcin, k, k2 = w.shape
    if wcin != cin or k != k2 or any(tuple(t.shape) != (cout,) for t in (gamma, beta, mean, var)):
        raise ValueError(f'w {tuple(w.shape)} / BatchNorm vectors do not match x {tuple(x.shape)}')
    pad = k // 2
    ho, wo = (hi + 2 * pad - k) // stride + 1, (wi + 2 * pad - k) // stride + 1
    y = _out(out, (n, ho, wo, cout), torch.float32, x)
    if residual is not None and tuple(residual.shape) != tuple(y.shape):
        raise ValueError(f'residual {tuple(residual.shape)} must have the output shape {tuple(y.shape)}')
    res = None if residual is None else residual.contiguous()
    args = [t.contiguous() for t in (w, gamma, beta, mean, var)]
    lib = _lib.load()
    if not shift_identity and x2 is None and code is None and not reverse:
        _lib.check(lib.tsm_conv_bn_act(x.data_ptr(), *[a.data_ptr() for a in args], _ptr(res), y.data_ptr(),
                                       n, hi, wi, cin, cout, k, stride, int(relu), shift_segments, fold_div,
                                       _lib.DTYPES[dtype], _stream(x)))
        return y
    a = _lib.TsmConvArgs()
    a.struct_size = C.sizeof(_lib.TsmConvArgs)
    a.x, a.w, a.gamma, a.beta, a.mean, a.var = x.data_ptr(), *[t.data_ptr() for t in args]
    a.residual, a.y = _ptr(res), y.data_ptr()
    a.n, a.hi, a.wi, a.cin, a.cout, a.k, a.stride, a.relu = n, hi, wi, cin, cout, k, stride, int(relu)
    a.shift_segments, a.fold_div, a.dtype, a.shift_target = shift_segments, fold_div, _lib.DTYPES[dtype], int(shift_identity)
    keep = []
    if x2 is not None:
        if w2 is None or bn2 is None:
            raise ValueError('a second source needs w2 and bn2')
        _need_cuda_f32(**{f'bn2[{i}]': t for i, t in enumerate(bn2)})
        x2c = x2.contiguous()
        n2, hi2, wi2, cin2 = x2c.shape
        if n2 != n or tuple(w2.shape) != (cout, cin2, 1, 1) or any(tuple(t.shape) != (cout,) for t in bn2):
            raise ValueError(f'x2 {tuple(x2.shape)} / w2 {tuple(w2.shape)} / bn2 do not match x {tuple(x.shape)}, cout {cout}')
        keep = [x2c] + [t.contiguous() for t in (w2, *bn2)]
        a.x2, a.w2, a.gamma2, a.beta2, a.mean2, a.var2 = (t.data_ptr() for t in keep)
        a.cin2, a.hi2, a.wi2, a.stride2 = cin2, hi2, wi2, stride2
    a.code, a.reverse = int(code or 0), int(reverse)
    _lib.check(lib.tsm_conv_op(C.byref(a), _stream(x)))
    del keep
    return y


def preprocess_frames(frames, resize: int = 256, crop: int = 224, scale_255: bool = False, packed: bool = True,
                      layout: Optional[int] = None, out=None):
    import torch
    frames = frames.contiguous()
    if frames.dtype == torch.uint8:
        pixel = _lib.PIXEL_U8
    elif frames.dtype == torch.float32:
        pixel = _lib.PIXEL_F32
    else:
        raise ValueError(f'frames must be uint8 or float32, got {frames.dtype}')
    n, h, w, c = frames.shape
    if c != 3 or not frames.is_cuda:
        raise ValueError('frames must be a CUDA tensor [n,H,W,3]')
    if layout is None:
        layout = _lib.LAYOUT_NTHWC4 if packed else _lib.LAYOUT_NTCHW
    pairs = (crop + 1) // 2
    shape = {_lib.LAYOUT_NTHWC4: (n, crop, crop, 4), _lib.LAYOUT_NTHWC8S: (n, crop, pairs, 8),
             _lib.LAYOUT_NTHWC8B: (n, crop, pairs, 4),
             _lib.LAYOUT_NTCHW: (n, 3, crop, crop)}[layout]
    out = _out(out, shape, torch.float32, frames)
    _lib.check(_lib.load().tsm_preprocess(frames.data_ptr(), pixel, n, h, w, out.data_ptr(), layout, resize, crop,
                                          int(scale_255), _stream(frames)))
    return out


def gather_clips(frames, first_frame: int, total_frames: int, first_clip: int, n_clips: int, out=None,
                 n_segment: int = 8, clip_step: int = 8, clip_stride: int = 2, pad_frame: Optional[int] = None):
    import torch
    if not frames.is_cuda or not frames.is_contiguous():
        raise ValueError('frames must be a contiguous CUDA tensor')
    n = int(frames.shape[0])
    frame_bytes = int(frames[0].numel()) * frames.element_size()
    if out is None:
        out = torch.empty((n_clips, n_segment) + tuple(frames.shape[1:]), dtype=frames.dtype, device=frames.device)
    if (not out.is_cuda or not out.is_contiguous() or out.device != frames.device
            or out.numel() * out.element_size() != n_clips * n_segment * frame_bytes):
        raise ValueError('out must be a contiguous CUDA tensor of n_clips * n_segment frames on the frames\' device')
    _lib.check(_lib.load().tsm_gather_clips(frames.data_ptr(), n, frame_bytes, int(first_frame), int(total_frames),
                                            n - 1 if pad_frame is None else int(pad_frame), int(first_clip), n_clips,
                                            n_segment, clip_step, clip_stride, out.data_ptr(), _stream(frames)))
    return out


def preprocess_clips(frames, boxes, first_frame: int, total_frames: int, first_clip: int, n_clips: int, size: int = 224,
                     scale_255: bool = False, layout: Optional[int] = None, packed: bool = True, n_segment: int = 8,
                     clip_step: int = 8, clip_stride: int = 2, out=None):
    import torch
    if frames.dtype == torch.uint8:
        pixel = _lib.PIXEL_U8
    elif frames.dtype == torch.float32:
        pixel = _lib.PIXEL_F32
    else:
        raise ValueError(f'frames must be uint8 or float32, got {frames.dtype}')
    if frames.dim() != 4 or frames.shape[3] != 3 or not frames.is_cuda or not frames.is_contiguous():
        raise ValueError('frames must be a contiguous CUDA tensor [n,H,W,3]')
    n, h, w, _ = frames.shape
    if not (hasattr(boxes, 'is_cuda') and boxes.is_cuda and boxes.device == frames.device and boxes.dtype == torch.int32
            and tuple(boxes.shape) == (n_clips, 4) and boxes.is_contiguous()):
        raise ValueError(f'boxes must be a contiguous int32 tensor [{n_clips}, 4] = (top, left, h, w) on {frames.device}')
    if layout is None:
        layout = _lib.LAYOUT_NTHWC4 if packed else _lib.LAYOUT_NTCHW
    pairs = (size + 1) // 2
    frame = {_lib.LAYOUT_NTHWC4: (size, size, 4), _lib.LAYOUT_NTHWC8S: (size, pairs, 8), _lib.LAYOUT_NTHWC8B: (size, pairs, 4),
             _lib.LAYOUT_NTCHW: (3, size, size)}[layout]
    out = _out(out, (n_clips, n_segment) + frame, torch.float32, frames)
    _lib.check(_lib.load().tsm_preprocess_clips(frames.data_ptr(), pixel, n, h, w, int(first_frame), int(total_frames),
                                                int(first_clip), n_clips, n_segment, clip_step, clip_stride, boxes.data_ptr(),
                                                out.data_ptr(), layout, size, int(scale_255), _stream(frames)))
    return out


def scores_to_states(logits, threshold: float = 0.5, softmax: bool = True, return_top: bool = False, out=None, out_top=None):
    import torch
    _need_cuda_f32(logits=logits)
    if logits.dim() != 2 or logits.shape[0] == 0:
        raise ValueError(f'logits must be [n >= 1, num_class], got {tuple(logits.shape)}')
    logits = logits.contiguous()
    n, c = logits.shape
    if out_top is not None and not return_top:
        raise ValueError('out_top needs return_top=True')
    states = _out(out, (n,), torch.int32, logits)
    top = _out(out_top, (n,), torch.float32, logits, 'out_top') if return_top else None
    _lib.check(_lib.load().tsm_scores_to_states(logits.data_ptr(), n, c, int(softmax), float(threshold),
                                                states.data_ptr(), _ptr(top), _stream(logits)))
    return (states, top) if return_top else states


def maxpool3x3s2_nhwc(x, out=None):
    import torch
    _need_cuda_f32(x=x)
    x = x.contiguous()
    n, hi, wi, c = x.shape
    y = _out(out, (n, (hi - 1) // 2 + 1, (wi - 1) // 2 + 1, c), torch.float32, x)
    _lib.check(_lib.load().tsm_maxpool3x3s2(x.data_ptr(), y.data_ptr(), n, hi, wi, c, _stream(x)))
    return y


def head_nhwc(feat, fc_w, fc_b, n_segment: int, out=None):
    import torch
    _need_cuda_f32(feat=feat, fc_w=fc_w, fc_b=fc_b)
    feat = feat.contiguous()
    n, h, w, c = feat.shape
    if n_segment <= 0 or n % n_segment or tuple(fc_w.shape)[1:] != (c,) or tuple(fc_b.shape) != (fc_w.shape[0],):
        raise ValueError(f'feat {tuple(feat.shape)}, fc_w {tuple(fc_w.shape)}, fc_b {tuple(fc_b.shape)}, T={n_segment} do not fit')
    b = n // n_segment
    out = _out(out, (b, fc_w.shape[0]), torch.float32, feat)
    _lib.check(_lib.load().tsm_head(feat.data_ptr(), fc_w.contiguous().data_ptr(), fc_b.contiguous().data_ptr(),
                                    out.data_ptr(), b, n_segment, h * w, c, fc_w.shape[0], _stream(feat)))
    return out


def head_segments_nhwc(feat, fc_w, fc_b, out=None):
    import torch
# ... 10 lines not shown
```

Before: 1877.

## Add tap-skip 3x3 conv path that reorders output rows by live-tap class

Adds a new 3x3 conv mode for the 64x64 segmented fp32 igemm. Output pixels are regrouped into border classes so that each 64-row tile can skip K steps for filter taps that fall entirely in padding. Results are scattered back to their real positions in the epilogue, or in a new row-mapped split-K reduce kernel. The mode is offered as an extra autotune candidate. The cost is a per-tile row table in LDS, scattered stores, and the padding work saved only on border pixels.

```diff
diff --git a/workoutdetector_amd/csrc/tsm_engine.hip b/workoutdetector_amd/csrc/tsm_engine.hip
--- a/workoutdetector_amd/csrc/tsm_engine.hip
+++ b/workoutdetector_amd/csrc/tsm_engine.hip
@@ -153,6 +153,7 @@
   int fuse_block = -1;
   int fuse31 = -1;
   int fuse_front = -1;
+  int tap_skip = -1;
   int walk = -1;
   int n_cu = 256;
   int timing_left = 0;
@@ -357,7 +358,7 @@
 void tune_cache_store(tsm_engine *e, int key, const std::vector<int> &codes) {
   if (e->tune_path.empty()) return;
   std::string line = e->tune_sig + "|" + std::to_string(key) + "|";
-  for (size_t i = 0; i < codes.size(); ++i) line += (i ? "," : "") + std::to_string(codes[i]);
+  for (size_t i = 0; i < codes.size(); ++i) line += (i ? "," : "") + tune_code_text(codes[i]);
   line += "\n";
   if (line.size() >= 4096) return;
   FILE *f = fopen(e->tune_path.c_str(), "a");
@@ -373,8 +374,18 @@
   return from > 0;
 }
 
+bool tap_skip_applies(const tsm::ConvParams &p, int ks, int code) {
+  return (code & kCodeTapSkip) && (code & kCodeTileMask) == tsm::kTile64x64 && !(code & kCodeSplitK) && ks == 3 && p.pad == 1 &&
+         p.kseg_len > 0 && p.prec == tsm::kPrecF32 && p.T == 0 && !p.res && !p.x2 &&
+         (double)p.N * p.Hi * p.Wi * p.C * 4.0 <= 2.0e9 && (double)p.M * p.Cout * 4.0 <= 2.0e9;
+}
+
 hipError_t launch_conv_code(tsm::ConvParams p, int ks, int code, float *partial, size_t partial_elems, int n_cu, hipStream_t s) {
   p.tile = code & kCodeTileMask;
+  if (tap_skip_applies(p, ks, code)) {
+    p.tapskip = 1;
+    p.tap = tap_skip_map(p.N, p.Ho, p.Wo, p.stride, p.Hi, p.Wi);
+  }
   if ((code & kCodeSplitK) && p.kseg_len > 0 &&
       (size_t)tsm::conv_num_segments(p) * (size_t)p.M * (size_t)p.Cout <= partial_elems) {
     float *y = p.y;
@@ -395,8 +406,10 @@
       p.ypart = partial;
       hipError_t st = tsm::launch_conv(p, ks, s);
       if (st == hipSuccess)
-        st = tsm::launch_splitk_reduce(partial, tsm::conv_num_segments(p), p.M - mt0, p.Cout, p.bias, nullptr,
-                                       y + (size_t)mt0 * p.Cout, p.relu, s);
+        st = p.tapskip ? tsm::launch_splitk_reduce(partial, tsm::conv_num_segments(p), p.M - mt0, p.Cout, p.bias, nullptr, y, p.relu, s,
+                                                   &p.tap, mt0, p.Ho, p.Wo)
+                       : tsm::launch_splitk_reduce(partial, tsm::conv_num_segments(p), p.M - mt0, p.Cout, p.bias, nullptr,
+                                                   y + (size_t)mt0 * p.Cout, p.relu, s);
       return st;
     }
   }
@@ -616,6 +629,7 @@
     int code = tiles ? (*tiles)[idx] : 0;
     if (e->force_tile) code = e->force_tile;
     if (e->force_code >= 0) code = e->force_code;
+    if (e->tap_skip >= 0 && (code & kCodeTileMask) == tsm::kTile64x64) code = e->tap_skip ? code | kCodeTapSkip : code & ~kCodeTapSkip;
     TSM_LAUNCH_K(e, s, is3x3, launch_code(p, ks, checked_code(p, code)));
     return TSM_OK;
   }
@@ -629,6 +643,9 @@
     }
     int tail_from = 0;
     if (tail_split_from(p, e->n_cu, e->partial_elems, &tail_from)) cands.push_back((int)tsm::kTile64x64 | kCodeTailK);
+    if (e->tap_skip != 0)
+      for (size_t i = 0, n0 = cands.size(); i < n0; ++i)
+        if (tap_skip_applies(p, ks, cands[i] | kCodeTapSkip)) cands.push_back(cands[i] | kCodeTapSkip);
   } else {
     for (int t = 1; t < tsm::kNumTiles; ++t)
       if (tsm::conv_tile_valid(p, t)) cands.push_back(t);
@@ -964,6 +981,7 @@
   if (const char *fb = getenv("TSM_FUSE_BLOCK")) e->fuse_block = atoi(fb) != 0;
   if (const char *f31 = getenv("TSM_FUSE_C3C1")) e->fuse31 = atoi(f31) != 0;
   if (const char *ff = getenv("TSM_FUSE_FRONT")) e->fuse_front = atoi(ff) != 0;
+  if (const char *ts = getenv("TSM_TAP_SKIP")) e->tap_skip = atoi(ts) != 0;
   if (const char *wk = getenv("TSM_WALK")) e->walk = atoi(wk) != 0;
   if (const char *po = getenv("TSM_POISON")) e->poison = atoi(po) != 0;
   {
@@ -993,7 +1011,7 @@
                   " T" + std::to_string(cfg->num_segments) + " " + std::to_string(cfg->height) + "x" +
                   std::to_string(cfg->width) + " dtype" + std::to_string(cfg->dtype) + " shift" +
                   std::to_string(cfg->is_shift ? cfg->shift_div : 0) + " fuse" + std::to_string(e->fuse23) + "/" + std::to_string(e->fuse_block) + "/" + std::to_string(e->fuse31) + "/" + std::to_string(e->fuse_front) +
-                  " stem" + std::to_string(e->stem_direct ? 1 : 0) +
+                  " tapskip" + std::to_string(e->tap_skip) + " stem" + std::to_string(e->stem_direct ? 1 : 0) +
                   std::to_string(e->stem_pool ? 1 : 0) + std::to_string(e->stem_planar ? 1 : 0);
     e->tune_sig_base = e->tune_sig.size();
   }
@@ -1361,6 +1379,20 @@
       if (p.conv23) codes[b.conv2] |= it->second[b.conv2] & kCodeConv23;
       if (p.conv31_next) codes[b.conv3] |= it->second[b.conv3] & kCodeConv31;
     }
+    const int nn = n_clips * e->cfg.num_segments, shiftT = e->cfg.is_shift ? e->cfg.num_segments : 0;
+    std::vector<bool> takes(codes.size(), false);
+    int hh = e->hp, ww = e->wp;
+    for (size_t k = 0; k < e->blocks.size(); ++k) {
+      const Block &b = e->blocks[k];
+      const int ci = b.conv3 >= 0 ? b.conv2 : b.conv1;
+      const tsm::ConvParams p3 = b.conv3 >= 0 ? block_launches(e, k, nn, nullptr, nullptr, nullptr, nullptr, hh, ww).p2
+                                              : make_params(e->convs[ci], nullptr, nullptr, nullptr, nn, hh, ww, true, shiftT, e->cfg.shift_div, e->prec);
+      takes[ci] = e->tap_skip != 0 && !plan[k].block && !plan[k].front && !plan[k].conv23 && tap_skip_applies(p3, 3, codes[ci]);
+      hh = (hh + 2 - 3) / b.stride + 1;
+      ww = (ww + 2 - 3) / b.stride + 1;
+    }
+    for (size_t i = 0; i < codes.size(); ++i)
+      if (!takes[i]) codes[i] &= ~kCodeTapSkip;
   }
   std::vector<int> order{0};
   for (const Block &b : e->blocks)
@@ -1453,6 +1485,7 @@
   c.kp = (stem && x3) ? round_up(7 * 4 * 8, prec == tsm::kPrecBf16 ? 64 : 32)
                       : round_up(k * k * c.cp, prec == tsm::kPrecBf16 ? 64 : 32);
   const int kp2 = dual ? round_up(cin2, prec == tsm::kPrecBf16 ? 64 : 32) : 0;
+  if ((a->code & (kCodeSplitK | kCodeTailK | kCodeTapSkip)) && !dual && !stem && !(T > 0 && k == 3)) c.kseg = segment_len(c.kp, prec);
 #define TSM_HIP0(call)                                                                              \
   do {                                                                                              \
     hipError_t _st = (call);                                                                        \
diff --git a/workoutdetector_amd/csrc/tsm_host_util.h b/workoutdetector_amd/csrc/tsm_host_util.h
--- a/workoutdetector_amd/csrc/tsm_host_util.h
+++ b/workoutdetector_amd/csrc/tsm_host_util.h
@@ -5,7 +5,9 @@
 #include <cstdio>
 #include <cstdlib>
 #include <cstring>
+#include <initializer_list>
 #include <string>
+#include <utility>
 #include <vector>
 
 namespace tsm_host {
@@ -32,6 +34,85 @@
   const size_t tail_rows = (size_t)(m_rows - (from / ntn) * 64);
   if ((size_t)n_seg * tail_rows * (size_t)cout > scratch_elems) return 0;
   return from;
+}
+
+#ifdef __HIPCC__
+#define TSM_HD __host__ __device__
+#else
+#define TSM_HD
+#endif
+struct TapMap {
+  int off[10];
+  int cnt[9];
+  int nx[9];
+  int y0[9], x0[9];
+  int mask[9];
+};
+
+inline TapMap tap_skip_map(int frames, int Ho, int Wo, int stride, int Hi, int Wi) {
+  TapMap t{};
+  for (int c = 0; c < 9; ++c) t.cnt[c] = t.nx[c] = 1;
+  if (frames <= 0 || Ho <= 0 || Wo <= 0 || stride < 1 || Hi <= 0 || Wi <= 0 || Ho != (Hi - 1) / stride + 1 || Wo != (Wi - 1) / stride + 1 ||
+      (long long)frames * Ho * Wo > 0x7fffffffLL)
+    return t;
+  struct Group { int o0, n, mask; };
+  auto axis = [&](int no, int ni, Group g[3]) {
+    auto live = [&](int o) { int m = 0; for (int k = 0; k < 3; ++k) if (o * stride - 1 + k >= 0 && o * stride - 1 + k < ni) m |= 1 << k; return m; };
+    const bool last = no > 1 && live(no - 1) != 7;
+    g[0] = {0, 1, live(0)};
+    g[1] = {1, no - 1 - (last ? 1 : 0), 7};
+    g[2] = {no - 1, last ? 1 : 0, last ? live(no - 1) : 0};
+  };
+  Group gy[3], gx[3];
+  axis(Ho, Hi, gy);
+  axis(Wo, Wi, gx);
+  struct Cls { int dead, cnt, nx, y0, x0, mask; } cls[9];
+  int n = 0;
+  for (int a : {1, 0, 2})
+    for (int b : {1, 0, 2}) {
+      int mask = 0;
+      for (int ky = 0; ky < 3; ++ky)
+        for (int kx = 0; kx < 3; ++kx)
+          if ((gy[a].mask >> ky & 1) && (gx[b].mask >> kx & 1)) mask |= 1 << (ky * 3 + kx);
+      const int cnt = gy[a].n * gx[b].n;
+      if (cnt > 0) cls[n++] = {9 - __builtin_popcount(mask), cnt, gx[b].n, gy[a].o0, gx[b].o0, mask};
+    }
+  for (int i = 1; i < n; ++i)
+    for (int j = i; j > 0 && cls[j - 1].dead > cls[j].dead; --j) std::swap(cls[j - 1], cls[j]);
+  int row = 0;
+  for (int c = 0; c < 9; ++c) {
+    t.off[c] = row;
+    if (c >= n) continue;
+    t.cnt[c] = cls[c].cnt; t.nx[c] = cls[c].nx; t.y0[c] = cls[c].y0; t.x0[c] = cls[c].x0; t.mask[c] = cls[c].mask;
+    row += frames * cls[c].cnt;
+  }
+  t.off[9] = row;
+  return t;
+}
+
+TSM_HD inline void tap_map_row(const TapMap &t, int r, int *frame, int *oy, int *ox, unsigned *mask) {
+  int off = t.off[0], cnt = t.cnt[0], nx = t.nx[0], y0 = t.y0[0], x0 = t.x0[0], mk = t.mask[0];
+#ifdef __HIPCC__
+#pragma unroll
+#endif
+  for (int c = 1; c < 9; ++c) {
+    const bool in = r >= t.off[c];
+    off = in ? t.off[c] : off; cnt = in ? t.cnt[c] : cnt; nx = in ? t.nx[c] : nx;
+    y0 = in ? t.y0[c] : y0; x0 = in ? t.x0[c] : x0; mk = in ? t.mask[c] : mk;
+  }
+  const int i = r - off, f = i / cnt, px = i - f * cnt, dy = px / nx;
+  *frame = f; *oy = y0 + dy; *ox = x0 + (px - dy * nx); *mask = (unsigned)mk;
+}
+
+TSM_HD inline unsigned tap_map_tile_mask(const TapMap &t, int tile) {
+  const int m0 = tile * 64, m1 = m0 + 64 < t.off[9] ? m0 + 64 : t.off[9];
+  unsigned mask = 0;
+#ifdef __HIPCC__
+#pragma unroll
+#endif
+  for (int c = 0; c < 9; ++c)
+    if (t.off[c] < m1 && t.off[c + 1] > m0) mask |= (unsigned)t.mask[c];
+  return mask;
 }
 
 inline uint16_t f2bf(float f) {
@@ -196,9 +277,14 @@
 constexpr int kCodeBlock = 0x800;
 constexpr int kCodeConv31 = 0x1000;
 constexpr int kCodeFront = 0x2000;
+constexpr int kCodeTapSkip = 0x4000;
 constexpr int kCodeFused = kCodeConv23 | kCodeBlock | kCodeConv31 | kCodeFront;
-constexpr int kCodeValid = kCodeTileMask | kCodeSplitK | kCodeTailK | kCodeFused;
-
+constexpr int kCodeValid = kCodeTileMask | kCodeSplitK | kCodeTailK | kCodeTapSkip | kCodeFused;
+
+constexpr int kCodeFileBits = kCodeValid & ~kCodeTapSkip;
+inline std::string tune_code_text(int code) {
+  return std::to_string(code & ~kCodeTapSkip) + ((code & kCodeTapSkip) ? "t" : "");
+}
 inline bool parse_tune_line(const char *line, const std::string &want, int num_tiles, std::vector<int> *codes) {
   if (strncmp(line, want.c_str(), want.size()) != 0) return false;
   std::vector<int> got;
@@ -207,8 +293,12 @@
     char *end = nullptr;
     const long v = strtol(q, &end, 10);
     if (end == q) return false;
-    if (v < 0 || (v & ~(long)kCodeValid) != 0 || (int)(v & kCodeTileMask) >= num_tiles) return false;
+    if (v < 0 || (v & ~(long)kCodeFileBits) != 0 || (int)(v & kCodeTileMask) >= num_tiles) return false;
     got.push_back((int)v);
+    if (*end == 't') {
+      got.back() |= kCodeTapSkip;
+      ++end;
+    }
     if (*end == ',') q = end + 1;
     else if (*end == '\n' || *end == 0) q = end;
     else return false;
diff --git a/workoutdetector_amd/csrc/tsm_igemm.hip b/workoutdetector_amd/csrc/tsm_igemm.hip
--- a/workoutdetector_amd/csrc/tsm_igemm.hip
+++ b/workoutdetector_amd/csrc/tsm_igemm.hip
@@ -6,7 +6,10 @@
 __global__ void __launch_bounds__(64 * WGM * WGN, (SEG && BM == 64) ? ((PREC & kPrecBlockShift) ? 4 : 5) : 1)
 conv_igemm(const ConvParams p) {
   constexpr bool BSHIFT = (PREC & kPrecBlockShift) != 0;
-  constexpr int PMODE = PREC & ~kPrecBlockShift;
+  constexpr bool TSKIP = (PREC & kPrecTapSkip) != 0;
+  constexpr int PMODE = PREC & ~(kPrecBlockShift | kPrecTapSkip);
+  static_assert(!TSKIP || (SEG && KS == 3 && !SHIFT && !RES && !DUAL && !BSHIFT && BM == 64 && BN == 64),
+                "tap skip: the segmented fp32 3x3 on the 64x64 tile");
   static_assert(!BSHIFT || (!SHIFT && !RES), "block placement: a shifted identity (DUAL = false) or a shifted second source");
   constexpr bool RESID = RES || (BSHIFT && !DUAL);
   static_assert(!SEG || (PMODE == kPrecF32 && !RES && WGM * WGN <= 4 && BM == BN && BM <= 64),
@@ -30,7 +33,7 @@
   static_assert(TM >= 1 && TN >= 1, "wave tile must hold at least one 32x32 MFMA tile");
   constexpr int SMEM_FLOATS = NBUF * (BM + BN) * kLds > BM * CLD ? NBUF * (BM + BN) * kLds : BM * CLD;
 
-  __shared__ __attribute__((aligned(16))) float smem[SMEM_FLOATS];
+  __shared__ __attribute__((aligned(16))) float smem[SMEM_FLOATS + (TSKIP ? 3 * BM : 0)];
 
   const int tid = threadIdx.x;
   const int lane = tid & 63;
@@ -60,7 +63,7 @@
   const int m0 = tm * BM, n0 = tn * BN;
 
   const int HoWo = p.Ho * p.Wo;
-  const int n_first = m0 / HoWo;
+  const int n_first = TSKIP ? 0 : m0 / HoWo;
   const int frame0 = SHIFT ? (n_first > 0 ? n_first - 1 : 0) : n_first;
   constexpr bool PAIRS = KS == 7 && PMODE != kPrecF32;
   const int wpairs = (p.Wi + 1) >> 1;
@@ -83,9 +86,22 @@
   const int lrow = tid >> 3;
   const int chunk = tid & 7;
   const int frame_bytes = (int)(frame_elems * EB);
+  int *rowtab = reinterpret_cast<int *>(smem + SMEM_FLOATS);
+  if constexpr (TSKIP) {
+    if (tid < BM) {
+      const bool ok = m0 + tid < p.M;
+      int n, oy, ox;
+      unsigned live_taps;
+      tsm_host::tap_map_row(p.tap, ok ? m0 + tid : m0, &n, &oy, &ox, &live_taps);
+      rowtab[tid] = n * (int)(frame_elems * EB) + ((oy * p.stride - p.pad) * p.Wi + ox * p.stride - p.pad) * p.C * EB;
+      rowtab[BM + tid] = ok ? (int)live_taps : 0;
+      rowtab[2 * BM + tid] = ok ? (n * p.Ho + oy) * p.Wo + ox : -1;
+    }
+    __syncthreads();
+  }
   unsigned a_off[APASS];
   unsigned a_offp[SHIFT ? APASS : 1], a_offm[SHIFT ? APASS : 1];
-  unsigned a_mask[KS == 3 ? APASS : 1];
+  unsigned a_mask[(KS == 3 && !TSKIP) ? APASS : 1];
   unsigned a_off2[DUAL ? APASS : 1];
   unsigned a_off2p[(BSHIFT && DUAL) ? APASS : 1], a_off2m[(BSHIFT && DUAL) ? APASS : 1];
   int a_iy[KS == 7 ? APASS : 1], a_ix[KS == 7 ? APASS : 1];
@@ -93,6 +109,11 @@
   for (int pp = 0; pp < APASS; ++pp) {
     const int m = m0 + lrow + LRP * pp;
     const bool ok = m < p.M;
+    if constexpr (TSKIP) {
+      a_off[pp] = (unsigned)(rowtab[lrow + LRP * pp] + chunk * 16);
+      a_mask[0] = (pp ? a_mask[0] : 0u) | ((unsigned)rowtab[BM + lrow + LRP * pp] << (9 * pp));
+      continue;
+    }
     const int mm = ok ? m : m0;
     const int n = mm / HoWo;
     const int rem = mm - n * HoWo;
@@ -153,7 +174,7 @@
     k.tap_off = 0;
     int c0 = kt * KC;
     if (KS == 3) {
-      k.tap = (kt * KC) >> (p.logC4 + 2);
+      k.tap = TSKIP ? kt >> (p.logC4 - 3) : (kt * KC) >> (p.logC4 + 2);
       c0 = kt * KC - k.tap * p.C;
       const int ky = k.tap / 3, kx = k.tap - ky * 3;
       k.tap_off = ((ky * p.Wi + kx) * p.C + c0) * EB;
@@ -193,6 +214,8 @@
           const unsigned off = (a_offp[pp] & k.mp) | (a_offm[pp] & k.mm) | (a_off[pp] & k.m0);
           const bool ok = ((a_mask[pp] >> k.tap) & 1u) && off != kInvalid;
           ra[pp] = buf_load4(rsrcA, (ok ? off + (unsigned)k.tap_off : kInvalid) | k.dead, 0);
+        } else if (TSKIP) {
+          ra[pp] = buf_load4(rsrcA, (((a_mask[0] >> (k.tap + 9 * pp)) & 1u) ? a_off[pp] + (unsigned)k.tap_off : kInvalid) | k.dead, 0);
         } else {
           ra[pp] = buf_load4(rsrcA, (((a_mask[pp] >> k.tap) & 1u) ? a_off[pp] + (unsigned)k.tap_off : kInvalid) | k.dead, 0);
         }
@@ -419,15 +442,26 @@
     }
   };
   const int seg_len = (SEG && p.kseg_len > 0) ? p.kseg_len : 0x3fffffff;
+  const unsigned live = TSKIP ? tsm_host::tap_map_tile_mask(p.tap, tm) : 0x1ffu;
+  const int lcpt = TSKIP ? p.logC4 - 3 : 0, k_all = 9 << lcpt;
+  auto live_from = [&](int kt) {
+    if (kt >= k_all) return k_all;
+    const int tap = kt >> lcpt;
+    const unsigned rest = live >> tap;
+    if (rest & 1u) return kt;
+    return rest ? (tap + __builtin_ctz(rest)) << lcpt : k_all;
+  };
+  int kc = TSKIP ? live_from(kt0) : kt0, kn1 = TSKIP ? live_from(kc + 1) : kt0 + 1;
+  (void)k_all;
   {
-    const KStep k0 = kstep(kt0, nk);
-#pragma unroll
-    for (int it = 0; it < NITEMS; ++it) gload_item(k0, kt0, it);
+    const KStep k0 = kstep(kc, nk);
+#pragma unroll
+    for (int it = 0; it < NITEMS; ++it) gload_item(k0, kc, it);
 #pragma unroll
     for (int it = 0; it < NITEMS; ++it) lstore_item(0, it);
-    const KStep k1 = kstep(kt0 + 1, nk);
-#pragma unroll
-    for (int it = 0; it < NITEMS; ++it) gload_item(k1, kt0 + 1, it);
+    const KStep k1 = kstep(kn1, nk);
+#pragma unroll
+    for (int it = 0; it < NITEMS; ++it) gload_item(k1, kn1, it);
   }
   __syncthreads();
   if constexpr (BF) {
@@ -458,6 +492,45 @@
     f32x4 ra_[4], rb_[4];
     const bool trim = KS == 7 && p.Kp == 224 && nk == 7;
     const int nk_full = trim ? nk - 1 : nk;
+    if constexpr (TSKIP) {
+      for (int s0 = kt0; s0 < nk; s0 += seg_len) {
+        const int kend = s0 + seg_len < nk ? s0 + seg_len : nk;
+        while (kc < kend) {
+          const int kn2 = live_from(kn1 + 1);
+          const KStep k2 = kstep(kn2, nk);
+          {
+            const float *As = smem + (wm * WTM + l31) * kLds + half * 4;
+            const float *Bs = smem + BM * kLds + (wn * WTN + l31) * kLds + half * 4;
+#pragma unroll
+            for (int kk = 0; kk < 4; ++kk) {
+              ra_[kk] = *reinterpret_cast<const f32x4 *>(As + kk * 8);
+              rb_[kk] = *reinterpret_cast<const f32x4 *>(Bs + kk * 8);
+            }
+          }
+          __syncthreads();
+          int cnt = 0;
+#pragma unroll
+          for (int kk = 0; kk < 4; ++kk)
+#pragma unroll
+            for (int s4 = 0; s4 < 4; ++s4) {
+              acc[0][0] = __builtin_amdgcn_mfma_f32_32x32x2f32(ra_[kk][s4], rb_[kk][s4], acc[0][0], 0, 0, 0);
+              ++cnt;
+              const int done = cnt < 12 ? (cnt * 2 * NITEMS) / 12 : 2 * NITEMS;
+              const int before = cnt - 1 < 12 ? ((cnt - 1) * 2 * NITEMS) / 12 : 2 * NITEMS;
+#pragma unroll
+              for (int it = before; it < done; ++it) {
+                if (it < NITEMS) lstore_item(0, it);
+                else gload_item(k2, kn2, it - NITEMS);
+                __builtin_amdgcn_sched_barrier(0);
+              }
+            }
+          __syncthreads();
+          kc = kn1;
+          kn1 = kn2;
+        }
+        seg_flush();
+      }
+    } else {
     for (int kt = kt0; kt < nk_full;) {
     const int kend = (SEG && kt + seg_len < nk_full) ? kt + seg_len : nk_full;
     for (; kt < kend; ++kt) {
@@ -491,6 +564,7 @@
       __syncthreads();
     }
     seg_flush();
+    }
     }
     if (KS == 7 && trim) {
       const f32x4 a0 = *reinterpret_cast<const f32x4 *>(smem + (wm * WTM + l31) * kLds + half * 4);
@@ -554,11 +628,12 @@
             SEG ? tot[SEG ? i : 0][SEG ? j : 0][e] : acc[i][j][e];
   __syncthreads();
 
+  const bool scatter = TSKIP && !split_wg;
   const bool partial = split_wg;
-  const size_t y_bytes = ((size_t)p.M - m0) * p.Cout * EB;
+  const size_t y_bytes = ((size_t)p.M - (scatter ? 0 : m0)) * p.Cout * EB;
   const int mt0 = in_tail ? (p.tail_from / p.ntn) * BM : 0;
   char *ybase = in_tail ? reinterpret_cast<char *>(p.ypart) + ((size_t)seg * (p.M - mt0) + (m0 - mt0)) * p.Cout * EB
-                        : reinterpret_cast<char *>(p.y) + ((size_t)(partial ? seg : 0) * p.M + m0) * p.Cout * EB;
+                        : reinterpret_cast<char *>(p.y) + ((size_t)(partial ? seg : 0) * p.M + (scatter ? 0 : m0)) * p.Cout * EB;
   const __amdgpu_buffer_rsrc_t rsrcY = __builtin_amdgcn_make_buffer_rsrc(
       ybase, 0, (int)(y_bytes > 0x7FFFFFF0u ? 0x7FFFFFF0u : y_bytes), 0x00020000);
   const float floor_ = (p.relu && !partial) ? 0.f : -INFINITY;
@@ -594,8 +669,14 @@
       v[1] = fmaxf(v[1], floor_);
       v[2] = fmaxf(v[2], floor_);
       v[3] = fmaxf(v[3], floor_);
-      __builtin_amdgcn_raw_buffer_store_b128(__builtin_bit_cast(u32x4, v), rsrcY,
-                                             (int)((rr * p.Cout + n0 + ecol) * 4), 0, 0);
+      unsigned yoff = (unsigned)((rr * p.Cout + n0 + ecol) * 4);
+      if constexpr (TSKIP) {
+        if (scatter) {
+          const int px = rowtab[2 * BM + rr];
+          yoff = px >= 0 ? (unsigned)((px * p.Cout + n0 + ecol) * 4) : kInvalid;
+        }
+      }
+      __builtin_amdgcn_raw_buffer_store_b128(__builtin_bit_cast(u32x4, v), rsrcY, (int)yoff, 0, 0);
     }
   } else {
     const f32x4 bias0 = *reinterpret_cast<const f32x4 *>(p.bias + n0 + ecol);
@@ -653,6 +734,14 @@
       if (p.x2) {
         TSM_KLAUNCH_WALK(p.reverse, (conv_igemm<BM, BN, WGM, WGN, 1, false, false, kPrecF32, true, true>), grid, block, 0, s, p);
         return hipGetLastError();
+      }
+    }
+    if (p.tapskip) {
+      if constexpr (KS == 3 && !SHIFT && BM == 64) {
+        TSM_KLAUNCH_WALK(p.reverse, (conv_igemm<BM, BN, WGM, WGN, 3, false, false, kPrecF32 | kPrecTapSkip, false, true>), grid, block, 0, s, p);
+        return hipGetLastError();
+      } else {
+        return hipErrorInvalidValue;
       }
     }
     TSM_KLAUNCH_WALK(p.reverse, (conv_igemm<BM, BN, WGM, WGN, KS, SHIFT, false, kPrecF32, false, true>), grid, block, 0, s, p);
@@ -812,6 +901,11 @@
   if (p.kseg_len < 0 || (p.kseg_len > 0 && (p.prec != kPrecF32 || p.res || ks == 7))) return hipErrorInvalidValue;
   if ((p.ksplit && p.kseg_len <= 0) || p.ksplit < 0 || p.ksplit > 2) return hipErrorInvalidValue;
   if (p.prec != kPrecF32 && p.T > 0 && p.fold % 8 != 0) return hipErrorInvalidValue;
+  if (p.tapskip && (ks != 3 || p.pad != 1 || p.kseg_len <= 0 || p.prec != kPrecF32 || p.T > 0 || p.res || p.x2 || p.ksplit == 1 ||
+                    p.tile != kTile64x64 || p.tap.off[9] != p.M || p.M != p.N * p.Ho * p.Wo ||
+                    p.Ho != (p.Hi - 1) / p.stride + 1 || p.Wo != (p.Wi - 1) / p.stride + 1 ||
+                    (double)p.N * p.Hi * p.Wi * p.C * 4.0 > 2.0e9 || (double)p.M * p.Cout * 4.0 > 2.0e9))
+    return hipErrorInvalidValue;
   if (ks == 7 && (p.C != 4 || (p.prec != kPrecF32 && (p.stride != 2 || p.pad != 3)))) return hipErrorInvalidValue;
   const double frames = 128.0 / ((double)p.Ho * p.Wo) + 4.0;
   if (frames * (double)p.Hi * p.Wi * p.C * 4.0 > 2.0e9) return hipErrorInvalidValue;
@@ -849,10 +943,40 @@
 }
 
 
+__global__ void __launch_bounds__(256) splitk_reduce_rows_kernel(const float *__restrict__ partial, int n_seg, int64_t n4,
+                                                                 int64_t seg_stride4, int cout4, const float *__restrict__ bias,
+                                                                 float *__restrict__ y, int relu, const tsm_host::TapMap map,
+                                                                 int row0, int ho, int wo) {
+  const int64_t stride = (int64_t)gridDim.x * blockDim.x;
+  const float floor_ = relu ? 0.f : -INFINITY;
+  const f32x4 *p4 = reinterpret_cast<const f32x4 *>(partial);
+  for (int64_t i = (int64_t)blockIdx.x * blockDim.x + threadIdx.x; i < n4; i += stride) {
+    f32x4 t = p4[i];
+    for (int sgm = 1; sgm < n_seg; ++sgm) t += p4[i + sgm * seg_stride4];
+    const int row = (int)(i / cout4), c4 = (int)(i - (int64_t)row * cout4);
+    f32x4 v = t + reinterpret_cast<const f32x4 *>(bias)[c4];
+    v[0] = fmaxf(v[0], floor_);
+    v[1] = fmaxf(v[1], floor_);
+    v[2] = fmaxf(v[2], floor_);
+    v[3] = fmaxf(v[3], floor_);
+    int n, oy, ox;
+    unsigned unused;
+    tsm_host::tap_map_row(map, row0 + row, &n, &oy, &ox, &unused);
+    reinterpret_cast<f32x4 *>(y)[((int64_t)(n * ho + oy) * wo + ox) * cout4 + c4] = v;
+  }
+}
+
 hipError_t launch_splitk_reduce(const float *partial, int n_seg, int64_t m, int cout, const float *bias,
-                                const float *res, float *y, int relu, hipStream_t s) {
+                                const float *res, float *y, int relu, hipStream_t s, const tsm_host::TapMap *map, int row0,
+                                int ho, int wo) {
   if (!partial || !bias || !y || n_seg < 1 || m <= 0 || cout <= 0 || cout % 4 != 0) return hipErrorInvalidValue;
   const int64_t n4 = m * cout / 4;
+  if (map) {
+    if (res || row0 < 0 || row0 + m > map->off[9] || ho <= 0 || wo <= 0) return hipErrorInvalidValue;
+    TSM_KLAUNCH(splitk_reduce_rows_kernel, dim3(grid_for(n4, 2048)), dim3(256), 0, s, partial, n_seg, n4, n4, cout / 4, bias, y,
+                relu, *map, row0, ho, wo);
+    return hipGetLastError();
+  }
   TSM_KLAUNCH(splitk_reduce_kernel, dim3(grid_for(n4, 2048)), dim3(256), 0, s, partial, n_seg, n4, n4, cout / 4,
                      bias, res, y, relu);
   return hipGetLastError();
diff --git a/workoutdetector_amd/csrc/tsm_kernels.h b/workoutdetector_amd/csrc/tsm_kernels.h
--- a/workoutdetector_amd/csrc/tsm_kernels.h
+++ b/workoutdetector_amd/csrc/tsm_kernels.h
@@ -1,6 +1,8 @@
 #pragma once
 #include <hip/hip_runtime.h>
 #include <stdint.h>
+
+#include "tsm_host_util.h"
 
 namespace tsm {
 
@@ -29,10 +31,13 @@
   int tail_from;
   float *ypart;
   int reverse;
+  int tapskip;
+  tsm_host::TapMap tap;
 };
 
 enum ConvPrec { kPrecF32 = 0, kPrecBf16x3 = 1, kPrecBf16 = 2 };
 constexpr int kPrecBlockShift = 4;
+constexpr int kPrecTapSkip = 8;
 
 enum ConvTile {
   kTileAuto = 0, kTile128x128 = 1, kTile128x64 = 2, kTile64x64 = 3, kTile32x32 = 4,
@@ -122,7 +127,8 @@
                             int relu, int prec, hipStream_t s, int planar = 0);
 int conv_num_segments(const ConvParams &p);
 hipError_t launch_splitk_reduce(const float *partial, int n_seg, int64_t m, int cout, const float *bias,
-                                const float *res, float *y, int relu, hipStream_t s);
+                                const float *res, float *y, int relu, hipStream_t s, const tsm_host::TapMap *map = nullptr,
+                                int row0 = 0, int ho = 0, int wo = 0);
 void conv_tile_shape(const ConvParams &p, int *bm, int *bn);
 
 hipError_t launch_pack_input(const float *src, float *dst, int64_t n_frames, int h, int w,
diff --git a/workoutdetector_amd/engine.py b/workoutdetector_amd/engine.py
--- a/workoutdetector_amd/engine.py
+++ b/workoutdetector_amd/engine.py
@@ -222,7 +222,7 @@
 
     @classmethod
     def tile_name(cls, code: int) -> str:
-        return (cls.TILE_NAMES[code & 15] + ('/splitK' if code & 0x100 else '') + ('/tailK' if code & 0x200 else '') + ('+conv3' if code & 0x400 else '') +
+        return (cls.TILE_NAMES[code & 15] + ('/splitK' if code & 0x100 else '') + ('/tailK' if code & 0x200 else '') + ('/tapskip' if code & 0x4000 else '') + ('+conv3' if code & 0x400 else '') +
                 ('+block' if code & 0x800 else '') + ('+conv1' if code & 0x1000 else '') + ('+conv2' if code & 0x2000 else ''))
 
     def conv_tiles(self, n_clips: int) -> Dict[str, str]:
```

After: 1892 (median of 6 runs). No clear change (+0.8%).
